# innate2adaptive/decombinator

Hardware: AMD Instinct MI355X
Metric: Mreads/s decombined (150 bp human-beta) (higher is better)
Workload: dtype u8

## Files before the change

decombinator_amd/csrc/dcrx_kernels_v2.hip:

```cpp
#include <hip/hip_runtime.h>
#include <hip/hip_ext.h>

#include <algorithm>
#include <cstddef>
#include <cstdio>
#include <cstdlib>
#include <vector>

#include "../../include/dcrx.h"
#include "dcrx_device.h"
#include "dcrx_launch.h"
#include "dcrx_dcr_device.h"
#include "dcrx_v2_device.h"
#include "dcrx_sink_device.h"

namespace dcrx {

bool first_use_on_device(bool (&seen)[64]);
void attributes_set_on_device(bool (&seen)[64]);

constexpr int DCRX_V2_BLOCK = 1024;
#ifdef DCRX_SCAN_STAMPS
__device__ uint32_t *g_scan_stamps;
#endif
// ... 115 lines not shown
    const uint32_t n_ok = (uint32_t)__popcll(m_ok), n_jn = (uint32_t)__popcll(m_jn), n_jm = (uint32_t)__popcll(m_jm),
                   n_tl = (uint32_t)__popcll(m_tl), n_im = (uint32_t)__popcll(m_im), n_ov = (uint32_t)__popcll(m_ov);
    const uint32_t all = (uint32_t)__popcll(m_all);
    if (m_jw) atomicAdd(&lds_counts[DCRX_C_VJ_ASSIGNMENT_FAILED], (uint32_t)__popcll(m_jw));
    if (all) atomicAdd(&lds_counts[DCRX_C_READ_COUNT], all);
    if (n_ok) { atomicAdd(&lds_counts[DCRX_C_VJ_COUNT], n_ok); if (forward) atomicAdd(&lds_counts[DCRX_C_FRAME_FORWARD], n_ok); }
    if (n_jn) atomicAdd(&lds_counts[DCRX_C_NO_J_ASSIGNED], n_jn);
    if (n_jm) atomicAdd(&lds_counts[DCRX_C_MULTIPLE_J_MATCHES], n_jm);
    if (n_jn + n_jm) atomicAdd(&lds_counts[DCRX_C_VJ_ASSIGNMENT_FAILED], n_jn + n_jm);
    if (n_tl) atomicAdd(&lds_counts[DCRX_C_DCRFILTER_TOOLONG_INTERTAG], n_tl);
    if (n_im) atomicAdd(&lds_counts[DCRX_C_DCRFILTER_IMPOSS_DELETION], n_im);
    if (n_ov) atomicAdd(&lds_counts[DCRX_C_DCRFILTER_TAG_OVERLAP], n_ov);
  }
}

__device__ __forceinline__ void v2_tally_rescue(uint32_t *lds_counts, const int lane, const int status, const uint32_t errs, const bool forward) {
  const bool done = status >= 0;
  const unsigned long long m_all = __ballot(done);
  if (!m_all) return;
  auto cnt = [&](const bool c) { return (uint32_t)__popcll(__ballot(done && c)); };
  const uint32_t n_ok = cnt(status == DCRX_S_OK), n_v1 = cnt(status == DCRX_S_V_HALF1_EXHAUSTED), n_v2 = cnt(status == DCRX_S_V_HALF2_EXHAUSTED),
                 n_vn = cnt(status == DCRX_S_V_NONE), n_jm = cnt(status == DCRX_S_J_MULTI), n_jn = cnt(status == DCRX_S_J_NONE),
                 n_j1 = cnt(status == DCRX_S_J_HALF1_EXHAUSTED), n_j2 = cnt(status == DCRX_S_J_HALF2_EXHAUSTED),
                 n_tl = cnt(status == DCRX_S_F_TOOLONG), n_im = cnt(status == DCRX_S_F_IMPOSS_DEL), n_ov = cnt(status == DCRX_S_F_OVERLAP),
                 n_jw = cnt(status == DCRX_S_J_WALK_FAIL),
                 e_v1 = cnt((errs & 1u) != 0u), e_v2 = cnt((errs & 2u) != 0u), e_j1 = cnt((errs & 4u) != 0u), e_j2 = cnt((errs & 8u) != 0u);
  if (lane == 0) {
    auto add = [&](const int c, const uint32_t k) { if (k) atomicAdd(&lds_counts[c], k); };
    add(DCRX_C_READ_COUNT, (uint32_t)__popcll(m_all));
    add(DCRX_C_VJ_COUNT, n_ok);
    if (forward) add(DCRX_C_FRAME_FORWARD, n_ok);
    add(DCRX_C_FOUNDV1NOTV2, n_v1);
    add(DCRX_C_FOUNDV2NOTV1, n_v2 + n_j2);
    add(DCRX_C_NO_VTAGS_FOUND, n_vn);
    add(DCRX_C_MULTIPLE_J_MATCHES, n_jm);
    add(DCRX_C_NO_J_ASSIGNED, n_jn);
    add(DCRX_C_FOUNDJ1NOTJ2, n_j1);
    add(DCRX_C_VJ_ASSIGNMENT_FAILED, n_jm + n_jn + n_j1 + n_j2 + n_jw);
    add(DCRX_C_DCRFILTER_TOOLONG_INTERTAG, n_tl);
    add(DCRX_C_DCRFILTER_IMPOSS_DELETION, n_im);
    add(DCRX_C_DCRFILTER_TAG_OVERLAP, n_ov);
    add(DCRX_C_VERR1, e_v1); add(DCRX_C_VERR2, e_v2); add(DCRX_C_JERR1, e_j1); add(DCRX_C_JERR2, e_j2);
  }
}

template <int NW, int RPL>
__device__ __forceinline__ void v2_load_item(const BatchDev &B, const uint32_t nw, const uint64_t first, const uint64_t hi, const int lane,
                                             uint32_t (&w)[RPL][NW], unsigned long long (&xm)[RPL]) {
#pragma unroll
  for (int q = 0; q < RPL; q++) {
    const uint64_t r = first + (uint64_t)q * 64 + lane;
    const uint2 *wp2 = reinterpret_cast<const uint2 *>(B.packed + (r < hi ? r : 0) * B.stride);
#pragma unroll
    for (int k = 0; k < NW / 2; k++) {
      uint2 t = make_uint2(0u, 0u);
      if ((uint32_t)(2 * k) < nw && r < hi) t = wp2[k];
      w[q][2 * k] = t.x; w[q][2 * k + 1] = t.y;
    }
    xm[q] = 0ull;
    if (B.n_exc) {
      const uint64_t g = (first + (uint64_t)q * 64) >> 5;
      xm[q] = (unsigned long long)B.exc_flag[g] | ((unsigned long long)B.exc_flag[g + 1] << 32);
    }
  }
}


__device__ __forceinline__ void v2_exc_slice(const BatchDev &B, const uint64_t blk_lo, const uint64_t blk_hi, uint32_t *s, const int tid) {
  if (B.n_exc <= 16u * blockDim.x) {
    if (tid < 4) s[tid] = 0u;
    __syncthreads();
    uint32_t below_lo = 0, below_hi = 0;
    for (uint64_t i = (uint32_t)tid; i < B.n_exc; i += blockDim.x) {
      const uint64_t r = B.exc_read[i];
      below_lo += r < blk_lo ? 1u : 0u;
      below_hi += r < blk_hi ? 1u : 0u;
    }
#pragma unroll
    for (int o = 32; o > 0; o >>= 1) { below_lo += __shfl_xor(below_lo, o); below_hi += __shfl_xor(below_hi, o); }
    if ((tid & 63) == 0) { if (below_lo) atomicAdd(&s[0], below_lo); if (below_hi) atomicAdd(&s[2], below_hi); }
    __syncthreads();
    return;
  }
  const uint32_t half = blockDim.x >> 1;
  const int which = (uint32_t)tid >= half ? 1 : 0;
  const uint32_t j = (uint32_t)tid - (which ? half : 0u);
  const uint64_t key = which ? blk_hi : blk_lo;
  if (tid < 2) { s[2 * tid] = 0u; s[2 * tid + 1] = (uint32_t)B.n_exc; }
  for (;;) {
    __syncthreads();
    const uint32_t lo = s[2 * which], hi = s[2 * which + 1], span = hi - lo;
    const bool done = s[1] == s[0] && s[3] == s[2];
    __syncthreads();
    if (done) break;
    if (tid < 2) s[4 + tid] = 0u;
    __syncthreads();
    const uint32_t step = span ? (span + half - 1) / half : 1u;
    const uint64_t idx = (uint64_t)lo + (uint64_t)j * step;
    const bool below = span && idx < hi && (uint64_t)B.exc_read[idx] < key;
    const unsigned long long m = __ballot(below);
    if ((tid & 63) == 0 && m) atomicAdd(&s[4 + which], (uint32_t)__popcll(m));
    __syncthreads();
    if (j == 0 && span) {
      const uint32_t c = s[4 + which], probes = (span + step - 1) / step;
      s[2 * which] = c ? lo + (c - 1) * step + 1 : lo;
      s[2 * which + 1] = c < probes ? lo + c * step : hi;
    }
  }
}
__device__ __forceinline__ void v2_exc_marks(const BatchDev &B, const uint32_t e_lo, const uint32_t e_hi, const bool set, const int tid) {
  uint32_t *flag = const_cast<uint32_t *>(B.exc_flag);
  for (uint64_t i = (uint64_t)e_lo + (uint32_t)tid; i < e_hi; i += blockDim.x) {
    const uint32_t r = B.exc_read[i];
    if (set) { if (i == e_lo || B.exc_read[i - 1] != r) atomicOr(&flag[r >> 5], 1u << (r & 31)); }
    else flag[r >> 5] = 0u;
  }
}

template <int NW>
__device__ __forceinline__ uint32_t *v2_left_valid(uint4 *left_rows) { return reinterpret_cast<uint32_t *>(left_rows + (size_t)V2_LEFT_CAP * V2Rows<NW>::E); }
template <int NW>
__device__ __forceinline__ bool v2_left_push(uint4 *left_rows, uint32_t *__restrict__ queue_count, const uint32_t x0, const uint32_t (&lg)[NW], const uint32_t (&w)[NW]) {
  const uint32_t at = atomicAdd(queue_count + V2_QC_LEFT, 1u);
  if (at >= V2_LEFT_CAP) return false;
  uint32_t x[1 + 2 * NW];
  x[0] = x0;
#pragma unroll
  for (int k = 0; k < NW; k++) { x[1 + k] = lg[k]; x[1 + NW + k] = w[k]; }
  v2_put_rows<1 + 2 * NW>(left_rows, 0u, at, x);
  __threadfence();
  __hip_atomic_store(v2_left_valid<NW>(left_rows) + at, 1u, __ATOMIC_RELAXED, __HIP_MEMORY_SCOPE_AGENT);
  return true;
}

enum { V2_WK_NEXT = 0, V2_WK_LIST = 1, V2_WK_EXC = 8, V2_WK_HEAD = 16, V2_WK_CLAIM = 17, V2_WK_SCANNED = 18, V2_WK_SINK = 19, V2_WK_HEAD2 = 20, V2_WK_CLAIM2 = 21,
       V2_WK_FILLED = 32, V2_WK_GEN = 48, V2_WK_FILLED2 = 64, V2_WK_GEN2 = 80, V2_WK_WORDS = 96 };
#ifndef DCRX_V2_FUSE_TAILWAVES
#define DCRX_V2_FUSE_TAILWAVES 3
#endif
#ifndef DCRX_V2_PRIO_TAIL
#define DCRX_V2_PRIO_TAIL 1
#endif
constexpr int V2_FUSE_TAILWAVES = DCRX_V2_FUSE_TAILWAVES;
constexpr uint32_t V2_TW6_FRAC256 = 243, V2_TW5_FRAC256 = 205, V2_TW4_FRAC256 = 136, V2_TW3_FRAC256 = 64;
constexpr int V2_RING_STRIDE = 15;
constexpr uint32_t V2_RING_MAXBATCHES = 16;
template <int NW> constexpr int v2_ering_stride() { return (2 * NW + 4) | 1; }
constexpr uint32_t V2_ERING_BATCHES = 8;
#ifndef DCRX_V2_HELP_DRAIN
#define DCRX_V2_HELP_DRAIN 0
#endif
constexpr float V2_FUSE_E_MAX_SHARE = 0.25f;

template <bool UNIFORM_LEN, int NW, int RPL, bool NARROW, bool PREFETCH = true, int FUSE = -1, bool SINK = false, bool FUSE_E = false>
__global__ __launch_bounds__(DCRX_V2_BLOCK) void scan2_kernel(
    DevTables T0, BatchDev B, CfgDev cfg, dcrx_record_t *__restrict__ records, unsigned long long *__restrict__ counters,
    V2Lists Q, uint32_t *__restrict__ queue, uint32_t *__restrict__ gqueue, uint32_t qcap, uint32_t *__restrict__ queue_count,
    uint64_t per_block, uint32_t retry, const DevTables *__restrict__ Tmem, uint32_t ring_batches, V2SinkCall S, uint32_t tail_waves, uint32_t rescue_waves) {
  static_assert(!FUSE_E || (FUSE >= 0 && !SINK), "the event ring rides on the fused form, without a tuple sink");
  extern __shared__ __align__(64) uint32_t smem[];
  if constexpr (FUSE >= 0 && !SINK) S.dev = nullptr;
  const int o = FUSE >= 0 ? FUSE : (cfg.orientation == DCRX_ORIENT_FORWARD ? 0 : 1);
  V2Ori V0 = T0.v2[0];
  if (o) V0 = T0.v2[1];
  uint32_t *lds_trans = smem;
  uint32_t *lds_counts = smem + V0.trans_bytes / 4;
  uint32_t *lds_work = lds_counts + DCRX_N_COUNTERS;
  const int tid = threadIdx.x;
#ifdef DCRX_SCAN_STAMPS
  const unsigned long long stamp_r0 = __builtin_amdgcn_s_memrealtime();
  unsigned long long stamp_setup = 0, stamp_loop_end = 0;
#endif
  if (tid < DCRX_N_COUNTERS) lds_counts[tid] = 0;
  if (tid < V2_WK_WORDS) lds_work[tid] = 0;
  {
    const uint4 *src = reinterpret_cast<const uint4 *>(V0.trans);
    uint4 *dst = reinterpret_cast<uint4 *>(lds_trans);
    for (uint32_t i = tid; i < V0.trans_bytes / 16; i += blockDim.x) dst[i] = src[i];
  }
  const V2Tab tab{};
  uint32_t *lds_side = lds_work + V2_WK_WORDS;
  uint32_t *lds_bk = lds_side + (T0.lds_image_bytes - T0.dfa_bytes) / 4;
  uint32_t *ring = lds_bk + V0.bk_bytes / 4;
  const uint32_t ring_mask = 64u * ring_batches - 1u;
  constexpr uint32_t ES = (uint32_t)v2_ering_stride<NW>(), ering_mask = 64u * V2_ERING_BATCHES - 1u;
  uint32_t *ring2 = ring + (size_t)(ring_mask + 1u) * V2_RING_STRIDE;
  uint32_t *lds_dry = ring2 + (size_t)(ering_mask + 1u) * ES;
  if (FUSE >= 0) {
    {
      const uint4 *s1 = reinterpret_cast<const uint4 *>(T0.image + T0.dfa_bytes), *s2 = reinterpret_cast<const uint4 *>(V0.bk);
      uint4 *d1 = reinterpret_cast<uint4 *>(lds_side), *d2 = reinterpret_cast<uint4 *>(lds_bk);
      for (uint32_t i = tid; i < (T0.lds_image_bytes - T0.dfa_bytes) / 16; i += blockDim.x) d1[i] = s1[i];
      for (uint32_t i = tid; i < V0.bk_bytes / 16; i += blockDim.x) d2[i] = s2[i];
    }
    for (uint32_t i = tid; i <= ring_mask; i += blockDim.x) { ring[i * V2_RING_STRIDE + NW] = 0u; ring[i * V2_RING_STRIDE + NW + 1] = 0u; }
    if (FUSE_E) for (uint32_t i = tid; i <= ering_mask; i += blockDim.x) { ring2[i * ES + NW] = 0u; ring2[i * ES + NW + 1] = 0u; }
  }
  __syncthreads();
  const uint32_t nw = B.stride >> 2;
  const int lane = tid & 63;
  const unsigned long long lt_mask = (1ull << lane) - 1ull;
  const bool tagged = B.n_reads < (1ull << 30);

  const uint64_t blk_lo = (uint64_t)blockIdx.x * per_block;
  const uint64_t blk_hi = blk_lo + per_block < B.n_reads ? blk_lo + per_block : B.n_reads;
  uint32_t e_lo = 0u, e_hi = 0u;
  if (B.n_exc) {
    v2_exc_slice(B, blk_lo < blk_hi ? blk_lo : blk_hi, blk_hi, lds_work + V2_WK_EXC, tid);
    e_lo = lds_work[V2_WK_EXC]; e_hi = lds_work[V2_WK_EXC + 2];
    v2_exc_marks(B, e_lo, e_hi, true, tid);
    asm volatile("s_waitcnt vmcnt(0)" ::: "memory");
    __syncthreads();
  }
  uint32_t tw = tail_waves;
  if (FUSE >= 0 && tw == 0u) {
    const uint32_t h = Q.counts[V2_L_COUNTS * blockIdx.x + V2_L_TWHINT + (o ? 0 : 1)];
    tw = (h >= 2u && h <= 8u) ? h : (uint32_t)V2_FUSE_TAILWAVES;
    if (FUSE_E && tw > 2u) tw -= 1u;
  }
  const uint32_t rw = FUSE_E ? rescue_waves : 0u;
  const uint32_t n_scan_waves = (blockDim.x >> 6) - (FUSE >= 0 ? tw : 0u) - rw;
  const size_t region = blockIdx.x;
#ifdef DCRX_SCAN_STAMPS
  stamp_setup = __builtin_amdgcn_s_memrealtime();
#endif
  const uint32_t wv = (uint32_t)(tid >> 6);
  const bool scans = wv < n_scan_waves;
  if (scans) {
#ifdef DCRX_V2_PRIO_SCAN
  if (FUSE >= 0) __builtin_amdgcn_s_setprio(DCRX_V2_PRIO_SCAN);
#endif
  constexpr uint32_t WT = 64u * RPL;
  const uint32_t n_items = blk_lo < blk_hi ? (uint32_t)((blk_hi - blk_lo + WT - 1) / WT) : 0u;
  uint4 *tq = Q.tail + region * Q.tcap * V2Rows<NW>::T;
  uint4 *eq = Q.ev + region * Q.ecap * V2Rows<NW>::E;
  auto draw = [&]() -> uint32_t {
    uint32_t i = 0;
    if (lane == 0) i = atomicAdd(&lds_work[V2_WK_NEXT], 1u);
    return (uint32_t)__builtin_amdgcn_readfirstlane((int)i);
  };

  const int npairs = UNIFORM_LEN ? (int)((B.read_len + 1u) >> 1) : 8 * (int)(nw < (uint32_t)NW ? nw : (uint32_t)NW);
  uint32_t w[RPL][NW];
  unsigned long long xm[RPL];
  uint32_t item = draw();
  if (PREFETCH && item < n_items) v2_load_item<NW, RPL>(B, nw, blk_lo + (uint64_t)item * WT, blk_hi, lane, w, xm);
  if (PREFETCH) {
#pragma unroll
    for (int q = 0; q < RPL; q++) {
#pragma unroll
      for (int k = 0; k < NW; k++) asm volatile("" : "+v"(w[q][k]));
      asm volatile("" : "+v"(xm[q]));
    }
  }
  while (item < n_items) {
    uint32_t wn[RPL][NW];
    unsigned long long xn[RPL];
    const uint32_t next = draw();
    const bool more = next < n_items;
    if (!PREFETCH) v2_load_item<NW, RPL>(B, nw, blk_lo + (uint64_t)item * WT, blk_hi, lane, w, xm);
    if (PREFETCH) { if (more) v2_load_item<NW, RPL>(B, nw, blk_lo + (uint64_t)next * WT, blk_hi, lane, wn, xn); }
    uint32_t lg[RPL][NW];
#if DCRX_V2_LOOP_PRIO
    __builtin_amdgcn_s_setprio(DCRX_V2_LOOP_PRIO);
#endif
    if (UNIFORM_LEN && NW == 10 && npairs == 75) scan2<NW, RPL, NARROW, (UNIFORM_LEN && NW == 10) ? 75 : 0>(tab, w, lg, npairs);
    else scan2<NW, RPL, NARROW>(tab, w, lg, npairs);
#if DCRX_V2_LOOP_PRIO
    __builtin_amdgcn_s_setprio(0);
#endif
    unsigned long long tmask[RPL];
    uint32_t tdg[RPL];
#pragma unroll
    for (int q = 0; q < RPL; q++) { tmask[q] = 0ull; tdg[q] = 0u; }
#pragma unroll
    for (int q = 0; q < RPL; q++) {
      const uint64_t r = blk_lo + (uint64_t)item * WT + (uint64_t)q * 64 + lane;
      bool live = r < blk_hi;
      if (retry && live) live = records[r].status != DCRX_S_OK;
      const bool exc = live && ((xm[q] >> lane) & 1ull);
      const int n = UNIFORM_LEN ? (int)B.read_len : (live ? (int)B.lens[r] : 0);
      if (!UNIFORM_LEN) mask_log2<NW>(lg[q], n);
      const Digest2 d = digest2_scan<NW>(lg[q]);
      if (cfg.flags & DCRX_F_PROFILE_SCAN_ONLY) {
        if (live) {
          __align__(16) dcrx_record_t rec;
          rec.v = (uint16_t)d.any; rec.j = (uint16_t)d.vf_n; rec.v_start = (uint16_t)d.vf_pair; rec.j_end = (uint16_t)d.jf_n;
          rec.ins_start = (uint16_t)d.jf_pair; rec.ins_len = 0; rec.vdel = rec.jdel = 0; rec.status = 254; rec.frame = 0;
          DCRX_STORE_SCAN(records + r, rec);
        }
        continue;
      }
      const uint32_t bnd = (n & 1) ? log_nibble<NW>(lg[q], n >> 1) : 0u;
      int what = live ? classify2(d, bnd) : -1;
      if (exc && what != V2_VNONE) what = V2_EVENTS;
      const bool vnone = what == V2_VNONE, vmulti = what == V2_VMULTI;
#if DCRX_V2_FULL_LINE_RECORDS
      if (live && !(FUSE >= 0 && what == V2_TAIL)) {
#else
      if (vnone || vmulti) {
#endif
        __align__(16) dcrx_record_t rec;
        rec.v = rec.j = rec.v_start = rec.j_end = rec.ins_start = rec.ins_len = 0;
        rec.vdel = rec.jdel = 0;
        rec.status = (uint8_t)(vnone ? DCRX_S_V_NONE : (vmulti ? DCRX_S_V_MULTI : DCRX_S_DEFER));
        rec.frame = (uint8_t)(o == 0 ? 1 : 0);
        DCRX_STORE_SCAN(records + r, rec);
      }
      const unsigned long long mn = __ballot(vnone), mm = __ballot(vmulti);
      if (lane == 0) {
        if (mn) atomicAdd(&lds_counts[DCRX_C_NO_VTAGS_FOUND], (uint32_t)__popcll(mn));
        if (mm) atomicAdd(&lds_counts[DCRX_C_MULTIPLE_V_MATCHES], (uint32_t)__popcll(mm));
        if (mn | mm) atomicAdd(&lds_counts[DCRX_C_READ_COUNT], (uint32_t)__popcll(mn | mm));
      }
      if (cfg.flags & DCRX_F_PROFILE_NO_FINISH) continue;
      bool to_tail = what == V2_TAIL;
      const unsigned long long mt0 = __ballot(to_tail);
      if (FUSE >= 0) {
        tmask[q] = mt0; tdg[q] = tail2_pack(d);
      } else if (mt0) {
        uint32_t base = 0;
        if (lane == 0) base = atomicAdd(&lds_work[V2_WK_LIST + V2_L_TAIL], (uint32_t)__popcll(mt0));
        base = (uint32_t)__builtin_amdgcn_readfirstlane((int)base);
        const uint32_t at = base + (uint32_t)__popcll(mt0 & lt_mask);
        if (to_tail && at >= Q.tcap) { v2_hand_over(B, queue, gqueue, qcap, queue_count, tagged, (uint32_t)r, false); to_tail = false; }
        if (to_tail) {
          uint32_t x[2 + NW];
          x[0] = (uint32_t)r; x[1] = tail2_pack(d);
#pragma unroll
          for (int k = 0; k < NW; k++) x[2 + k] = w[q][k];
          v2_put_rows<2 + NW>(tq, Q.tcap, at, x);
        }
      }
      int lst = 0;
      if (what == V2_EVENTS) lst = (exc || bnd) ? V2_L_X : (shape2(d.vf_n, d.jf_n, d.any) == V2_SHAPE_BOTH ? V2_L_C : V2_L_E);
      auto put_event = [&](uint4 *rows, const uint32_t at) {
        uint32_t x[2 + 2 * NW];
        x[0] = (uint32_t)r | (exc ? V2_R_EXC : 0u);
#pragma unroll
        for (int k = 0; k < NW; k++) { x[1 + k] = lg[q][k]; x[1 + NW + k] = w[q][k]; }
        x[1 + 2 * NW] = rescue2_digest_pack(d);
        v2_put_rows<2 + 2 * NW>(rows, 0u, at, x);
      };
      bool to_ev = lst == V2_L_E;
      const unsigned long long me0 = __ballot(to_ev);
      if (FUSE_E) {
        if (me0) {
          constexpr uint32_t nb_mask = V2_ERING_BATCHES - 1u, nb_shift = (uint32_t)__builtin_ctz(V2_ERING_BATCHES);
          const uint32_t total = (uint32_t)__popcll(me0);
          const uint32_t genv = __hip_atomic_load(&lds_work[V2_WK_GEN2 + ((uint32_t)lane & nb_mask)], __ATOMIC_RELAXED, __HIP_MEMORY_SCOPE_WORKGROUP);
          uint32_t base = 0;
          if (lane == 0) base = atomicAdd(&lds_work[V2_WK_HEAD2], total);
          base = (uint32_t)__builtin_amdgcn_readfirstlane((int)base);
          const uint32_t gb0 = base >> 6, gbl = (base + total - 1u) >> 6;
          bool room = true;
          for (uint32_t g = gb0; g <= gbl; g++) room = room && (uint32_t)__builtin_amdgcn_readlane((int)genv, (int)(g & nb_mask)) >= (g >> nb_shift);
          if (!room && lane == 0) {
            bool ok = false;
            for (uint32_t spins = 0; spins < (1u << 24) && !ok; spins++) {
              ok = true;
              for (uint32_t g = gb0; g <= gbl; g++)
                ok = ok && __hip_atomic_load(&lds_work[V2_WK_GEN2 + (g & nb_mask)], __ATOMIC_RELAXED, __HIP_MEMORY_SCOPE_WORKGROUP) >= (g >> nb_shift);
              if (!ok) __builtin_amdgcn_s_sleep(2);
            }
            if (!ok) atomicAdd(&counters[DCRX_C_DEVICE_ERRORS], 1ull);
          }
          asm volatile("" ::: "memory");
          if (to_ev) {
            uint32_t *sl = ring2 + ((base + (uint32_t)__popcll(me0 & lt_mask)) & ering_mask) * ES;
#pragma unroll
            for (int k = 0; k < NW; k++) { sl[k] = w[q][k]; sl[NW + 3 + k] = lg[q][k]; }
            sl[NW + 2] = (uint32_t)r; sl[2 * NW + 3] = rescue2_digest_pack(d);
          }
          asm volatile("" ::: "memory");
          if (lane == 0) {
            for (uint32_t g = gb0; g <= gbl; g++) {
              const uint32_t lo = max(base, g << 6), hi = min(base + total, (g + 1u) << 6);
              atomicAdd(&lds_work[V2_WK_FILLED2 + (g & nb_mask)], hi - lo);
            }
          }
        }
      } else if (me0) {
        uint32_t base = 0;
        if (lane == 0) base = atomicAdd(&lds_work[V2_WK_LIST + V2_L_E], (uint32_t)__popcll(me0));
        base = (uint32_t)__builtin_amdgcn_readfirstlane((int)base);
        const uint32_t at = base + (uint32_t)__popcll(me0 & lt_mask);
        if (to_ev && at >= Q.ecap) {
          v2_hand_over(B, queue, gqueue, qcap, queue_count, tagged, (uint32_t)r, exc);
          to_ev = false;
        }
        if (to_ev) put_event(eq, at);
      }
      if (__ballot(lst > V2_L_E)) {
#pragma unroll 1
        for (int which = V2_L_C; which <= V2_L_X; which++) {
          const bool mine = lst == which;
          const unsigned long long mr = __ballot(mine);
          if (!mr) continue;
          uint32_t base = 0;
          if (lane == 0) base = atomicAdd(&lds_work[V2_WK_LIST + which], (uint32_t)__popcll(mr));
          base = (uint32_t)__builtin_amdgcn_readfirstlane((int)base);
          if (mine) {
            const V2ListRef l = v2_list<NW>(Q, which, region);
            const uint32_t at = base + (uint32_t)__popcll(mr & lt_mask);
            if (at >= l.cap) v2_hand_over(B, queue, gqueue, qcap, queue_count, tagged, (uint32_t)r, exc);
            else put_event(l.rows, at);
          }
        }
      }
    }
    if constexpr (FUSE >= 0) {
      uint32_t cnts[RPL], total = 0;
#pragma unroll
      for (int q = 0; q < RPL; q++) { cnts[q] = (uint32_t)__popcll(tmask[q]); total += cnts[q]; }
      if (total) {
        const uint32_t nb_mask = ring_batches - 1u, nb_shift = (uint32_t)__builtin_ctz(ring_batches);
        const uint32_t genv = __hip_atomic_load(&lds_work[V2_WK_GEN + ((uint32_t)lane & nb_mask)], __ATOMIC_RELAXED, __HIP_MEMORY_SCOPE_WORKGROUP);
        uint32_t base = 0;
        if (lane == 0) base = atomicAdd(&lds_work[V2_WK_HEAD], total);
        base = (uint32_t)__builtin_amdgcn_readfirstlane((int)base);
        const uint32_t gb0 = base >> 6, gbl = (base + total - 1u) >> 6;
        bool room = true;
        for (uint32_t g = gb0; g <= gbl; g++) room = room && (uint32_t)__builtin_amdgcn_readlane((int)genv, (int)(g & nb_mask)) >= (g >> nb_shift);
        if (!room && lane == 0) {
          bool ok = false;
          for (uint32_t spins = 0; spins < (1u << 24) && !ok; spins++) {
            ok = true;
            for (uint32_t g = gb0; g <= gbl; g++)
              ok = ok && __hip_atomic_load(&lds_work[V2_WK_GEN + (g & nb_mask)], __ATOMIC_RELAXED, __HIP_MEMORY_SCOPE_WORKGROUP) >= (g >> nb_shift);
            if (!ok) __builtin_amdgcn_s_sleep(2);
          }
          if (!ok) atomicAdd(&counters[DCRX_C_DEVICE_ERRORS], 1ull);
        }
        asm volatile("" ::: "memory");
        uint32_t at0 = base;
#pragma unroll
        for (int q = 0; q < RPL; q++) {
          if ((tmask[q] >> lane) & 1ull) {
            uint32_t *sl = ring + ((at0 + (uint32_t)__popcll(tmask[q] & lt_mask)) & ring_mask) * V2_RING_STRIDE;
#pragma unroll
            for (int k = 0; k < NW; k++) sl[k] = w[q][k];
            sl[NW + 2] = (uint32_t)(blk_lo + (uint64_t)item * WT + (uint64_t)q * 64 + lane); sl[NW + 3] = tdg[q];
          }
          at0 += cnts[q];
        }
        asm volatile("" ::: "memory");
        if (lane == 0) {
          for (uint32_t g = gb0; g <= gbl; g++) {
            const uint32_t lo = max(base, g << 6), hi = min(base + total, (g + 1u) << 6);
            atomicAdd(&lds_work[V2_WK_FILLED + (g & nb_mask)], hi - lo);
          }
        }
      }
    }
    if (PREFETCH && more) {
#pragma unroll
      for (int q = 0; q < RPL; q++) {
#pragma unroll
        for (int k = 0; k < NW; k++) w[q][k] = wn[q][k];
        xm[q] = xn[q];
      }
    }
    item = next;
  }
  if (FUSE >= 0 && lane == 0) {
    asm volatile("s_waitcnt lgkmcnt(0)" ::: "memory");
    atomicAdd(&lds_work[V2_WK_SCANNED], 1u);
  }
  }
  if (FUSE_E && (wv >= n_scan_waves + tw || (DCRX_V2_HELP_DRAIN && scans))) {
   if constexpr (FUSE_E) {
    constexpr bool REV = FUSE == 1;
#if DCRX_V2_PRIO_TAIL
    __builtin_amdgcn_s_setprio(DCRX_V2_PRIO_TAIL);
#endif
    uint32_t kw_base[K_NCLASS];
#pragma unroll
    for (int c = 0; c < K_NCLASS; c++) kw_base[c] = T0.kw_base[c];
    const Rescue2Tabs rt = rescue2_tabs(T0, V0, reinterpret_cast<const uint8_t *>(lds_side), reinterpret_cast<const uint8_t *>(lds_bk), REV, kw_base);
    const Counters C{lds_counts}, Cdry{lds_dry};
    constexpr uint32_t nb_mask = V2_ERING_BATCHES - 1u, nb_shift = (uint32_t)__builtin_ctz(V2_ERING_BATCHES);
    constexpr uint32_t V2_RING_EXIT = 0xFFFFFFFFu;
    for (uint32_t spins = 0;;) {
      uint32_t c = 0, nvalid = 0;
      if (lane == 0) {
        c = __hip_atomic_load(&lds_work[V2_WK_CLAIM2], __ATOMIC_RELAXED, __HIP_MEMORY_SCOPE_WORKGROUP);
        const bool mine = __hip_atomic_load(&lds_work[V2_WK_GEN2 + (c & nb_mask)], __ATOMIC_RELAXED, __HIP_MEMORY_SCOPE_WORKGROUP) == (c >> nb_shift);
        const uint32_t f = __hip_atomic_load(&lds_work[V2_WK_FILLED2 + (c & nb_mask)], __ATOMIC_RELAXED, __HIP_MEMORY_SCOPE_WORKGROUP);
        if (!mine) nvalid = 0;
        else if (f == 64u) nvalid = 64u;
        else if (__hip_atomic_load(&lds_work[V2_WK_SCANNED], __ATOMIC_RELAXED, __HIP_MEMORY_SCOPE_WORKGROUP) == n_scan_waves) {
          const uint32_t h = __hip_atomic_load(&lds_work[V2_WK_HEAD2], __ATOMIC_RELAXED, __HIP_MEMORY_SCOPE_WORKGROUP);
          const uint32_t rem = h - 64u * c;
          nvalid = (int32_t)rem <= 0 ? V2_RING_EXIT : min(rem, 64u);
        }
        if (nvalid && nvalid != V2_RING_EXIT) {
          uint32_t expect = c;
          if (!__hip_atomic_compare_exchange_strong(&lds_work[V2_WK_CLAIM2], &expect, c + 1u, __ATOMIC_RELAXED, __ATOMIC_RELAXED, __HIP_MEMORY_SCOPE_WORKGROUP)) nvalid = 0;
        }
      }
      c = (uint32_t)__builtin_amdgcn_readfirstlane((int)c);
      nvalid = (uint32_t)__builtin_amdgcn_readfirstlane((int)nvalid);
      if (nvalid == V2_RING_EXIT) break;
      if (!nvalid) {
        if (++spins > (1u << 24)) { if (lane == 0) atomicAdd(&counters[DCRX_C_DEVICE_ERRORS], 1ull); break; }
        __builtin_amdgcn_s_sleep(4);
        continue;
      }
      asm volatile("s_waitcnt lgkmcnt(0)" ::: "memory");
      uint32_t *sl = ring2 + ((64u * c + (uint32_t)lane) & ering_mask) * ES;
      int status = -2;
      uint32_t errs = 0, x0 = 0;
      uint32_t lg[NW];
#pragma unroll
      for (int k = 0; k < NW; k++) lg[k] = 0u;
      if ((uint32_t)lane < nvalid) {
        x0 = sl[NW + 2];
#pragma unroll
        for (int k = 0; k < NW; k++) lg[k] = sl[NW + 3 + k];
        const uint32_t dg = sl[2 * NW + 3];
        const uint32_t r = x0 & V2_R_MASK;
        const int n = UNIFORM_LEN ? (int)B.read_len : (int)B.lens[r];
        const LdsWords lw{dcrx_ldsaddr_of(sl)};
        auto on_ok = [&](dcrx_record_t rec, const uint32_t) {
          rec.frame = (uint8_t)(o ? 0 : 1);
          DCRX_STORE_FINISH(records + r, rec);
        };
        status = rescue2_fast_to<REV, NW, V2_SHAPE_ONE>(rt, lw, lg, n, cfg, on_ok, errs, *Tmem, C, Cdry, dg);
        if (status > 0) {
          dcrx_record_t rec;
          rec.v = rec.j = rec.v_start = rec.j_end = rec.ins_start = rec.ins_len = 0; rec.vdel = rec.jdel = 0;
          rec.status = (uint8_t)status; rec.frame = (uint8_t)(o ? 0 : 1);
          DCRX_STORE_FINISH(records + r, rec);
        } else if (status < 0) errs = 0;
      }
      v2_tally_rescue(lds_counts, lane, status, errs, o == 0);
      if (__builtin_expect(status == RESCUE2_SLOW, 0)) {
        uint32_t ww[NW];
#pragma unroll
        for (int k = 0; k < NW; k++) ww[k] = sl[k];
        if (!v2_left_push<NW>(Q.left, queue_count, x0, lg, ww)) v2_hand_over(B, queue, gqueue, qcap, queue_count, tagged, x0 & V2_R_MASK, false);
      }
      asm volatile("s_waitcnt lgkmcnt(0)" ::: "memory");
      if (lane == 0) {
        __hip_atomic_store(&lds_work[V2_WK_FILLED2 + (c & nb_mask)], 0u, __ATOMIC_RELAXED, __HIP_MEMORY_SCOPE_WORKGROUP);
        asm volatile("s_waitcnt lgkmcnt(0)" ::: "memory");
        atomicAdd(&lds_work[V2_WK_GEN2 + (c & nb_mask)], 1u);
      }
      spins = 0;
    }
   }
  }
  if (FUSE >= 0 && (DCRX_V2_HELP_DRAIN || (wv >= n_scan_waves && wv < n_scan_waves + tw))) {
   if constexpr (FUSE >= 0) {
    constexpr bool REV = FUSE == 1;
#if DCRX_V2_PRIO_TAIL
    __builtin_amdgcn_s_setprio(DCRX_V2_PRIO_TAIL);
#endif
    const Tail2Tabs tt = tail2_tabs(T0, V0, reinterpret_cast<const uint8_t *>(lds_side), reinterpret_cast<const uint8_t *>(lds_bk), REV);
    const Counters C{lds_counts};
    const uint32_t nb_mask = ring_batches - 1u, nb_shift = (uint32_t)__builtin_ctz(ring_batches);
    constexpr uint32_t V2_RING_EXIT = 0xFFFFFFFFu;
    for (uint32_t spins = 0;;) {
      uint32_t c = 0, nvalid = 0;
      if (lane == 0) {
        c = __hip_atomic_load(&lds_work[V2_WK_CLAIM], __ATOMIC_RELAXED, __HIP_MEMORY_SCOPE_WORKGROUP);
        const bool mine = __hip_atomic_load(&lds_work[V2_WK_GEN + (c & nb_mask)], __ATOMIC_RELAXED, __HIP_MEMORY_SCOPE_WORKGROUP) == (c >> nb_shift);
        const uint32_t f = __hip_atomic_load(&lds_work[V2_WK_FILLED + (c & nb_mask)], __ATOMIC_RELAXED, __HIP_MEMORY_SCOPE_WORKGROUP);
        if (!mine) nvalid = 0;
        else if (f == 64u) nvalid = 64u;
        else if (__hip_atomic_load(&lds_work[V2_WK_SCANNED], __ATOMIC_RELAXED, __HIP_MEMORY_SCOPE_WORKGROUP) == n_scan_waves) {
          const uint32_t h = __hip_atomic_load(&lds_work[V2_WK_HEAD], __ATOMIC_RELAXED, __HIP_MEMORY_SCOPE_WORKGROUP);
          const uint32_t rem = h - 64u * c;
          nvalid = (int32_t)rem <= 0 ? V2_RING_EXIT : min(rem, 64u);
        }
        if (nvalid && nvalid != V2_RING_EXIT) {
          uint32_t expect = c;
          if (!__hip_atomic_compare_exchange_strong(&lds_work[V2_WK_CLAIM], &expect, c + 1u, __ATOMIC_RELAXED, __ATOMIC_RELAXED, __HIP_MEMORY_SCOPE_WORKGROUP)) nvalid = 0;
        }
      }
      c = (uint32_t)__builtin_amdgcn_readfirstlane((int)c);
      nvalid = (uint32_t)__builtin_amdgcn_readfirstlane((int)nvalid);
      if (nvalid == V2_RING_EXIT) break;
      if (!nvalid) {
        if (++spins > (1u << 24)) {
          if (lane == 0) atomicAdd(&counters[DCRX_C_DEVICE_ERRORS], 1ull);
          break;
        }
        __builtin_amdgcn_s_sleep(4);
        continue;
      }
      asm volatile("s_waitcnt lgkmcnt(0)" ::: "memory");
      uint32_t *sl = ring + ((64u * c + (uint32_t)lane) & ring_mask) * V2_RING_STRIDE;
      int status = -2;
      uint32_t r = 0, dg = 0;
      uint64_t tup = 0;
      if ((uint32_t)lane < nvalid) {
        r = sl[NW + 2]; dg = sl[NW + 3];
        const int n = UNIFORM_LEN ? (int)B.read_len : (int)B.lens[r];
        dcrx_record_t rec;
        rec.v = rec.j = rec.v_start = rec.j_end = rec.ins_start = rec.ins_len = 0; rec.vdel = rec.jdel = 0;
        const LdsWords lw{dcrx_ldsaddr_of(sl)};
        if (cfg.flags & DCRX_F_PROFILE_TAIL_STREAM_ONLY) { status = DCRX_S_J_NONE; rec.v = (uint16_t)(sl[0] ^ sl[NW - 1]); }
        else
        status = tail2_fast<REV>(tt, lw, n, dg, cfg, rec, *Tmem, C);
        rec.frame = (uint8_t)(o ? 0 : 1);
        if (status >= 0) { rec.status = (uint8_t)status; DCRX_STORE_FINISH(records + r, rec); }
        if (S.dev && status == DCRX_S_OK) tup = sink_tuple_lean(rec, S.wpack, false);
      }
      v2_tally(lds_counts, lane, status, o == 0);
      if (S.dev) sink_put(S, (uint32_t)region, 0u, 64u * c + (uint32_t)lane, (uint32_t)lane < nvalid, status == DCRX_S_OK, r, tup, lane, &lds_work[V2_WK_SINK]);
      if (__builtin_expect(status == TAIL2_SLOW, 0)) {
        __align__(16) dcrx_record_t rec;
        rec.v = rec.j = rec.v_start = rec.j_end = rec.ins_start = rec.ins_len = 0; rec.vdel = rec.jdel = 0;
        rec.status = (uint8_t)DCRX_S_DEFER; rec.frame = (uint8_t)(o ? 0 : 1);
        DCRX_STORE_FINISH(records + r, rec);
        const uint32_t vp = dg & 0xFFu, jp = (dg >> 8) & 0xFFu, jc = (dg >> 16) & 3u;
        uint32_t lg[NW], ww[NW];
#pragma unroll
        for (int k = 0; k < NW; k++) {
          uint32_t l = (vp >> 3) == (uint32_t)k ? (V2_F_VF << (4 * (vp & 7u))) : 0u;
          if (jc == 1u && (jp >> 3) == (uint32_t)k) l |= V2_F_JF << (4 * (jp & 7u));
          lg[k] = l; ww[k] = sl[k];
        }
        if (!v2_left_push<NW>(Q.left, queue_count, r | (jc == 2u ? V2_R_JMULTI : 0u), lg, ww)) v2_hand_over(B, queue, gqueue, qcap, queue_count, tagged, r, false);
      }
      asm volatile("s_waitcnt lgkmcnt(0)" ::: "memory");
      if (lane == 0) {
        __hip_atomic_store(&lds_work[V2_WK_FILLED + (c & nb_mask)], 0u, __ATOMIC_RELAXED, __HIP_MEMORY_SCOPE_WORKGROUP);
        asm volatile("s_waitcnt lgkmcnt(0)" ::: "memory");
        atomicAdd(&lds_work[V2_WK_GEN + (c & nb_mask)], 1u);
      }
      spins = 0;
    }
   }
  }
#ifdef DCRX_SCAN_STAMPS
  stamp_loop_end = __builtin_amdgcn_s_memrealtime();
#endif
  __syncthreads();
  if (B.n_exc) v2_exc_marks(B, e_lo, e_hi, false, tid);
#ifdef DCRX_SCAN_STAMPS
  if (lane == 0) {
    uint32_t *c = g_scan_stamps + 4 * ((size_t)blockIdx.x * (DCRX_V2_BLOCK / 64) + (size_t)(tid >> 6));
    c[0] = (uint32_t)stamp_r0; c[1] = (uint32_t)stamp_setup; c[2] = (uint32_t)stamp_loop_end; c[3] = (uint32_t)__builtin_amdgcn_s_memrealtime();
  }
#else
  if (tid < V2_L_COUNTS) {
    uint32_t c = tid <= V2_L_X ? lds_work[V2_WK_LIST + tid] : 0u;
    c = min(c, tid == V2_L_TAIL ? Q.tcap : (tid == V2_L_E ? Q.ecap : Q.scap / 2));
    if (tid == V2_L_RING) c = lds_work[V2_WK_HEAD];
    if ((tid == V2_L_TWHINT || tid == V2_L_TWHINT + 1) && FUSE >= 0) c = Q.counts[V2_L_COUNTS * region + tid];
    if (tid == V2_L_TWHINT + (o ? 0 : 1) && FUSE >= 0 && blk_hi > blk_lo) {
      const uint32_t frac256 = (uint32_t)(((uint64_t)lds_work[V2_WK_HEAD] << 8) / (blk_hi - blk_lo));
      c = frac256 >= V2_TW6_FRAC256 ? 6u : (frac256 >= V2_TW5_FRAC256 ? 5u : (frac256 >= V2_TW4_FRAC256 ? 4u : (frac256 >= V2_TW3_FRAC256 ? 3u : 2u)));
    }
    Q.counts[V2_L_COUNTS * region + tid] = c;
  }
  if (S.dev && tid == 0 && lds_work[V2_WK_SINK]) (void)__hip_atomic_fetch_add(S.hits + region, lds_work[V2_WK_SINK], __ATOMIC_RELAXED, __HIP_MEMORY_SCOPE_AGENT);
#endif
  if (tid < DCRX_N_COUNTERS && lds_counts[tid]) atomicAdd(&counters[tid], (unsigned long long)lds_counts[tid]);
}

static uint32_t v2_finish_lds_bytes(const DevTables &T, int o) {
  return DCRX_N_COUNTERS * 4 + (T.lds_image_bytes - T.dfa_bytes) + T.v2[o].bk_bytes;
}

template <bool UNIFORM_LEN, int NW, int ORI>
__device__ __forceinline__ void v2_general_entry(const DevTables &T, const V2Ori &V, const BatchDev &B, const CfgDev &cfg, const uint32_t x0,
                                                 const uint32_t (&lg)[NW], const uint32_t (&w)[NW], const Counters &C, dcrx_record_t *__restrict__ records,
                                                 uint32_t *__restrict__ queue, uint32_t *__restrict__ gqueue, const uint32_t qcap,
                                                 uint32_t *__restrict__ queue_count, const bool tagged) {
  const uint32_t r = x0 & V2_R_MASK;
  const bool exc = (x0 & V2_R_EXC) != 0u;
  const int n = UNIFORM_LEN ? (int)B.read_len : (int)B.lens[r];
  const Digest2 d = digest2<NW>(lg);
  const uint32_t bnd = (n & 1) ? log_nibble<NW>(lg, n >> 1) : 0u;
  uint32_t ev[3];
  const bool fits = events2<NW>(lg, d, exc ? 0xFu : bnd, ev);
  if (!fits) { v2_hand_over(B, queue, gqueue, qcap, queue_count, tagged, r, exc); return; }
  int x0e = 0, x1e = 0;
  if (exc) {
    uint64_t lo = 0, hi = B.n_exc;
    while (lo < hi) { const uint64_t mid = (lo + hi) >> 1; if (B.exc_read[mid] < r) lo = mid + 1; else hi = mid; }
    x0e = (int)lo;
    while (lo < B.n_exc && B.exc_read[lo] == r) lo++;
    x1e = (int)lo;
    ExcLayout xl;
    if (x1e - x0e > V2_MAX_EXC && !exc_layout(B.exc_pos, B.exc_chr, x0e, x1e, xl)) {
      v2_hand_over(B, queue, gqueue, qcap, queue_count, tagged, r, true); return;
    }
  }
  if (!finish2_words<UNIFORM_LEN, NW, ORI>(T, V, B, cfg, (uint64_t)r, w, ev, (x0 & V2_R_JMULTI) != 0u, x0e, x1e, C, records))
    v2_hand_over(B, queue, gqueue, qcap, queue_count, tagged, r, exc);
}

constexpr int V2_LEFT_SLOTS = 15;
struct V2FinishLds {
  uint32_t *counts, *side, *bk, *strip, *dry, *left;
};
template <int NW, int BLOCK>
__device__ __forceinline__ V2FinishLds v2_finish_layout(const DevTables &T0, const V2Ori &V, uint32_t *smem, const int tid) {
  V2FinishLds L;
  L.counts = smem;
  L.side = smem + DCRX_N_COUNTERS;
  L.bk = L.side + (T0.lds_image_bytes - T0.dfa_bytes) / 4;
  L.strip = L.bk + V.bk_bytes / 4 + (uint32_t)tid * lds_words_stride<NW>();
  L.dry = L.bk + V.bk_bytes / 4 + (uint32_t)BLOCK * lds_words_stride<NW>();
  L.left = L.dry + DCRX_N_COUNTERS + (uint32_t)(tid >> 6) * (1 + V2_LEFT_SLOTS);
  return L;
}
template <int NW, int BLOCK>
__device__ __forceinline__ V2FinishLds v2_finish_stage(const DevTables &T0, const V2Ori &V, uint32_t *smem, const int tid) {
  const V2FinishLds L = v2_finish_layout<NW, BLOCK>(T0, V, smem, tid);
  if (tid < DCRX_N_COUNTERS) L.counts[tid] = 0;
  stage_lds<BLOCK>(T0.image + T0.dfa_bytes, L.side, (T0.lds_image_bytes - T0.dfa_bytes) / 16, 0, 0, tid);
  stage_lds<BLOCK>(V.bk, L.bk, V.bk_bytes / 16, 0, 0, tid);
  L.strip[NW] = 0u; L.strip[NW + 1] = 0u;
  if ((tid & 63) == 0) L.left[0] = 0u;
  return L;
}
template <int NW>
static uint32_t v2_finish_block_lds(const DevTables &T, int o, int block) {
  return DCRX_N_COUNTERS * 4 + (T.lds_image_bytes - T.dfa_bytes) + T.v2[o].bk_bytes + (uint32_t)block * lds_words_stride<NW>() * 4 + DCRX_N_COUNTERS * 4 +
         (uint32_t)(block / 64) * (1 + V2_LEFT_SLOTS) * 4;
}

__device__ __forceinline__ void v2_note_left(uint32_t *left, const uint32_t slot, const BatchDev &B, uint32_t *__restrict__ queue, uint32_t *__restrict__ gqueue,
                                             const uint32_t qcap, uint32_t *__restrict__ queue_count, const uint32_t r, const bool exc) {
  const uint32_t at = atomicAdd(&left[0], 1u);
  if (at < (uint32_t)V2_LEFT_SLOTS) left[1 + at] = slot;
  else v2_hand_over(B, queue, gqueue, qcap, queue_count, B.n_reads < (1ull << 30), r, exc);
}
template <int NW>
struct V2EntryWords { uint32_t lg[NW], w[NW]; };
template <bool UNIFORM_LEN, int NW, int ORI>
__device__ __forceinline__ void v2_tail_jobs(const Tail2Tabs &tt, const V2FinishLds &L, const BatchDev &B, const CfgDev &cfg, dcrx_record_t *__restrict__ records,
                                             const V2Lists &Q, const uint32_t n_regions, const uint32_t split, uint32_t *__restrict__ queue,
                                             uint32_t *__restrict__ gqueue, const uint32_t qcap, uint32_t *__restrict__ queue_count,
                                             const DevTables *__restrict__ Tmem, const uint32_t gwave, const uint32_t n_gwaves, const int tid, const V2SinkCall &S) {
  constexpr int o = ORI;
  const Counters C{L.counts};
  const LdsWords lw{dcrx_ldsaddr_of(L.strip)};
  uint32_t *strip = L.strip, *lds_counts = L.counts;
  uint32_t *s_left = L.left;
  const int lane = tid & 63;
  for (uint32_t job = gwave; job < n_regions * split; job += n_gwaves) {
    const uint32_t region = job / split, part = job % split;
    const uint32_t tn = Q.counts[V2_L_COUNTS * region + V2_L_TAIL];
    const uint4 *tq = Q.tail + (size_t)region * Q.tcap * V2Rows<NW>::T;
    const uint32_t STEP = 64 * split;
    constexpr bool AHEAD = NW <= DCRX_NWMAX;
    uint32_t x1[2 + NW];
    if constexpr (AHEAD) v2_get_rows<2 + NW>(tq, Q.tcap, 64 * part + lane, 64 * part + lane < tn, x1);
    for (uint32_t first = 64 * part; first < tn && !(cfg.flags & DCRX_F_PROFILE_NO_TAIL); first += STEP) {
      uint32_t x[2 + NW];
      if constexpr (AHEAD) {
#pragma unroll
        for (int k = 0; k < 2 + NW; k++) x[k] = x1[k];
        const uint32_t nf = v2_landed(x, first + STEP);
        v2_get_rows<2 + NW>(tq, Q.tcap, nf + lane, nf + lane < tn, x1);
      } else {
        v2_get_rows<2 + NW>(tq, Q.tcap, first + lane, first + lane < tn, x);
      }
      uint32_t w[NW];
#pragma unroll
      for (int k = 0; k < NW; k++) w[k] = x[2 + k];
      int status = -2;
      uint64_t tup = 0;
      const uint32_t r = x[0], dg = x[1];
      if (first + lane < tn) {
        const int n = UNIFORM_LEN ? (int)B.read_len : (int)B.lens[r];
        dcrx_record_t rec;
        rec.v = rec.j = rec.v_start = rec.j_end = rec.ins_start = rec.ins_len = 0; rec.vdel = rec.jdel = 0;
#if DCRX_LEAN_LDS_WORDS
#pragma unroll
        for (int k = 0; k < NW; k++) strip[k] = w[k];
        if (cfg.flags & DCRX_F_PROFILE_TAIL_STREAM_ONLY) { status = DCRX_S_J_NONE; rec.v = (uint16_t)(w[0] ^ w[NW - 1]); }
        else
        status = tail2_fast<ORI == 1>(tt, lw, n, dg, cfg, rec, *Tmem, C);
#else
        const RegWords<NW> rw{w};
        status = tail2_fast<ORI == 1>(tt, rw, n, dg, cfg, rec, *Tmem, C);
#endif
        if (status >= 0) { rec.status = (uint8_t)status; rec.frame = (uint8_t)(o ? 0 : 1); DCRX_STORE_FINISH(records + r, rec); }
        if (S.dev && status == DCRX_S_OK) tup = sink_tuple_lean(rec, S.wpack, false);
      }
      v2_tally(lds_counts, lane, status, o == 0);
      if (S.dev) sink_put(S, region, 0u, first + (uint32_t)lane, first + lane < tn, status == DCRX_S_OK, r, tup, lane, nullptr);
      if (__builtin_expect(status == TAIL2_SLOW, 0)) v2_note_left(s_left, first + (uint32_t)lane, B, queue, gqueue, qcap, queue_count, r, false);
    }
    const uint32_t n_left = min(s_left[0], (uint32_t)V2_LEFT_SLOTS);
    if (__builtin_expect(n_left != 0u, 0)) {
      const bool live = (uint32_t)lane < n_left;
      const uint32_t slot = live ? s_left[1 + lane] : 0u;
      uint32_t x[2 + NW];
      v2_get_rows<2 + NW>(tq, Q.tcap, slot, live, x);
      if (live) {
        const uint32_t dg = x[1], vp = dg & 0xFFu, jp = (dg >> 8) & 0xFFu, jc = (dg >> 16) & 3u;
        V2EntryWords<NW> e;
#pragma unroll
        for (int k = 0; k < NW; k++) {
          uint32_t l = (vp >> 3) == (uint32_t)k ? (V2_F_VF << (4 * (vp & 7u))) : 0u;
          if (jc == 1u && (jp >> 3) == (uint32_t)k) l |= V2_F_JF << (4 * (jp & 7u));
          e.lg[k] = l; e.w[k] = x[2 + k];
        }
        if (!v2_left_push<NW>(Q.left, queue_count, x[0] | (jc == 2u ? V2_R_JMULTI : 0u), e.lg, e.w)) v2_hand_over(B, queue, gqueue, qcap, queue_count, B.n_reads < (1ull << 30), x[0], false);
      }
      if (lane == 0) s_left[0] = 0u;
    }
  }
}

template <bool UNIFORM_LEN, int NW, int ORI>
__device__ __forceinline__ void v2_rescue_jobs(const Rescue2Tabs &rt, const V2FinishLds &L, const BatchDev &B, const CfgDev &cfg, dcrx_record_t *__restrict__ records,
                                               const V2Lists &Q, const uint32_t n_regions, const uint32_t split_ec, uint32_t *__restrict__ queue,
                                               uint32_t *__restrict__ gqueue, const uint32_t qcap, uint32_t *__restrict__ queue_count,
                                               const DevTables *__restrict__ Tmem, const uint32_t gwave, const uint32_t n_gwaves, const int tid, const V2SinkCall &S,
                                               uint32_t *__restrict__ tickets) {
  constexpr int o = ORI;
  const Counters C{L.counts}, Cdry{L.dry};
  const LdsWords lw{dcrx_ldsaddr_of(L.strip)};
  uint32_t *strip = L.strip, *lds_counts = L.counts;
  uint32_t *s_left = L.left;
  const int lane = tid & 63;
  const uint32_t split_e = split_ec & 255u, split_c = (split_ec >> 8) ? (split_ec >> 8) : split_e;
  for (uint32_t job = gwave; job < n_regions * (split_e + split_c) && !(cfg.flags & DCRX_F_PROFILE_NO_EVENTS); job += n_gwaves) {
    const int which = job < n_regions * split_e ? V2_L_E : V2_L_C;
    const uint32_t split = which == V2_L_E ? split_e : split_c, jrel = which == V2_L_E ? job : job - n_regions * split_e;
    const uint32_t region = jrel / split, part = jrel % split;
    const V2ListRef l = v2_list<NW>(Q, which, region);
    const uint32_t en = min(Q.counts[V2_L_COUNTS * region + which], l.cap);
    auto draw = [&]() -> uint32_t {
      uint32_t t = 0;
      if (lane == 0) t = __hip_atomic_fetch_add(tickets + V2_L_COUNTS * region + V2_L_TICKETS, which == V2_L_E ? 1u : 0x10000u, __ATOMIC_RELAXED, __HIP_MEMORY_SCOPE_AGENT);
      t = (uint32_t)__builtin_amdgcn_readfirstlane((int)t);
      return split + (which == V2_L_E ? (t & 0xFFFFu) : (t >> 16));
    };
    constexpr bool AHEAD = NW <= 10;
    uint32_t x1[2 + 2 * NW];
    uint32_t first = 64 * part, next_first = 64 * part + 64 * en + 64;
    if (first < en) next_first = 64 * draw();
    if constexpr (AHEAD) v2_get_rows<2 + 2 * NW>(l.rows, l.cap, first + lane, first + lane < en, x1);
    for (; first < en; ) {
      uint32_t x[2 + 2 * NW];
      const bool more = next_first < en;
      uint32_t after_raw = 0;
      uint32_t nf = next_first;
      if constexpr (AHEAD) {
#pragma unroll
        for (int k = 0; k < 2 + 2 * NW; k++) x[k] = x1[k];
        nf = v2_landed(x, next_first);
      }
      if (more && lane == 0) after_raw = __hip_atomic_fetch_add(tickets + V2_L_COUNTS * region + V2_L_TICKETS, which == V2_L_E ? 1u : 0x10000u, __ATOMIC_RELAXED, __HIP_MEMORY_SCOPE_AGENT);
      if constexpr (AHEAD) {
        v2_get_rows<2 + 2 * NW>(l.rows, l.cap, nf + lane, nf + lane < en, x1);
      } else {
        v2_get_rows<2 + 2 * NW>(l.rows, l.cap, first + lane, first + lane < en, x);
      }
      uint32_t lg[NW], w[NW];
#pragma unroll
      for (int k = 0; k < NW; k++) { lg[k] = x[1 + k]; w[k] = x[1 + NW + k]; }
      int status = -2;
      uint32_t errs = 0;
      uint64_t tup = 0;
      const uint32_t r = x[0] & V2_R_MASK;
      if (first + lane < en) {
        status = RESCUE2_SLOW;
        if (!(x[0] & V2_R_EXC)) {
          const int n = UNIFORM_LEN ? (int)B.read_len : (int)B.lens[r];
#pragma unroll
          for (int k = 0; k < NW; k++) strip[k] = w[k];
          auto on_ok = [&](dcrx_record_t rec, const uint32_t e) {
            rec.frame = (uint8_t)(o ? 0 : 1);
            DCRX_STORE_FINISH(records + r, rec);
            if (S.dev) tup = sink_tuple_lean(rec, S.wpack, (e & 8u) != 0u && 2 * rt.split[1] != (int)rt.t.L[1]);
          };
          if (which == V2_L_E) status = rescue2_fast_to<ORI == 1, NW, V2_SHAPE_ONE>(rt, lw, lg, n, cfg, on_ok, errs, *Tmem, C, Cdry, x[1 + 2 * NW]);
          else status = rescue2_fast_to<ORI == 1, NW, V2_SHAPE_BOTH>(rt, lw, lg, n, cfg, on_ok, errs, *Tmem, C, Cdry, x[1 + 2 * NW]);
          if (status > 0) {
            dcrx_record_t rec;
            rec.v = rec.j = rec.v_start = rec.j_end = rec.ins_start = rec.ins_len = 0; rec.vdel = rec.jdel = 0;
            rec.status = (uint8_t)status; rec.frame = (uint8_t)(o ? 0 : 1);
            DCRX_STORE_FINISH(records + r, rec);
          } else if (status < 0) errs = 0;
        }
      }
      v2_tally_rescue(lds_counts, lane, status, errs, o == 0);
      if (S.dev) sink_put(S, region, which == V2_L_E ? S.e_off : S.c_off, first + (uint32_t)lane, first + lane < en, status == DCRX_S_OK, r, tup, lane, nullptr);
      if (__builtin_expect(status == RESCUE2_SLOW, 0)) v2_note_left(s_left, first + (uint32_t)lane, B, queue, gqueue, qcap, queue_count, r, (x[0] & V2_R_EXC) != 0u);
      first = next_first;
      if (more) {
        const uint32_t t = (uint32_t)__builtin_amdgcn_readfirstlane((int)after_raw);
        next_first = 64u * (split + (which == V2_L_E ? (t & 0xFFFFu) : (t >> 16)));
      }
    }
    const uint32_t n_left = min(s_left[0], (uint32_t)V2_LEFT_SLOTS);
    if (__builtin_expect(n_left != 0u, 0)) {
      const bool live = (uint32_t)lane < n_left;
      const uint32_t slot = live ? s_left[1 + lane] : 0u;
      uint32_t x[1 + 2 * NW];
      v2_get_rows<1 + 2 * NW>(l.rows, l.cap, slot, live, x);
      if (live) {
        V2EntryWords<NW> e;
#pragma unroll
        for (int k = 0; k < NW; k++) { e.lg[k] = x[1 + k]; e.w[k] = x[1 + NW + k]; }
        if (!v2_left_push<NW>(Q.left, queue_count, x[0], e.lg, e.w)) v2_hand_over(B, queue, gqueue, qcap, queue_count, B.n_reads < (1ull << 30), x[0] & V2_R_MASK, (x[0] & V2_R_EXC) != 0u);
      }
      if (lane == 0) s_left[0] = 0u;
    }
  }
}

template <bool UNIFORM_LEN, int NW, int ORI, bool SINK>
DCRX_V2_ROLE void v2_general_role(const uint32_t mode_, const uint32_t vblock_, const uint32_t ka_lo, const uint32_t ka_hi);

struct V2Roles { uint32_t xgrid, rgrid, tgrid, rsplit, tsplit, bsplit, width; };
struct V2FinishArgs {
  DevTables T0; BatchDev B; CfgDev cfg; dcrx_record_t *records; unsigned long long *counters; V2Lists Q; uint32_t n_regions; V2Roles R;
  uint32_t *queue, *gqueue; uint32_t qcap; uint32_t *queue_count; const DevTables *Tmem; V2SinkCall S;
};
typedef const __attribute__((address_space(4))) uint32_t *dcrx_kwords;
template <class T>
__device__ __forceinline__ T v2_karg(const dcrx_kwords base, const size_t offset) {
  static_assert(sizeof(T) % 4 == 0, "whole dwords");
  T out;
  uint32_t *d = reinterpret_cast<uint32_t *>(&out);
#pragma unroll
  for (size_t i = 0; i < sizeof(T) / 4; i++) d[i] = base[offset / 4 + i];
  return out;
}
template <class T>
__device__ __forceinline__ T *v2_global(T *p) {
  return (T *)(__attribute__((address_space(1))) T *)(uintptr_t)p;
}
template <class T>
__device__ __forceinline__ T *v2_constant(T *p) { return (T *)(__attribute__((address_space(4))) T *)(uintptr_t)p; }
struct V2FinishLocals {
  DevTables T0; BatchDev B; CfgDev cfg; dcrx_record_t *records; V2Lists Q; uint32_t n_regions; V2Roles R;
  uint32_t *queue, *gqueue; uint32_t qcap; uint32_t *queue_count; const DevTables *Tmem; V2SinkCall S;
  uint32_t *tickets;
};
__device__ __forceinline__ V2FinishLocals v2_finish_args(const uint32_t lo, const uint32_t hi) {
  uint32_t slo = (uint32_t)__builtin_amdgcn_readfirstlane((int)lo), shi = (uint32_t)__builtin_amdgcn_readfirstlane((int)hi);
  asm volatile("" : "+s"(slo), "+s"(shi));
  const uint64_t p = (uint64_t)slo | ((uint64_t)shi << 32);
  const dcrx_kwords k = reinterpret_cast<dcrx_kwords>(p);
  V2FinishLocals A;
#define DCRX_KARG(F) A.F = v2_karg<decltype(A.F)>(k, offsetof(V2FinishArgs, F))
  DCRX_KARG(T0); DCRX_KARG(B); DCRX_KARG(cfg); DCRX_KARG(records); DCRX_KARG(Q); DCRX_KARG(R);
  DCRX_KARG(queue); DCRX_KARG(gqueue); DCRX_KARG(queue_count); DCRX_KARG(Tmem); DCRX_KARG(S);
#undef DCRX_KARG
  A.n_regions = k[offsetof(V2FinishArgs, n_regions) / 4];
  A.qcap = k[offsetof(V2FinishArgs, qcap) / 4];
#define DCRX_GLOBAL(P) P = v2_global(P)
  DCRX_GLOBAL(A.records); DCRX_GLOBAL(A.Q.tail); DCRX_GLOBAL(A.Q.ev); DCRX_GLOBAL(A.Q.sx); DCRX_GLOBAL(A.queue);
  DCRX_GLOBAL(A.gqueue); DCRX_GLOBAL(A.queue_count); DCRX_GLOBAL(A.B.packed); DCRX_GLOBAL(A.B.lens); DCRX_GLOBAL(A.B.exc_read);
  DCRX_GLOBAL(A.B.exc_pos); DCRX_GLOBAL(A.B.exc_chr); DCRX_GLOBAL(A.B.exc_flag); DCRX_GLOBAL(A.T0.image);
#undef DCRX_GLOBAL
  A.tickets = v2_global(A.Q.counts);
  A.Tmem = v2_constant(A.Tmem); A.Q.counts = v2_constant(A.Q.counts); A.T0.kw_base = v2_constant(A.T0.kw_base);
  A.S.dev = v2_constant(A.S.dev);
  A.S.items = v2_global(A.S.items); A.S.hits = v2_global(A.S.hits);
  return A;
}
template <bool UNIFORM_LEN, int NW, int ORI, bool SINK>
DCRX_V2_ROLE void v2_rescue_role(const uint32_t vblock_, const uint32_t ka_lo, const uint32_t ka_hi) {
  extern __shared__ __align__(64) uint32_t smem[];
  V2FinishLocals A = v2_finish_args(ka_lo, ka_hi);
  if constexpr (!SINK) A.S.dev = nullptr;
  const uint32_t vblock = (uint32_t)__builtin_amdgcn_readfirstlane((int)vblock_);
  const int tid = threadIdx.x;
  const V2Ori V = A.T0.v2[ORI];
  const V2FinishLds L = v2_finish_layout<NW, DCRX_V2_FBLOCK>(A.T0, V, smem, tid);
  uint32_t kw_base[K_NCLASS];
#pragma unroll
  for (int c = 0; c < K_NCLASS; c++) kw_base[c] = A.T0.kw_base[c];
  const Rescue2Tabs rt = rescue2_tabs(A.T0, V, reinterpret_cast<const uint8_t *>(L.side), reinterpret_cast<const uint8_t *>(L.bk), ORI == 1, kw_base);
  constexpr uint32_t WPB = DCRX_V2_FBLOCK / 64;
  v2_rescue_jobs<UNIFORM_LEN, NW, ORI>(rt, L, A.B, A.cfg, A.records, A.Q, A.n_regions, A.R.rsplit, A.queue, A.gqueue, A.qcap, A.queue_count, A.Tmem,
                                       vblock * WPB + (uint32_t)(tid >> 6), A.R.rgrid * WPB, tid, A.S, A.tickets);
}
template <bool UNIFORM_LEN, int NW, int ORI, bool SINK>
DCRX_V2_ROLE void v2_tail_role(const uint32_t vblock_, const uint32_t ka_lo, const uint32_t ka_hi) {
  extern __shared__ __align__(64) uint32_t smem[];
  V2FinishLocals A = v2_finish_args(ka_lo, ka_hi);
  if constexpr (!SINK) A.S.dev = nullptr;
  const uint32_t vblock = (uint32_t)__builtin_amdgcn_readfirstlane((int)vblock_);
  const int tid = threadIdx.x;
  const V2Ori V = A.T0.v2[ORI];
  const V2FinishLds L = v2_finish_layout<NW, DCRX_V2_FBLOCK>(A.T0, V, smem, tid);
  const Tail2Tabs tt = tail2_tabs(A.T0, V, reinterpret_cast<const uint8_t *>(L.side), reinterpret_cast<const uint8_t *>(L.bk), ORI == 1);
  constexpr uint32_t WPB = DCRX_V2_FBLOCK / 64;
  v2_tail_jobs<UNIFORM_LEN, NW, ORI>(tt, L, A.B, A.cfg, A.records, A.Q, A.n_regions, A.R.tsplit, A.queue, A.gqueue, A.qcap, A.queue_count, A.Tmem,
                                     vblock * WPB + (uint32_t)(tid >> 6), A.R.tgrid * WPB, tid, A.S);
}
template <bool UNIFORM_LEN, int NW, int ORI, bool SINK>
DCRX_V2_ROLE void v2_general_role(const uint32_t mode_, const uint32_t vblock_, const uint32_t ka_lo, const uint32_t ka_hi) {
  extern __shared__ __align__(64) uint32_t smem[];
  V2FinishLocals A = v2_finish_args(ka_lo, ka_hi);
  if constexpr (!SINK) A.S.dev = nullptr;
  const uint32_t vblock = (uint32_t)__builtin_amdgcn_readfirstlane((int)vblock_), mode = (uint32_t)__builtin_amdgcn_readfirstlane((int)mode_);
  const int tid = threadIdx.x, lane = tid & 63;
  V2Ori V = A.T0.v2[ORI];
  const V2FinishLds L = v2_finish_layout<NW, DCRX_V2_FBLOCK>(A.T0, V, smem, tid);
  const DevTables T = tables_in_lds(A.T0, reinterpret_cast<const uint8_t *>(L.side), A.T0.dfa_bytes, false);
  V.bk = reinterpret_cast<const uint8_t *>(L.bk);
  const Counters C{L.counts};
  const bool tagged = A.B.n_reads < (1ull << 30);
  uint32_t width = A.R.width;
  const uint32_t region = vblock / A.R.bsplit, bpart = vblock % A.R.bsplit;
  const bool do_x = (mode & 1u) && region < A.n_regions && !(A.cfg.flags & DCRX_F_PROFILE_NO_EVENTS);
  const V2ListRef lx = v2_list<NW>(A.Q, V2_L_X, do_x ? region : 0u);
  const uint32_t x_total = do_x ? min(A.Q.counts[V2_L_COUNTS * region + V2_L_X], lx.cap) : 0u;
  if (x_total > 64u * A.R.bsplit * (DCRX_V2_FBLOCK / 64)) width = 64u;
  else if (x_total > 16u * A.R.bsplit * (DCRX_V2_FBLOCK / 64)) width = 16u;
  uint32_t first = width * ((uint32_t)(tid >> 6) + (DCRX_V2_FBLOCK / 64) * bpart);
  const uint32_t step = width * (DCRX_V2_FBLOCK / 64) * A.R.bsplit;
  uint4 *lrows = A.Q.left;
  uint32_t *valid = v2_left_valid<NW>(lrows);
  const uint32_t others = A.R.xgrid + A.R.rgrid + A.R.tgrid - 1u;
  bool polling = false;
  uint32_t consumed = 0, spins = 0;
  for (;;) {
    const uint4 *rows;
    uint32_t i;
    bool live;
    if (!polling) {
      if (first >= x_total) {
        if (!(mode & 2u) || tid >= 64) break;
        polling = true;
        continue;
      }
      rows = lx.rows; i = first + (uint32_t)lane; live = (uint32_t)lane < width && i < x_total;
      first += step;
    } else {
      const uint32_t done = __hip_atomic_load(A.queue_count + V2_QC_DONE, __ATOMIC_RELAXED, __HIP_MEMORY_SCOPE_AGENT);
      const uint32_t n = min(__hip_atomic_load(A.queue_count + V2_QC_LEFT, __ATOMIC_RELAXED, __HIP_MEMORY_SCOPE_AGENT), V2_LEFT_CAP);
      i = consumed + (uint32_t)lane;
      const bool ok = i < n && __hip_atomic_load(valid + (i < V2_LEFT_CAP ? i : 0u), __ATOMIC_RELAXED, __HIP_MEMORY_SCOPE_AGENT) != 0u;
      const unsigned long long m = __ballot(ok);
      const uint32_t run = ~m ? (uint32_t)__builtin_ctzll(~m) : 64u;
      if (!run) {
        if (done >= others && consumed >= n) break;
        if (++spins > (1u << 22)) break;
        __builtin_amdgcn_s_sleep(16);
        continue;
      }
      __builtin_amdgcn_fence(__ATOMIC_ACQUIRE, "agent");
      rows = lrows; live = (uint32_t)lane < run;
      consumed += run;
    }
    uint32_t x[1 + 2 * NW];
    v2_get_rows<1 + 2 * NW>(rows, 0u, i, live, x);
    uint32_t lg[NW], w[NW];
#pragma unroll
    for (int k = 0; k < NW; k++) { lg[k] = x[1 + k]; w[k] = x[1 + NW + k]; }
    if (live) {
      v2_general_entry<UNIFORM_LEN, NW, ORI>(T, V, A.B, A.cfg, x[0], lg, w, C, A.records, A.queue, A.gqueue, A.qcap, A.queue_count, tagged);
      if (A.S.dev) sink_late(A.S, A.records, x[0] & V2_R_MASK);
      if (polling) valid[i] = 0u;
    }
  }
  if (polling && lane == 0) { A.queue_count[V2_QC_LEFT] = 0u; A.queue_count[V2_QC_DONE] = 0u; }
}

template <bool UNIFORM_LEN, int NW, int ORI, bool TAIL_ROLE = true, bool SINK = false>
__global__ __launch_bounds__(DCRX_V2_FBLOCK, DCRX_V2_RWAVES) void finish2_kernel(const V2FinishArgs A) {
  extern __shared__ __align__(64) uint32_t smem[];
  const int tid = threadIdx.x;
  const V2Roles R = A.R;
  const uint64_t ka = (uint64_t)__builtin_amdgcn_kernarg_segment_ptr();
  uint32_t b = blockIdx.x;
  int role;
  bool work = true;
  if (b < R.xgrid) {
    role = 0;
    const uint32_t g = b / R.bsplit;
    work = g < A.n_regions && R.width * (DCRX_V2_FBLOCK / 64) * (b % R.bsplit) < A.Q.counts[V2_L_COUNTS * g + V2_L_X];
  } else {
    b -= R.xgrid;
    const uint32_t paired = 2u * min(R.rgrid, R.tgrid);
    if (b < paired) { role = (b & 1u) ? 2 : 1; b >>= 1; }
    else { b -= paired; role = R.rgrid > R.tgrid ? 1 : 2; b += min(R.rgrid, R.tgrid); }
  }
  const V2Ori V = A.T0.v2[ORI];
  V2FinishLds L = v2_finish_layout<NW, DCRX_V2_FBLOCK>(A.T0, V, smem, tid);
  const bool staged = work || blockIdx.x == 0;
  if (staged) {
    L = v2_finish_stage<NW, DCRX_V2_FBLOCK>(A.T0, V, smem, tid);
    __syncthreads();
    if (role == 1) v2_rescue_role<UNIFORM_LEN, NW, ORI, SINK>(b, (uint32_t)ka, (uint32_t)(ka >> 32));
    else if (TAIL_ROLE && role == 2) v2_tail_role<UNIFORM_LEN, NW, ORI, SINK>(b, (uint32_t)ka, (uint32_t)(ka >> 32));
    else v2_general_role<UNIFORM_LEN, NW, ORI, SINK>(blockIdx.x == 0 ? 3u : 1u, b, (uint32_t)ka, (uint32_t)(ka >> 32));
  }
  __syncthreads();
  if (blockIdx.x != 0 && tid == 0) atomicAdd(A.queue_count + V2_QC_DONE, 1u);
  __syncthreads();
  if (staged && tid < DCRX_N_COUNTERS && L.counts[tid]) atomicAdd(&A.counters[tid], (unsigned long long)L.counts[tid]);
}

template <bool UNIFORM_LEN, int NW, int ORI>
__global__ __launch_bounds__(DCRX_V2_FBLOCK, DCRX_V2_RWAVES) void left2_kernel(const V2FinishArgs A) {
  extern __shared__ __align__(64) uint32_t smem[];
  const int tid = threadIdx.x;
  if (A.queue_count[V2_QC_LEFT] == 0u) return;
  if (tid == 0) A.queue_count[V2_QC_DONE] = A.R.xgrid + A.R.rgrid + A.R.tgrid;
  __syncthreads();
  const uint64_t ka = (uint64_t)__builtin_amdgcn_kernarg_segment_ptr();
  const V2Ori V = A.T0.v2[ORI];
  const V2FinishLds L = v2_finish_stage<NW, DCRX_V2_FBLOCK>(A.T0, V, smem, tid);
  __syncthreads();
  v2_general_role<UNIFORM_LEN, NW, ORI, false>(2u, 0u, (uint32_t)ka, (uint32_t)(ka >> 32));
  __syncthreads();
  if (tid < DCRX_N_COUNTERS && L.counts[tid]) atomicAdd(&A.counters[tid], (unsigned long long)L.counts[tid]);
}

template <bool UNIFORM_LEN, int NW, int ORI>
__global__ __launch_bounds__(DCRX_V2_TBLOCK, DCRX_V2_TWAVES) void tail2_kernel(
    DevTables T0, BatchDev B, CfgDev cfg, dcrx_record_t *__restrict__ records, unsigned long long *__restrict__ counters,
    V2Lists Q, uint32_t n_regions, uint32_t split, uint32_t *__restrict__ queue, uint32_t *__restrict__ gqueue, uint32_t qcap,
    uint32_t *__restrict__ queue_count, const DevTables *__restrict__ Tmem) {
  extern __shared__ __align__(64) uint32_t smem[];
  const int tid = threadIdx.x;
  const V2Ori V = T0.v2[ORI];
  const V2FinishLds L = v2_finish_stage<NW, DCRX_V2_TBLOCK>(T0, V, smem, tid);
  const Tail2Tabs tt = tail2_tabs(T0, V, reinterpret_cast<const uint8_t *>(L.side), reinterpret_cast<const uint8_t *>(L.bk), ORI == 1);
  __syncthreads();
  v2_tail_jobs<UNIFORM_LEN, NW, ORI>(tt, L, B, cfg, records, Q, n_regions, split, queue, gqueue, qcap, queue_count, Tmem,
                                     blockIdx.x * (DCRX_V2_TBLOCK / 64) + (uint32_t)(tid >> 6), gridDim.x * (DCRX_V2_TBLOCK / 64), tid, V2SinkCall{});
  __syncthreads();
  if (tid < DCRX_N_COUNTERS && L.counts[tid]) atomicAdd(&counters[tid], (unsigned long long)L.counts[tid]);
}

template <bool UNIFORM_LEN, int NW, int ORI>
__global__ __launch_bounds__(DCRX_V2_FBLOCK, DCRX_V2_RWAVES) void rescue2_kernel(
    DevTables T0, BatchDev B, CfgDev cfg, dcrx_record_t *__restrict__ records, unsigned long long *__restrict__ counters,
    V2Lists Q, uint32_t n_regions, uint32_t split, uint32_t *__restrict__ queue, uint32_t *__restrict__ gqueue, uint32_t qcap,
    uint32_t *__restrict__ queue_count, const DevTables *__restrict__ Tmem) {
  extern __shared__ __align__(64) uint32_t smem[];
  const int tid = threadIdx.x;
  const V2Ori V = T0.v2[ORI];
  const V2FinishLds L = v2_finish_stage<NW, DCRX_V2_FBLOCK>(T0, V, smem, tid);
  uint32_t kw_base[K_NCLASS];
#pragma unroll
  for (int c = 0; c < K_NCLASS; c++) kw_base[c] = T0.kw_base[c];
  const Rescue2Tabs rt = rescue2_tabs(T0, V, reinterpret_cast<const uint8_t *>(L.side), reinterpret_cast<const uint8_t *>(L.bk), ORI == 1, kw_base);
  __syncthreads();
  v2_rescue_jobs<UNIFORM_LEN, NW, ORI>(rt, L, B, cfg, records, Q, n_regions, split, queue, gqueue, qcap, queue_count, Tmem,
                                       blockIdx.x * (DCRX_V2_FBLOCK / 64) + (uint32_t)(tid >> 6), gridDim.x * (DCRX_V2_FBLOCK / 64), tid, V2SinkCall{}, Q.counts);
  __syncthreads();
  if (tid < DCRX_N_COUNTERS && L.counts[tid]) atomicAdd(&counters[tid], (unsigned long long)L.counts[tid]);
}

template <bool UNIFORM_LEN, int NW, int ORI>
__global__ __launch_bounds__(DCRX_V2_FBLOCK, 4) void events2_kernel(
    DevTables T0, BatchDev B, CfgDev cfg, dcrx_record_t *__restrict__ records, unsigned long long *__restrict__ counters,
    V2Lists Q, int which, uint32_t group, uint32_t width, uint32_t bsplit, uint32_t ext, uint32_t n_regions, uint32_t *__restrict__ queue, uint32_t *__restrict__ gqueue, uint32_t qcap,
    uint32_t *__restrict__ queue_count) {
  extern __shared__ __align__(64) uint32_t smem[];
  V2Ori V = T0.v2[ORI];
  const uint32_t lcap = v2_list<NW>(Q, which, 0).cap;
  const uint32_t side_bytes = (ext ? T0.lds_image2_bytes : T0.lds_image_bytes) - T0.dfa_bytes;
  uint32_t *lds_counts = smem;
  uint32_t *lds_side = smem + DCRX_N_COUNTERS;
  uint32_t *lds_bk = lds_side + side_bytes / 4;
  const int tid = threadIdx.x;
  if (group == 1u && gridDim.x / bsplit >= n_regions) {
    const uint32_t g = blockIdx.x / bsplit;
    if (g >= n_regions || width * (DCRX_V2_FBLOCK / 64) * (blockIdx.x % bsplit) >= min(Q.counts[V2_L_COUNTS * g + which], lcap)) return;
  }
  if (tid < DCRX_N_COUNTERS) lds_counts[tid] = 0;
  stage_lds<DCRX_V2_FBLOCK>(T0.image + T0.dfa_bytes, lds_side, side_bytes / 16, 0, 0, tid);
  stage_lds<DCRX_V2_FBLOCK>(V.bk, lds_bk, V.bk_bytes / 16, 0, 0, tid);
  const DevTables T = tables_in_lds(T0, reinterpret_cast<const uint8_t *>(lds_side), T0.dfa_bytes, ext != 0u);
  V.bk = reinterpret_cast<const uint8_t *>(lds_bk);
  __syncthreads();
  const Counters C{lds_counts};
  const int lane = tid & 63;
  const bool tagged = B.n_reads < (1ull << 30);
  __shared__ uint32_t pref[DCRX_V2_GROUP_MAX + 1];
  const uint32_t bpart = blockIdx.x % bsplit, bsteps = width * (DCRX_V2_FBLOCK / 64) * bsplit;
  for (uint32_t g0 = (blockIdx.x / bsplit) * group; g0 < n_regions; g0 += (gridDim.x / bsplit) * group) {
    __syncthreads();
    if (tid == 0) {
      uint32_t acc = 0;
      for (uint32_t k = 0; k < group; k++) {
        pref[k] = acc;
        if (g0 + k < n_regions) acc += min(Q.counts[V2_L_COUNTS * (g0 + k) + which], lcap);
      }
      pref[group] = acc;
    }
    __syncthreads();
    const uint32_t total = pref[group];
    for (uint32_t first = width * ((uint32_t)(tid >> 6) + (DCRX_V2_FBLOCK / 64) * bpart); first < total && !(cfg.flags & DCRX_F_PROFILE_NO_EVENTS); first += bsteps) {
      const uint32_t i = first + lane;
      const bool live = (uint32_t)lane < width && i < total;
      uint32_t g = 0;
      for (uint32_t k = 1; k < group; k++) g += i >= pref[k] ? 1u : 0u;
      const uint32_t slot = i - pref[g];
      const V2ListRef l = v2_list<NW>(Q, which, (size_t)(g0 + g));
      uint32_t x[1 + 2 * NW];
      v2_get_rows<1 + 2 * NW>(l.rows, l.cap, slot, live, x);
      uint32_t lg[NW], w[NW];
#pragma unroll
      for (int k = 0; k < NW; k++) { lg[k] = x[1 + k]; w[k] = x[1 + NW + k]; }
      if (live) v2_general_entry<UNIFORM_LEN, NW, ORI>(T, V, B, cfg, x[0], lg, w, C, records, queue, gqueue, qcap, queue_count, tagged);
    }
  }
  __syncthreads();
  if (tid < DCRX_N_COUNTERS && lds_counts[tid]) atomicAdd(&counters[tid], (unsigned long long)lds_counts[tid]);
}

constexpr int V2_PLACE_BLOCK = 1024;
constexpr int V2_PLACE_KEEP = 24;
__device__ __forceinline__ uint32_t v2_wave_sum(uint32_t x) {
#pragma unroll
  for (int d = 32; d > 0; d >>= 1) x += (uint32_t)__shfl_xor((int)x, d);
  return x;
}
__device__ __forceinline__ uint32_t v2_block_sum(uint32_t x, uint32_t *s16, const int tid) {
  x = v2_wave_sum(x);
  __syncthreads();
  if ((tid & 63) == 0) s16[tid >> 6] = x;
  __syncthreads();
  uint32_t t = 0;
#pragma unroll
  for (int w = 0; w < V2_PLACE_BLOCK / 64; w++) t += s16[w];
  return t;
}
__device__ __forceinline__ uint32_t v2_block_exclusive(const uint32_t x, uint32_t *s16, const int tid) {
  uint32_t inc = x;
#pragma unroll
  for (int d = 1; d < 64; d <<= 1) { const uint32_t v = (uint32_t)__shfl_up((int)inc, d); if ((tid & 63) >= d) inc += v; }
  __syncthreads();
  if ((tid & 63) == 63) s16[tid >> 6] = inc;
  __syncthreads();
  uint32_t off = 0;
#pragma unroll
  for (int w = 0; w < V2_PLACE_BLOCK / 64; w++) off += w < (tid >> 6) ? s16[w] : 0u;
  return off + inc - x;
}
__global__ __launch_bounds__(V2_PLACE_BLOCK) void v2_place_kernel(const V2SinkCall S, const uint32_t *__restrict__ counts, const uint32_t n_regions,
                                                                  const uint32_t tcap, const uint32_t ecap, const uint32_t ccap, const uint32_t fused,
                                                                  const uint64_t n_reads, const uint64_t n_slots, uint8_t *__restrict__ msg,
                                                                  const uint32_t hi_bytes, uint64_t *__restrict__ d_total, const uint32_t hcap) {
  extern __shared__ __align__(16) uint32_t smem[];
  __shared__ uint32_t s16[V2_PLACE_BLOCK / 64];
  __shared__ uint32_t s_last, s_mine;
  const V2SinkDev D = *S.dev;
  const int tid = threadIdx.x;
  const uint32_t region = blockIdx.x;
  const uint32_t wpr = S.per_block >> 5;
  uint32_t *bm = smem, *pre = smem + wpr;
  uint32_t *stage_a = smem + 2 * wpr;
  uint8_t *stage_b = reinterpret_cast<uint8_t *>(stage_a + hcap);
  const uint32_t n_late = D.late[region];
  const uint32_t n_tail = fused ? counts[V2_L_COUNTS * region + V2_L_RING] : min(counts[V2_L_COUNTS * region + V2_L_TAIL], tcap);
  const uint32_t n_e = min(counts[V2_L_COUNTS * region + V2_L_E], ecap), n_c = min(counts[V2_L_COUNTS * region + V2_L_C], ccap);
  const uint32_t c0 = n_tail, c1 = c0 + n_e, c2 = c1 + n_c, n_items = c2 + min(n_late, S.late_cap);
  const uint64_t blk_lo = (uint64_t)region * S.per_block;
  const uint2 *items = S.items + (size_t)region * S.stride;
  auto addr = [&](const uint32_t f) -> uint32_t {
    return f < c0 ? f : (f < c1 ? S.e_off + (f - c0) : (f < c2 ? S.c_off + (f - c1) : S.late_off + (f - c2)));
  };
  constexpr int KEEP = V2_PLACE_KEEP;
  uint2 it[KEEP];
#pragma unroll
  for (int k = 0; k < KEEP; k++) {
    const uint32_t f = (uint32_t)tid + (uint32_t)k * V2_PLACE_BLOCK;
    it[k] = make_uint2(0u, V2_SINK_EMPTY);
    if (f < n_items) it[k] = items[addr(f)];
  }
  uint32_t before = 0, all = 0;
  for (uint32_t q = (uint32_t)tid; q < n_regions; q += V2_PLACE_BLOCK) { const uint32_t h = S.hits[q]; all += h; if (q < region) before += h; if (q == region) s_mine = h; }
  for (uint32_t i = (uint32_t)tid; i < wpr; i += V2_PLACE_BLOCK) bm[i] = 0u;
  const uint64_t base = v2_block_sum(before, s16, tid);
  const uint64_t total = v2_block_sum(all, s16, tid);
  if (tid == 0) s_last = atomicAdd(D.ticket, 1u) == n_regions - 1u ? 1u : 0u;
  auto mark = [&](const uint32_t y) { if (y != V2_SINK_EMPTY) { const uint32_t k = y & 0xFFFFFFu; atomicOr(&bm[k >> 5], 1u << (k & 31u)); } };
#pragma unroll
  for (int k = 0; k < KEEP; k++) mark(it[k].y);
  for (uint32_t f = (uint32_t)tid + (uint32_t)KEEP * V2_PLACE_BLOCK; f < n_items; f += V2_PLACE_BLOCK) mark(items[addr(f)].y);
  __syncthreads();
  const uint32_t per = (wpr + V2_PLACE_BLOCK - 1) / V2_PLACE_BLOCK;
  uint32_t run = 0;
  for (uint32_t i = (uint32_t)tid * per; i < min(((uint32_t)tid + 1u) * per, wpr); i++) run += (uint32_t)__popc(bm[i]);
  uint32_t acc = v2_block_exclusive(run, s16, tid);
  for (uint32_t i = (uint32_t)tid * per; i < min(((uint32_t)tid + 1u) * per, wpr); i++) { pre[i] = acc; acc += (uint32_t)__popc(bm[i]); }
  __syncthreads();
  const uint64_t bm_bytes = ((n_slots + 63) / 64) * 8;
  uint32_t *plane_a = reinterpret_cast<uint32_t *>(msg + bm_bytes);
  uint8_t *plane_b = msg + bm_bytes + total * 4;
  const uint32_t mine = s_mine;
  const bool staged = mine <= hcap;
  auto place = [&](const uint2 v) {
    if (v.y == V2_SINK_EMPTY) return;
    const uint32_t k = v.y & 0xFFFFFFu;
    const uint32_t rank = pre[k >> 5] + (uint32_t)__popc(bm[k >> 5] & ((1u << (k & 31u)) - 1u));
    if (staged) {
      if (rank < hcap) { stage_a[rank] = v.x; stage_b[rank] = (uint8_t)(v.y >> 24); }
    } else {
      plane_a[base + rank] = v.x;
      if (hi_bytes) plane_b[base + rank] = (uint8_t)(v.y >> 24);
    }
  };
#pragma unroll
  for (int k = 0; k < KEEP; k++) place(it[k]);
  for (uint32_t f = (uint32_t)tid + (uint32_t)KEEP * V2_PLACE_BLOCK; f < n_items; f += V2_PLACE_BLOCK) place(items[addr(f)]);
  if (staged) {
    __syncthreads();
    for (uint32_t i = (uint32_t)tid; i < mine; i += V2_PLACE_BLOCK) plane_a[base + i] = stage_a[i];
    if (hi_bytes)
      for (uint32_t i = (uint32_t)tid; i < mine; i += V2_PLACE_BLOCK) plane_b[base + i] = stage_b[i];
  }
  uint64_t *out_bm = reinterpret_cast<uint64_t *>(msg);
  const uint64_t w_lo = blk_lo >> 6, w_all = bm_bytes / 8;
  for (uint32_t i = (uint32_t)tid; i < (wpr >> 1); i += V2_PLACE_BLOCK)
    if (w_lo + i < w_all) out_bm[w_lo + i] = (uint64_t)bm[2 * i] | ((uint64_t)bm[2 * i + 1] << 32);
  if (region == n_regions - 1u)
    for (uint64_t w = w_lo + (wpr >> 1) + (uint32_t)tid; w < w_all; w += V2_PLACE_BLOCK) out_bm[w] = 0ull;
  if (region == 0 && tid == 0) *d_total = total;
  if (tid == 0) D.late[region] = 0u;
  if (s_last) {
    for (uint32_t q = (uint32_t)tid; q < n_regions; q += V2_PLACE_BLOCK) S.hits[q] = 0u;
    if (tid == 0) *D.ticket = 0u;
  }
}

static uint32_t v2_scan_lds_bytes(const DevTables &T, int o) { return T.v2[o].trans_bytes + DCRX_N_COUNTERS * 4 + V2_WK_WORDS * 4; }

bool v2_applies(const LaunchPlan &P, const DevTables &T, const CfgDev &cfg, const uint32_t stride) {
  if (!T.v2_ok || !P.v2_events || !P.v2_slow || !P.v2_acc || !P.v2_left) return false;
  if (cfg.flags & (DCRX_F_V1_KERNELS | DCRX_F_FORCE_SLOW_READER | DCRX_F_ONE_BASE_SCAN | DCRX_F_LIST_RESCUE | DCRX_F_PROFILE_LIST_SCAN_ONLY)) return false;
  auto fits = [&](int o) {
    const uint32_t fin = stride <= 40 ? v2_finish_block_lds<10>(T, o, DCRX_V2_FBLOCK)
                                      : (stride <= 4 * DCRX_NWMAX ? v2_finish_block_lds<DCRX_NWMAX>(T, o, DCRX_V2_FBLOCK) : v2_finish_block_lds<DCRX_V2_NWLONG>(T, o, DCRX_V2_FBLOCK));
    return v2_scan_lds_bytes(T, o) <= 160u * 1024u && fin <= 64u * 1024u;
  };
  if (cfg.orientation == DCRX_ORIENT_BOTH) return fits(0) && fits(1) && !(cfg.flags & DCRX_F_PROFILE_MASK);
  return fits(cfg.orientation == DCRX_ORIENT_FORWARD ? 0 : 1);
}

template <bool UNIFORM, int NW, int RPL, bool NARROW, bool PREFETCH = true>
static hipError_t launch_v2(const LaunchPlan &P, const DevTables &T, const BatchDev &B, const CfgDev &cfg, dcrx_record_t *rec,
                            uint32_t *queue, uint32_t *gqueue, uint32_t qcap, uint32_t *queue_count,
                            unsigned long long *d_counters, hipStream_t s, hipEvent_t ev_start, hipEvent_t ev_stop, uint32_t retry, V2SinkLaunch *sink) {
  const int o = cfg.orientation == DCRX_ORIENT_FORWARD ? 0 : 1;
  constexpr bool CAN_FUSE = NW == 10 && ((RPL == 2 && PREFETCH) || (RPL == 3 && !PREFETCH));
  uint32_t ring_batches = 0;
  static const uint32_t fuse_limit = [] { const char *e = dcrx_debug_env("DCRX_DEBUG_FUSE_LIMIT_KB"); const int v = e ? atoi(e) : 0; return v > 0 ? (uint32_t)v * 1024u : 64u * 1024u; }();
  if (CAN_FUSE && T.v2[o].trans_bytes <= fuse_limit && !(cfg.flags & (DCRX_F_V2_NO_FUSE | DCRX_F_V2_SIDE_STREAMS | DCRX_F_V2_LEAN_SERIAL | DCRX_F_V2_NO_LEAN_RESCUE | (DCRX_F_PROFILE_MASK & ~DCRX_F_PROFILE_TAIL_STREAM_ONLY)))) {
    const uint32_t fixed = v2_scan_lds_bytes(T, o) + (T.lds_image_bytes - T.dfa_bytes) + T.v2[o].bk_bytes;
    static const uint32_t nb_max = [] {
      const char *e = dcrx_debug_env("DCRX_DEBUG_RING_BATCHES");
      const uint32_t v = e ? (uint32_t)atoi(e) : V2_RING_MAXBATCHES;
      return (v == 4u || v == 8u || v == 16u) ? v : V2_RING_MAXBATCHES;
    }();
    const uint32_t nb_min = dcrx_debug_env("DCRX_DEBUG_RING_BATCHES") ? 4u : 8u;
    for (uint32_t nb = nb_max; nb >= nb_min; nb >>= 1)
      if (fixed + nb * 64u * V2_RING_STRIDE * 4u <= 160u * 1024u) { ring_batches = nb; break; }
  }
  auto ks = scan2_kernel<UNIFORM, NW, RPL, NARROW, PREFETCH>;
  if constexpr (CAN_FUSE) {
    if (ring_batches) ks = o ? scan2_kernel<UNIFORM, NW, RPL, NARROW, PREFETCH, 1> : scan2_kernel<UNIFORM, NW, RPL, NARROW, PREFETCH, 0>;
  }
  constexpr bool CAN_FUSE_E = CAN_FUSE && UNIFORM && RPL == 2;
  auto ks_e = ks;
  bool fuse_e = false;
  uint32_t ring_batches_e = 0, scan_lds_e = 0;
  static const int fuse_e_env = [] { const char *e = dcrx_debug_env("DCRX_DEBUG_FUSE_E"); return e ? atoi(e) : -1; }();
  static const uint32_t rescue_waves_fused = [] { const char *e = dcrx_debug_env("DCRX_DEBUG_FUSE_E_WAVES"); const int v = e ? atoi(e) : 0; return (v >= 1 && v <= 8) ? (uint32_t)v : 3u; }();
  V2TuneSlot *eslot = nullptr;
  hipEvent_t e_ev_start = nullptr, e_ev_stop = nullptr;
  if constexpr (CAN_FUSE_E) {
    const int ec = V2Tune::size_class(B.n_reads);
    if (P.tune && ec >= 0 && !retry && !cfg.flags && ring_batches) eslot = &P.tune[o].slot[ec];
    if (eslot && eslot->fuse_e == -1 && eslot->e_sampling && hipEventQuery(eslot->ev_counts) == hipSuccess) {
      uint64_t e_entries = 0;
      for (uint32_t r = 0; r < eslot->e_regions; r++) e_entries += eslot->h_counts[(size_t)V2_L_COUNTS * r + V2_L_E];
      eslot->e_share = eslot->e_reads ? (float)((double)e_entries / (double)eslot->e_reads) : 0.f;
      eslot->fuse_e = eslot->e_share <= V2_FUSE_E_MAX_SHARE ? -2 : 0;
      eslot->e_sampling = false;
      static const bool say = dcrx_debug_env("DCRX_DEBUG_TUNE") != nullptr;
      if (say) fprintf(stderr, "dcrx tune: list E holds %.1f %% of %llu reads, frame %d: %s\n", 100.0 * eslot->e_share, (unsigned long long)eslot->e_reads, o,
                       eslot->fuse_e ? "both forms will be timed" : "stays a role of the finishing launch");
    }
    (void)hipGetLastError();
    bool want = fuse_e_env >= 0 ? fuse_e_env != 0 : (eslot && eslot->fuse_e == 1);
    if (fuse_e_env < 0 && eslot && eslot->fuse_e == -2 && eslot->choice != 0u && !ev_start && !ev_stop && !P.ev_step_start && !P.ev_step_stop && !(sink && P.sink.dev)) {
      bool ok = true;
      constexpr int NP = V2TuneSlot::E_PAIRS, FIRST = V2TuneSlot::E_FIRST;
      if (!eslot->ev_e[0][0])
        for (int a = 0; a < 2 * NP && ok; a++) for (int b = 0; b < 2 && ok; b++) ok = hipEventCreate(&eslot->ev_e[a][b]) == hipSuccess;
      const int k = eslot->e_phase - FIRST;
      if (!ok) { (void)hipGetLastError(); eslot->fuse_e = 0; }
      else if (k < 0) eslot->e_phase++;
      else if (k < NP) { e_ev_start = eslot->ev_e[k][0]; e_ev_stop = eslot->ev_e[k][1]; want = false; eslot->e_phase++; }
      else if (k == NP) { want = true; eslot->e_phase++; }
      else if (k <= 2 * NP) { e_ev_start = eslot->ev_e[k - 1][0]; e_ev_stop = eslot->ev_e[k - 1][1]; want = true; eslot->e_phase++; }
      else {
        bool ready = true;
        for (int a = 0; a < 2 * NP && ready; a++) ready = hipEventQuery(eslot->ev_e[a][1]) == hipSuccess;
        want = true;
        if (ready) {
          float ms[2] = {0.f, 0.f};
          for (int a = 0; a < 2 * NP && ok; a++) { float t = 0.f; ok = hipEventElapsedTime(&t, eslot->ev_e[a][0], eslot->ev_e[a][1]) == hipSuccess; ms[a < NP ? 0 : 1] += t; }
          eslot->us_e[0] = 1e3f * ms[0] / NP; eslot->us_e[1] = 1e3f * ms[1] / NP;
          eslot->fuse_e = (ok && ms[1] > 0.f && ms[1] < 0.985f * ms[0]) ? 1 : 0;
          want = eslot->fuse_e == 1;
          static const bool say = dcrx_debug_env("DCRX_DEBUG_TUNE") != nullptr;
          if (say) fprintf(stderr, "dcrx tune: scan + finishing launch of %llu reads, frame %d: %.1f us with list E a role, %.1f inside the scan -> %s\n",
                           (unsigned long long)B.n_reads, o, eslot->us_e[0], eslot->us_e[1], eslot->fuse_e ? "inside the scan" : "a role");
        }
      }
      (void)hipGetLastError();
    }
    if (ring_batches && want && !retry && !(cfg.flags & ~(DCRX_F_V2_SHAPE(3)))) {
      const uint32_t fixed = v2_scan_lds_bytes(T, o) + (T.lds_image_bytes - T.dfa_bytes) + T.v2[o].bk_bytes + 64u * V2_ERING_BATCHES * (uint32_t)v2_ering_stride<NW>() * 4u +
                             DCRX_N_COUNTERS * 4u;
      for (uint32_t nb = ring_batches; nb >= 8u; nb >>= 1)
        if (fixed + nb * 64u * V2_RING_STRIDE * 4u <= 160u * 1024u) { ring_batches_e = nb; scan_lds_e = fixed + nb * 64u * V2_RING_STRIDE * 4u; break; }
      if (!ring_batches_e && eslot && fuse_e_env < 0) eslot->fuse_e = 0;
      if (ring_batches_e) {
        fuse_e = true;
        ks_e = o ? scan2_kernel<UNIFORM, NW, RPL, NARROW, PREFETCH, 1, false, true> : scan2_kernel<UNIFORM, NW, RPL, NARROW, PREFETCH, 0, false, true>;
      }
    }
  }
  if (P.tune && ring_batches) P.tune[o].last_form = 3u;
  const uint32_t scan_lds = v2_scan_lds_bytes(T, o) + (ring_batches ? (T.lds_image_bytes - T.dfa_bytes) + T.v2[o].bk_bytes + ring_batches * 64u * V2_RING_STRIDE * 4u : 0u);
  auto ke = o ? events2_kernel<UNIFORM, NW, 1> : events2_kernel<UNIFORM, NW, 0>;
  auto kt = o ? tail2_kernel<UNIFORM, NW, 1> : tail2_kernel<UNIFORM, NW, 0>;
  auto kr = o ? rescue2_kernel<UNIFORM, NW, 1> : rescue2_kernel<UNIFORM, NW, 0>;
  auto kf = o ? finish2_kernel<UNIFORM, NW, 1> : finish2_kernel<UNIFORM, NW, 0>;
  auto kf0 = o ? finish2_kernel<UNIFORM, NW, 1, false> : finish2_kernel<UNIFORM, NW, 0, false>;
  constexpr bool CAN_SINK = NW == 10;
  auto ks_sink = ks;
  auto kf_sink = kf, kf0_sink = kf0;
  if constexpr (CAN_SINK) {
    kf_sink = o ? finish2_kernel<UNIFORM, NW, 1, true, true> : finish2_kernel<UNIFORM, NW, 0, true, true>;
    kf0_sink = o ? finish2_kernel<UNIFORM, NW, 1, false, true> : finish2_kernel<UNIFORM, NW, 0, false, true>;
    if constexpr (CAN_FUSE) {
      if (ring_batches) ks_sink = o ? scan2_kernel<UNIFORM, NW, RPL, NARROW, PREFETCH, 1, true> : scan2_kernel<UNIFORM, NW, RPL, NARROW, PREFETCH, 0, true>;
    }
  }
  auto kl = o ? left2_kernel<UNIFORM, NW, 1> : left2_kernel<UNIFORM, NW, 0>;
  static bool seen[64];
  hipError_t e;
  if (first_use_on_device(seen)) {
    {
      const void *scans[] = {reinterpret_cast<const void *>(ks), reinterpret_cast<const void *>(ks_sink)};
      for (const void *k : scans) {
        hipFuncAttributes fa;
        e = hipFuncGetAttributes(&fa, k);
        if (e != hipSuccess) return e;
        if (fa.sharedSizeBytes != 0) return hipErrorNotSupported;
      }
    }
    e = hipFuncSetAttribute(reinterpret_cast<const void *>(scan2_kernel<UNIFORM, NW, RPL, NARROW, PREFETCH>), hipFuncAttributeMaxDynamicSharedMemorySize, 160 * 1024);
    if (e != hipSuccess) return e;
    if constexpr (CAN_FUSE_E) {
      const void *ke2[] = {reinterpret_cast<const void *>(scan2_kernel<UNIFORM, NW, RPL, NARROW, PREFETCH, 0, false, true>),
                           reinterpret_cast<const void *>(scan2_kernel<UNIFORM, NW, RPL, NARROW, PREFETCH, 1, false, true>)};
      for (const void *k : ke2) {
        hipFuncAttributes fa;
        e = hipFuncGetAttributes(&fa, k);
        if (e != hipSuccess) return e;
        if (fa.sharedSizeBytes != 0) return hipErrorNotSupported;
        e = hipFuncSetAttribute(k, hipFuncAttributeMaxDynamicSharedMemorySize, 160 * 1024);
        if (e != hipSuccess) return e;
      }
    }
    if constexpr (CAN_FUSE) {
      e = hipFuncSetAttribute(reinterpret_cast<const void *>(scan2_kernel<UNIFORM, NW, RPL, NARROW, PREFETCH, 0>), hipFuncAttributeMaxDynamicSharedMemorySize, 160 * 1024);
      if (e != hipSuccess) return e;
      e = hipFuncSetAttribute(reinterpret_cast<const void *>(scan2_kernel<UNIFORM, NW, RPL, NARROW, PREFETCH, 1>), hipFuncAttributeMaxDynamicSharedMemorySize, 160 * 1024);
      if (e != hipSuccess) return e;
    }
    e = hipFuncSetAttribute(reinterpret_cast<const void *>(kt), hipFuncAttributeMaxDynamicSharedMemorySize, 128 * 1024);
    if (e != hipSuccess) return e;
    e = hipFuncSetAttribute(reinterpret_cast<const void *>(ke), hipFuncAttributeMaxDynamicSharedMemorySize, 64 * 1024);
    if (e != hipSuccess) return e;
    e = hipFuncSetAttribute(reinterpret_cast<const void *>(kr), hipFuncAttributeMaxDynamicSharedMemorySize, 64 * 1024);
    if (e != hipSuccess) return e;
    e = hipFuncSetAttribute(reinterpret_cast<const void *>(kf), hipFuncAttributeMaxDynamicSharedMemorySize, 64 * 1024);
    if (e != hipSuccess) return e;
    e = hipFuncSetAttribute(reinterpret_cast<const void *>(kf0), hipFuncAttributeMaxDynamicSharedMemorySize, 64 * 1024);
    if (e != hipSuccess) return e;
    e = hipFuncSetAttribute(reinterpret_cast<const void *>(kl), hipFuncAttributeMaxDynamicSharedMemorySize, 64 * 1024);
    if (e != hipSuccess) return e;
    if constexpr (CAN_SINK) {
      e = hipFuncSetAttribute(reinterpret_cast<const void *>(kf_sink), hipFuncAttributeMaxDynamicSharedMemorySize, 64 * 1024);
      if (e != hipSuccess) return e;
      e = hipFuncSetAttribute(reinterpret_cast<const void *>(kf0_sink), hipFuncAttributeMaxDynamicSharedMemorySize, 64 * 1024);
      if (e != hipSuccess) return e;
      if constexpr (CAN_FUSE) {
        e = hipFuncSetAttribute(reinterpret_cast<const void *>(scan2_kernel<UNIFORM, NW, RPL, NARROW, PREFETCH, 0, true>), hipFuncAttributeMaxDynamicSharedMemorySize, 160 * 1024);
        if (e != hipSuccess) return e;
        e = hipFuncSetAttribute(reinterpret_cast<const void *>(scan2_kernel<UNIFORM, NW, RPL, NARROW, PREFETCH, 1, true>), hipFuncAttributeMaxDynamicSharedMemorySize, 160 * 1024);
        if (e != hipSuccess) return e;
      }
    }
    attributes_set_on_device(seen);
  }
#ifdef DCRX_SCAN_STAMPS
  {
    static uint32_t *stamps = nullptr;
    if (!stamps) { (void)hipMalloc(&stamps, (size_t)4096 * 16 * 16); (void)hipMemcpyToSymbol(HIP_SYMBOL(g_scan_stamps), &stamps, sizeof(stamps)); }
  }
#endif
  if (B.n_reads == 0) return hipSuccess;
  const uint32_t cus = P.n_cu > P.reserved_cus ? P.n_cu - P.reserved_cus : 1u;
  const uint64_t wt = 64ull * RPL;
  const uint64_t n_items = (B.n_reads + wt - 1) / wt;
  const uint32_t grid = (uint32_t)std::max<uint64_t>(1, std::min<uint64_t>(cus, (n_items + 15) / 16));
  const uint64_t per_block = (((B.n_reads + grid - 1) / grid + 511) / 512) * 512;
  V2Lists Q;
  Q.tail = P.v2_tail; Q.ev = P.v2_events; Q.sx = P.v2_slow; Q.left = P.v2_left; Q.counts = P.v2_counts;
  const uint32_t n_regions = grid;
  const uint64_t pb128 = (per_block + 255) & ~127ull;
  Q.tcap = (uint32_t)std::min<uint64_t>(pb128, P.v2_tail_rows / V2Rows<NW>::T / n_regions) & ~63u;
  Q.ecap = (uint32_t)std::min<uint64_t>(pb128, P.v2_event_rows / V2Rows<NW>::E / n_regions) & ~127u;
  Q.scap = (uint32_t)std::min<uint64_t>(Q.ecap, P.v2_slow_rows / V2Rows<NW>::E / n_regions) & ~127u;
  if (!ring_batches && (!P.v2_tail || Q.tcap < 64)) return B.n_reads ? hipErrorNotReady : hipSuccess;
  if (ring_batches) Q.tcap = (uint32_t)pb128 & ~63u;
  if (Q.ecap < 128 || Q.scap < 128) return hipErrorInvalidValue;
  const bool finish = !(cfg.flags & (DCRX_F_PROFILE_SCAN_ONLY | DCRX_F_PROFILE_NO_FINISH));
  const bool separate = (cfg.flags & (DCRX_F_V2_SIDE_STREAMS | DCRX_F_V2_LEAN_SERIAL | DCRX_F_V2_NO_LEAN_RESCUE)) != 0u;
  const bool side = finish && (cfg.flags & DCRX_F_V2_SIDE_STREAMS) && !(cfg.flags & DCRX_F_V2_LEAN_SERIAL) && P.v2_side && P.v2_side2 && P.v2_ev_fork &&
                    P.v2_ev_join && P.v2_ev_join2;
  const hipEvent_t fork_ev = ev_stop ? ev_stop : P.v2_ev_fork;
  static const uint32_t tail_waves_forced = [] { const char *e = dcrx_debug_env("DCRX_DEBUG_TAIL_WAVES"); const int v = e ? atoi(e) : 0; return (v >= 2 && v <= 8) ? (uint32_t)v : 0u; }();
  V2SinkCall S{};
  if (CAN_SINK && sink && P.sink.dev && finish && !separate && !retry && !(cfg.flags & DCRX_F_PROFILE_MASK)) {
    const uint64_t stride = (uint64_t)Q.tcap + Q.ecap + Q.scap / 2 + pb128;
    if (n_regions <= P.sink.regions_cap && stride * n_regions <= P.sink.items_cap && stride < (1ull << 32) && per_block / 32 * 8 <= 144u * 1024u &&
        per_block < 0xFFFFFFull) {
      S.dev = P.sink.dev; S.items = P.sink.items; S.hits = P.sink.hits; S.stride = (uint32_t)stride; S.e_off = Q.tcap; S.c_off = Q.tcap + Q.ecap; S.late_off = Q.tcap + Q.ecap + Q.scap / 2;
      S.late_cap = (uint32_t)pb128; S.per_block = (uint32_t)per_block; S.wpack = P.sink.wpack;
      sink->S = S; sink->n_regions = n_regions; sink->tcap = Q.tcap; sink->ecap = Q.ecap; sink->ccap = Q.scap / 2; sink->fused = ring_batches ? 1u : 0u;
      sink->counts = Q.counts;
    }
  }
  if (S.dev) fuse_e = false;
  if (P.tune && fuse_e) P.tune[o].last_form = 4u;
  static const uint32_t scan_threads = [] { const char *e = dcrx_debug_env("DCRX_DEBUG_SCAN_THREADS"); const int v = e ? atoi(e) : 0; return (v >= 512 && v <= DCRX_V2_BLOCK && v % 64 == 0) ? (uint32_t)v : (uint32_t)DCRX_V2_BLOCK; }();
  hipExtLaunchKernelGGL(S.dev ? ks_sink : (fuse_e ? ks_e : ks), dim3(grid), dim3(scan_threads), fuse_e ? scan_lds_e : scan_lds, s, ev_start ? ev_start : e_ev_start, side ? fork_ev : ev_stop, 0, T, B, cfg, rec,
                        d_counters, Q, queue, gqueue, qcap, queue_count, per_block, retry, P.dev_tables, fuse_e ? ring_batches_e : ring_batches, S, tail_waves_forced,
                        fuse_e ? rescue_waves_fused : 0u);
  e = hipGetLastError();
  if (e != hipSuccess) return e;
  if constexpr (CAN_FUSE_E) {
    if (eslot && eslot->fuse_e == -1 && !eslot->e_sampling && !fuse_e && fuse_e_env < 0 && !S.dev && finish) {
      bool ok = eslot->h_counts || hipHostMalloc(reinterpret_cast<void **>(&eslot->h_counts), (size_t)4096 * V2_L_COUNTS * 4, hipHostMallocDefault) == hipSuccess;
      ok = ok && (eslot->ev_counts || hipEventCreateWithFlags(&eslot->ev_counts, hipEventDisableTiming) == hipSuccess);
      ok = ok && grid <= 4096u && hipMemcpyAsync(eslot->h_counts, Q.counts, (size_t)grid * V2_L_COUNTS * 4, hipMemcpyDeviceToHost, s) == hipSuccess &&
           hipEventRecord(eslot->ev_counts, s) == hipSuccess;
      if (ok) { eslot->e_sampling = true; eslot->e_regions = grid; eslot->e_reads = B.n_reads; }
      else { (void)hipGetLastError(); eslot->fuse_e = 0; }
    }
  }
  if (finish) {
    static const uint32_t rescue_waves_env = [] { const char *e = dcrx_debug_env("DCRX_DEBUG_RESCUE_WAVES"); const int v = e ? atoi(e) : 0; return v >= 256 ? (uint32_t)v : 0u; }();
    const bool big = B.n_reads >= V2Tune::BIG_BATCH;
    const uint32_t waves_first = (ring_batches && !separate && big) ? 8192u : 4096u, waves_second = (ring_batches && !separate && big) ? 4096u : 3072u;
    uint32_t rescue_waves = rescue_waves_env ? rescue_waves_env : ((ring_batches || separate) ? waves_first : (big ? 4096u : 3072u));
    hipEvent_t tune_start = nullptr, tune_stop = nullptr;
    static const bool tune_off = dcrx_debug_env("DCRX_DEBUG_NO_TUNE") != nullptr;
    const int tune_class = V2Tune::size_class(B.n_reads);
    if (ring_batches && !separate && !rescue_waves_env && !tune_off && P.tune && !retry && !cfg.flags && tune_class >= 0) {
      V2TuneSlot &U = P.tune[o].slot[tune_class];
      if (U.choice) rescue_waves = U.choice;
      else {
        const int k = U.launches - 1;
        if (k >= 0 && k < V2Tune::SAMPLES) {
          if (!U.created) {
            bool ok = true;
            for (int i = 0; i < V2Tune::SAMPLES && ok; i++)
              ok = hipEventCreate(&U.ev[i][0]) == hipSuccess && hipEventCreate(&U.ev[i][1]) == hipSuccess;
            U.created = ok;
            if (!ok) { (void)hipGetLastError(); U.choice = waves_first; }
          }
          if (U.created) { rescue_waves = (k & 1) ? waves_second : waves_first; tune_start = U.ev[k][0]; tune_stop = U.ev[k][1]; }
        } else if (k >= V2Tune::SAMPLES && U.created) {
          if (big && k == V2Tune::SAMPLES && P.tune[o].may_wait) (void)hipEventSynchronize(U.ev[V2Tune::SAMPLES - 1][1]);
          bool ready = true;
          for (int i = 0; i < V2Tune::SAMPLES && ready; i++) ready = hipEventQuery(U.ev[i][1]) == hipSuccess;
          (void)hipGetLastError();
          if (ready) {
            float ms[2] = {0.f, 0.f};
            bool ok = true;
            for (int i = 0; i < V2Tune::SAMPLES && ok; i++) {
              float t = 0.f;
              ok = hipEventElapsedTime(&t, U.ev[i][0], U.ev[i][1]) == hipSuccess;
              ms[i & 1] += t;
            }
            (void)hipGetLastError();
            U.choice = (ok && ms[1] < 0.985f * ms[0]) ? waves_second : waves_first;
            if (ok) { U.us[0] = 1e3f * ms[0] / (V2Tune::SAMPLES / 2); U.us[1] = 1e3f * ms[1] / (V2Tune::SAMPLES / 2); }
            rescue_waves = U.choice;
            static const bool say = dcrx_debug_env("DCRX_DEBUG_TUNE") != nullptr;
            if (say) fprintf(stderr, "dcrx tune: finishing launches of %llu reads, frame %d: %.1f us on %u rescue waves, %.1f on %u -> %u (launch %d)\n",
                             (unsigned long long)B.n_reads, o, 1e3f * ms[0] / (V2Tune::SAMPLES / 2), waves_first, 1e3f * ms[1] / (V2Tune::SAMPLES / 2), waves_second, U.choice, U.launches);
          }
        }
        U.launches++;
      }
    }
    static const uint32_t tail_role_waves_env = [] { const char *e = dcrx_debug_env("DCRX_DEBUG_TAIL_ROLE_WAVES"); const int v = e ? atoi(e) : 0; return v >= 256 ? (uint32_t)v : 0u; }();
    const uint32_t tail_role_waves = tail_role_waves_env ? tail_role_waves_env : (separate ? 8192u : 4096u);
    const uint32_t tsplit = std::max<uint32_t>(1u, std::min<uint32_t>(64u, tail_role_waves / n_regions));
    const uint32_t rsplit_full = std::max<uint32_t>(1u, std::min<uint32_t>(64u, rescue_waves / n_regions));
    const uint32_t rsplit = fuse_e ? 1u : rsplit_full;
    static const uint32_t rescue_waves_c = [] { const char *e = dcrx_debug_env("DCRX_DEBUG_RESCUE_WAVES_C"); const int v = e ? atoi(e) : 0; return v >= 256 ? (uint32_t)v : 0u; }();
    const uint32_t csplit = rescue_waves_c ? std::max<uint32_t>(1u, std::min<uint32_t>(64u, rescue_waves_c / n_regions)) : rsplit_full;
    const uint32_t fgrid = (n_regions * (rsplit + csplit) + DCRX_V2_FBLOCK / 64 - 1) / (DCRX_V2_FBLOCK / 64);
    const uint32_t egrid = (n_regions + DCRX_V2_FBLOCK / 64 - 1) / (DCRX_V2_FBLOCK / 64);
    static const uint32_t bsplit_env = [] { const char *e = dcrx_debug_env("DCRX_DEBUG_X_BSPLIT"); const int v = e ? atoi(e) : 0; return (v >= 1 && v <= 16) ? (uint32_t)v : 0u; }();
    const uint32_t bsplit = bsplit_env ? bsplit_env : (separate ? std::max<uint32_t>(1u, std::min<uint32_t>(16u, 1024u / n_regions)) : (fuse_e ? 2u : 1u));
    const uint32_t sgrid = n_regions * bsplit;
    const uint32_t flds = v2_finish_lds_bytes(T, o);
    const uint32_t llds = v2_finish_block_lds<NW>(T, o, DCRX_V2_FBLOCK);
    const uint32_t tlds = v2_finish_block_lds<NW>(T, o, DCRX_V2_TBLOCK);
    const uint32_t elds_ext = flds + (T.lds_image2_bytes - T.lds_image_bytes);
    const uint32_t ext = elds_ext <= 64u * 1024u ? 1u : 0u;
    const uint32_t elds = ext ? elds_ext : flds;
    const uint32_t slow_width = 4u;
    const uint32_t tgrid = (n_regions * tsplit + DCRX_V2_TBLOCK / 64 - 1) / (DCRX_V2_TBLOCK / 64);
    V2Roles R;
    R.xgrid = sgrid; R.rgrid = fgrid; R.tgrid = ring_batches ? 0u : (n_regions * tsplit + DCRX_V2_FBLOCK / 64 - 1) / (DCRX_V2_FBLOCK / 64);
    R.rsplit = rsplit | (csplit << 8); R.tsplit = tsplit; R.bsplit = bsplit; R.width = slow_width;
    V2FinishArgs A;
    A.T0 = T; A.B = B; A.cfg = cfg; A.records = rec; A.counters = d_counters; A.Q = Q; A.n_regions = n_regions; A.R = R;
    A.queue = queue; A.gqueue = gqueue; A.qcap = qcap; A.queue_count = queue_count; A.Tmem = P.dev_tables; A.S = S;
    if (!separate) {
      hipExtLaunchKernelGGL(S.dev ? (ring_batches ? kf0_sink : kf_sink) : (ring_batches ? kf0 : kf), dim3(R.xgrid + R.rgrid + R.tgrid), dim3(DCRX_V2_FBLOCK), llds, s, tune_start,
                            tune_stop ? tune_stop : e_ev_stop, 0, A);
      e = hipGetLastError();
      if (e != hipSuccess) return e;
    } else {
      auto general = [&](hipStream_t st, const int which, const bool whole_list, hipEvent_t stop) -> hipError_t {
        if (whole_list)
          hipExtLaunchKernelGGL(ke, dim3(egrid), dim3(DCRX_V2_FBLOCK), elds, st, nullptr, stop, 0, T, B, cfg, rec, d_counters, Q, which, (uint32_t)(DCRX_V2_FBLOCK / 64), 64u, 1u, ext,
                                n_regions, queue, gqueue, qcap, queue_count);
        else
          hipExtLaunchKernelGGL(ke, dim3(sgrid), dim3(DCRX_V2_FBLOCK), elds, st, nullptr, stop, 0, T, B, cfg, rec, d_counters, Q, which, 1u, slow_width, bsplit, ext, n_regions, queue,
                                gqueue, qcap, queue_count);
        return hipGetLastError();
      };
      if (side) {
        e = hipStreamWaitEvent(P.v2_side, fork_ev, 0); if (e != hipSuccess) return e;
        hipExtLaunchKernelGGL(kt, dim3(tgrid), dim3(DCRX_V2_TBLOCK), tlds, P.v2_side, nullptr, P.v2_ev_join, 0, T, B, cfg, rec, d_counters, Q, n_regions, tsplit, queue,
                              gqueue, qcap, queue_count, P.dev_tables);
        e = hipGetLastError(); if (e != hipSuccess) return e;
        e = hipStreamWaitEvent(P.v2_side2, fork_ev, 0); if (e != hipSuccess) return e;
        e = general(P.v2_side2, V2_L_X, false, P.v2_ev_join2); if (e != hipSuccess) return e;
      }
      if (cfg.flags & DCRX_F_V2_NO_LEAN_RESCUE) {
        for (int which = V2_L_E; which <= V2_L_C; which++) { e = general(s, which, true, nullptr); if (e != hipSuccess) return e; }
      } else {
        hipLaunchKernelGGL(kr, dim3(fgrid), dim3(DCRX_V2_FBLOCK), llds, s, T, B, cfg, rec, d_counters, Q, n_regions, rsplit | (csplit << 8), queue, gqueue, qcap,
                           queue_count, P.dev_tables);
        e = hipGetLastError();
        if (e != hipSuccess) return e;
      }
      if (side) {
        e = hipStreamWaitEvent(s, P.v2_ev_join, 0); if (e != hipSuccess) return e;
        e = hipStreamWaitEvent(s, P.v2_ev_join2, 0); if (e != hipSuccess) return e;
      } else {
        hipLaunchKernelGGL(kt, dim3(tgrid), dim3(DCRX_V2_TBLOCK), tlds, s, T, B, cfg, rec, d_counters, Q, n_regions, tsplit, queue, gqueue, qcap, queue_count, P.dev_tables);
        e = hipGetLastError();
        if (e != hipSuccess) return e;
        e = general(s, V2_L_X, false, nullptr); if (e != hipSuccess) return e;
      }
      hipLaunchKernelGGL(kl, dim3(1), dim3(DCRX_V2_FBLOCK), llds, s, A);
      e = hipGetLastError(); if (e != hipSuccess) return e;
    }
    static const bool dbg = dcrx_debug_env("DCRX_DEBUG_V2_COUNTS") != nullptr;
    if (dbg && e == hipSuccess) {
      std::vector<uint32_t> h((size_t)V2_L_COUNTS * n_regions);
      (void)hipStreamSynchronize(s);
      (void)hipMemcpy(h.data(), Q.counts, h.size() * 4, hipMemcpyDeviceToHost);
      unsigned long long t[V2_L_COUNTS] = {0};
      for (uint32_t r = 0; r < n_regions; r++) for (int k = 0; k < V2_L_COUNTS; k++) t[k] += h[(size_t)V2_L_COUNTS * r + k];
      fprintf(stderr, "dcrx v2 lists: regions %u tail %llu E %llu C %llu X %llu; LDS of a finishing block %u bytes (side tables %u, buckets %u), of a scan block %u\n", n_regions,
              t[V2_L_TAIL], t[V2_L_E], t[V2_L_C], t[V2_L_X], llds, T.lds_image_bytes - T.dfa_bytes, T.v2[o].bk_bytes, scan_lds);
    }
  }
#ifdef DCRX_SCAN_STAMPS
  {
    static int launches = 0;
    static const int want = [] { const char *e = dcrx_debug_env("DCRX_STAMPS_LAUNCH"); return e ? atoi(e) : 30; }();
    if (launches++ == want && e == hipSuccess) {
      const size_t nw = (size_t)n_regions * (DCRX_V2_BLOCK / 64);
      std::vector<uint32_t> h(4 * nw);
      (void)hipStreamSynchronize(s);
      uint32_t *dptr = nullptr;
      (void)hipMemcpyFromSymbol(&dptr, HIP_SYMBOL(g_scan_stamps), sizeof(dptr));
      (void)hipMemcpy(h.data(), dptr, h.size() * 4, hipMemcpyDeviceToHost);
      if (const char *dump = dcrx_debug_env("DCRX_STAMPS_DUMP")) { FILE *f = fopen(dump, "wb"); if (f) { fwrite(h.data(), 4, h.size(), f); fclose(f); } }
      uint32_t t0 = 0xFFFFFFFFu;
      for (size_t i = 0; i < nw; i++) t0 = std::min(t0, h[4 * i]);
      auto pcs = [&](const char *what, std::vector<double> v) {
        std::sort(v.begin(), v.end());
        auto pc = [&](double q) { return v[(size_t)(q * (v.size() - 1))]; };
        fprintf(stderr, "dcrx scan stamps: %-44s min %6.1f p10 %6.1f p50 %6.1f p90 %6.1f p99 %6.1f max %6.1f us\n", what, pc(0), pc(0.1), pc(0.5), pc(0.9), pc(0.99), pc(1.0));
      };
      std::vector<double> st, su, le_scan, le_tail, en, blk_scan_end, blk_end;
      for (uint32_t r = 0; r < n_regions; r++) {
        double last_scan = 0, last = 0;
        for (int wv = 0; wv < DCRX_V2_BLOCK / 64; wv++) {
          const uint32_t *c = &h[4 * ((size_t)r * (DCRX_V2_BLOCK / 64) + wv)];
          st.push_back((c[0] - t0) / 100.0); su.push_back((c[1] - t0) / 100.0); en.push_back((c[3] - t0) / 100.0);
          const bool tailw = ring_batches && wv >= (DCRX_V2_BLOCK / 64) - 3;
          (tailw ? le_tail : le_scan).push_back((c[2] - t0) / 100.0);
          if (!tailw) last_scan = std::max(last_scan, (c[2] - t0) / 100.0);
          last = std::max(last, (c[3] - t0) / 100.0);
        }
        blk_scan_end.push_back(last_scan); blk_end.push_back(last);
      }
      pcs("wave start", st); pcs("wave set-up done (tables staged)", su); pcs("scanning wave leaves its loop", le_scan);
      if (!le_tail.empty()) pcs("tail wave leaves its loop (last three waves)", le_tail);
      pcs("wave end", en); pcs("per block: last scanning wave leaves", blk_scan_end); pcs("per block: end", blk_end);
    }
  }
#endif
  return e;
}

hipError_t launch_v2_place(const LaunchPlan &P, const V2SinkLaunch &K, uint64_t n_reads, hipStream_t s, hipEvent_t ev_stop) {
  static bool seen[64];
  if (first_use_on_device(seen)) {
    hipError_t e = hipFuncSetAttribute(reinterpret_cast<const void *>(v2_place_kernel), hipFuncAttributeMaxDynamicSharedMemorySize, 150 * 1024);
    if (e != hipSuccess) return e;
    attributes_set_on_device(seen);
  }
  const uint32_t words = (K.S.per_block / 32u) * 2u;
  static const int hcap_forced = [] { const char *e = dcrx_debug_env("DCRX_DEBUG_PLACE_HCAP"); return e ? atoi(e) : -1; }();
  const uint32_t hcap = hcap_forced >= 0 ? ((uint32_t)hcap_forced & ~3u) : (std::min<uint32_t>(K.S.per_block, (150u * 1024u - words * 4u) / 5u) & ~3u);
  const uint32_t lds = words * 4u + hcap * 5u;
  hipExtLaunchKernelGGL(v2_place_kernel, dim3(K.n_regions), dim3(V2_PLACE_BLOCK), lds, s, nullptr, ev_stop, 0, K.S, K.counts, K.n_regions, K.tcap, K.ecap,
                        K.ccap, K.fused, (uint64_t)n_reads, P.sink.n_slots, P.sink.msg, P.sink.bytes - 4u, P.sink.d_total, hcap);
  return hipGetLastError();
}
uint64_t v2_sink_items(uint64_t max_reads, uint32_t n_cu) { return 4 * (max_reads + (uint64_t)n_cu * 1024) + 4096; }

hipError_t launch_v2_any(const LaunchPlan &P, const DevTables &T, const BatchDev &B, const CfgDev &cfg, dcrx_record_t *rec,
                         uint32_t *queue, uint32_t *gqueue, uint32_t qcap, uint32_t *queue_count, unsigned long long *d_counters,
                         hipStream_t s, hipEvent_t ev_start, hipEvent_t ev_stop, uint32_t retry, V2SinkLaunch *sink) {
  const int o = cfg.orientation == DCRX_ORIENT_FORWARD ? 0 : 1;
  const bool uniform = B.lens == nullptr, nw10 = B.stride <= 40, narrow = T.v2[o].narrow != 0;
  int shape = (int)((cfg.flags >> 8) & 3u);
  if (shape == 0) shape = nw10 ? 2 : 3;
#define DCRX_V2A(UN, NW_, RP, NA) launch_v2<UN, NW_, RP, NA>(P, T, B, cfg, rec, queue, gqueue, qcap, queue_count, d_counters, s, ev_start, ev_stop, retry, sink)
#define DCRX_V2X(UN, NW_, RP, NA, PF) launch_v2<UN, NW_, RP, NA, PF>(P, T, B, cfg, rec, queue, gqueue, qcap, queue_count, d_counters, s, ev_start, ev_stop, retry, sink)
#define DCRX_V2(UN, NW_, NA) (shape == 3 ? DCRX_V2A(UN, NW_, 1, NA) : (shape == 1 && UN && NW_ == 10 && NA) ? DCRX_V2X(true, 10, 4, true, false) : DCRX_V2A(UN, NW_, 2, NA))
#ifdef DCRX_FAST_BUILD
  if (nw10 && uniform && shape == 2) return narrow ? DCRX_V2A(true, 10, 2, true) : DCRX_V2A(true, 10, 2, false);
  return hipErrorNotSupported;
#else
  if (nw10) {
    if (uniform) return narrow ? DCRX_V2(true, 10, true) : DCRX_V2(true, 10, false);
    return narrow ? DCRX_V2(false, 10, true) : DCRX_V2(false, 10, false);
  }
  if (B.stride <= 4 * DCRX_NWMAX) {
    if (uniform) return narrow ? DCRX_V2(true, DCRX_NWMAX, true) : DCRX_V2(true, DCRX_NWMAX, false);
    return narrow ? DCRX_V2(false, DCRX_NWMAX, true) : DCRX_V2(false, DCRX_NWMAX, false);
  }
  if (uniform) return narrow ? DCRX_V2X(true, DCRX_V2_NWLONG, 1, true, false) : DCRX_V2X(true, DCRX_V2_NWLONG, 1, false, false);
  return narrow ? DCRX_V2X(false, DCRX_V2_NWLONG, 1, true, false) : DCRX_V2X(false, DCRX_V2_NWLONG, 1, false, false);
#endif
#undef DCRX_V2
#undef DCRX_V2A
#undef DCRX_V2X
}

void v2_list_rows(uint64_t max_reads, uint32_t stride, uint32_t n_cu, uint64_t *tail_rows, uint64_t *event_rows) {
  const uint64_t rt = stride <= 40 ? V2Rows<10>::T : stride <= 4 * DCRX_NWMAX ? V2Rows<DCRX_NWMAX>::T : V2Rows<DCRX_V2_NWLONG>::T;
  const uint64_t re = stride <= 40 ? V2Rows<10>::E : stride <= 4 * DCRX_NWMAX ? V2Rows<DCRX_NWMAX>::E : V2Rows<DCRX_V2_NWLONG>::E;
  const uint64_t entries = max_reads + max_reads / 8 + (uint64_t)n_cu * 16 * 256;
  *tail_rows = entries * rt;
  *event_rows = (entries / 2) * re;
}
uint64_t v2_slow_rows(uint64_t max_reads, uint32_t stride, uint32_t n_cu) {
  uint64_t tr, er;
  v2_list_rows(max_reads, stride, n_cu, &tr, &er);
  return er;
}

}
```

decombinator_amd/csrc/dcrx_v2_device.h:

```cpp
#pragma once

#include "dcrx_dcr_device.h"

namespace dcrx {

#ifndef DCRX_HOST_EMUL
DCRX_DEV uint32_t dcrx_alignbit(uint32_t hi, uint32_t lo, uint32_t sh) { return __builtin_amdgcn_alignbit(hi, lo, sh); }
typedef __attribute__((address_space(3))) uint16_t dcrx_lds_u16;
struct V2Tab {};
DCRX_DEV uint32_t v2_entry(const V2Tab &, uint32_t byte_off) {
  return *reinterpret_cast<const dcrx_lds_u16 *>(static_cast<uintptr_t>(byte_off));
}
#else
inline uint32_t dcrx_alignbit(uint32_t hi, uint32_t lo, uint32_t sh) { return (uint32_t)((((uint64_t)hi << 32) | lo) >> (sh & 31)); }
struct V2Tab { const uint16_t *base; };
inline uint32_t v2_entry(const V2Tab &tab, uint32_t byte_off) { return tab.base[byte_off >> 1]; }
#endif

#ifndef DCRX_HOST_EMUL
typedef uint32_t dcrx_ldsaddr;
template <typename T>
DCRX_DEV T dcrx_lds_at(dcrx_ldsaddr a, uint32_t i) {
  return reinterpret_cast<const __attribute__((address_space(3))) T *>(static_cast<uintptr_t>(a))[i];
}
// ... 680 lines not shown
}

template <int NW>
DCRX_DEV uint64_t reg_stored64(const uint32_t (&w)[NW], const int s) {
  const int i = s >> 4, sh = (s & 15) * 2;
  uint32_t w0 = 0, w1 = 0, w2 = 0;
#pragma unroll
  for (int k = 0; k < NW; k++) {
    const bool at = i == k;
    w0 = at ? w[k] : w0;
    if (k + 1 < NW) w1 = at ? w[k + 1] : w1;
    if (k + 2 < NW) w2 = at ? w[k + 2] : w2;
  }
  return (uint64_t)dcrx_funnel_r(w0, w1, sh) | ((uint64_t)dcrx_funnel_r(w1, w2, sh) << 32);
}

template <int NW>
struct RegWords {
  const uint32_t (&w)[NW];
  DCRX_DEV uint64_t stored64(const int s) const { return reg_stored64<NW>(w, s); }
};
struct LdsWords {
  dcrx_ldsaddr strip;
  DCRX_DEV uint64_t stored64(const int s) const {
    const uint32_t i = (uint32_t)s >> 4;
    const int sh = (s & 15) * 2;
    const uint32_t w0 = dcrx_lds_at<uint32_t>(strip, i), w1 = dcrx_lds_at<uint32_t>(strip, i + 1), w2 = dcrx_lds_at<uint32_t>(strip, i + 2);
    return (uint64_t)dcrx_funnel_r(w0, w1, sh) | ((uint64_t)dcrx_funnel_r(w1, w2, sh) << 32);
  }
};
template <int NW>
constexpr int lds_words_stride() { return ((NW + 2) | 1); }

template <bool REV_, class WS>
struct FrameWS {
  static constexpr bool kRev = REV_;
  static constexpr bool kWindowedWalks = true;
  const WS &w;
  int len;
  DCRX_DEV int n() const { return len; }
  DCRX_DEV bool has_exc() const { return false; }
  DCRX_DEV bool clean(int, int) const { return true; }
  DCRX_DEV uint64_t exc_slots(int) const { return 0ull; }
  DCRX_DEV bool has_N(int, int) const { return false; }
  DCRX_DEV uint64_t load64(int b) const { return w.stored64(b); }
  DCRX_DEV uint32_t window(int a, int l) const {
    const int lo = REV_ ? len - a - l : a;
    const uint32_t v = (uint32_t)w.stored64(lo);
    return v & ((l >= 16) ? 0xFFFFFFFFu : ((1u << (2 * l)) - 1u));
  }
  DCRX_DEV int code(int i) const {
    const int m = REV_ ? len - 1 - i : i;
    const int c = (int)(w.stored64(m) & 3ull);
    return REV_ ? (c ^ 3) : c;
  }
  DCRX_DEV uint8_t chr(int i) const { return (uint8_t)("ACGT"[code(i)]); }
};

template <bool REV, class WS>
DCRX_DEV int tail2_fast(const Tail2Tabs &tt, const WS &w, const int n, const uint32_t digest, const CfgDev &cfg,
                        dcrx_record_t &rec, const DevTables &T, const Counters &C) {
  const int vpair = (int)(digest & 0xFFu), jpair = (int)((digest >> 8) & 0xFFu), jc = (int)((digest >> 16) & 3u);
  const int Lv = (int)tt.L[0], Lj = (int)tt.L[1];
  bool slow = n < 32 || Lv > 31 || Lj > 31;
  const int top = max(n, 32) - 32;
  const int sva = 2 * vpair - Lv + 1;
  const int wsv = min(max(sva, 0), top);
  const uint64_t Wv = w.stored64(wsv);
  const int sja = 2 * jpair - Lj + 1;
  const int wsj = min(max(sja, 0), top);
  const uint64_t Wj = w.stored64(wsj);
  const uint64_t mv = (1ull << (2 * (Lv & 31))) - 1ull, mj = (1ull << (2 * (Lj & 31))) - 1ull;
  int v, sv, j = 0, sj = 0;
  {
    const LookupQ q[4] = {
        {tt.bk_mask[0], tt.bk_tag[0], tt.bk_pk[0], (Wv >> v2_sh(sva - wsv)) & mv, sva >= 0},
        {tt.bk_mask[0], tt.bk_tag[0], tt.bk_pk[0], (Wv >> v2_sh(sva + 1 - wsv)) & mv, sva + 1 + Lv <= n},
        {tt.bk_mask[1], tt.bk_tag[1], tt.bk_pk[1], (Wj >> v2_sh(sja - wsj)) & mj, jc == 1 && sja >= 0},
        {tt.bk_mask[1], tt.bk_tag[1], tt.bk_pk[1], (Wj >> v2_sh(sja + 1 - wsj)) & mj, jc == 1 && sja + 1 + Lj <= n}};
    int t[4];
    lookup_lockstep<4>(q, t);
    slow |= (t[0] >= 0) == (t[1] >= 0);
    v = max(t[0] >= 0 ? t[0] : t[1], 0); sv = t[0] >= 0 ? sva : sva + 1;
    slow |= jc == 1 && (t[2] >= 0) == (t[3] >= 0);
    j = max(t[2] >= 0 ? t[2] : t[3], 0); sj = t[2] >= 0 ? sja : sja + 1;
  }
  const int jumpv = dcrx_lds_at<int32_t>(tt.jump[0], (uint32_t)v);
  const int vp = REV ? n - sv - Lv : sv;
  const int te = vp + jumpv - 1;
  const int fv = te + 1;
  const bool vedge = !(fv >= 32 && fv < n) || !dcrx_lds_at<uint8_t>(tt.w64_ok[0], (uint32_t)v);
  const uint64_t rwv = w.stored64(min(max(REV ? n - fv : fv - 32, 0), top));
  const int jumpj = dcrx_lds_at<int32_t>(tt.jump[1], (uint32_t)j);
  const int jp = REV ? n - sj - Lj : sj;
  const int ts = jp - jumpj;
  const bool jedge = !(ts >= 0 && ts + 32 <= n) || !dcrx_lds_at<uint8_t>(tt.w64_ok[1], (uint32_t)j);
  const uint64_t rwj = w.stored64(min(max(REV ? n - ts - 32 : ts, 0), top));
  if (slow) return TAIL2_SLOW;
  const uint64_t yv = mismatch_slots(rwv, dcrx_lds_at<uint64_t>(tt.w64[0], (uint32_t)v));
  int kv = REV ? first_clean_up(or10_up(yv), 0) : first_clean_down(or10_down(yv), 0);
  if (vedge) kv = -1;
  int end_v = te - kv;
  if (kv < 0) {
    const FrameWS<REV, WS> F{w, n};
    if (!get_v_deletions(T.g[0], F, v, te, end_v, kv, C)) return te >= n ? DCRX_S_V_WALK_FAIL_AT_END : DCRX_S_V_WALK_FAIL;
  }
  const int end_of_v = end_v + 1;
  const int k0 = end_of_v > ts ? end_of_v - ts : 0;
  const uint64_t yj = mismatch_slots(rwj, dcrx_lds_at<uint64_t>(tt.w64[1], (uint32_t)j));
  int kj = REV ? first_clean_down(or10_down(yj), k0) : first_clean_up(or10_up(yj), k0);
  if (jedge) kj = -1;
  int start_j = ts + kj;
  if (jc == 1 && kj < 0) {
    const FrameWS<REV, WS> F{w, n};
    if (!get_j_deletions(T.g[1], F, j, ts, end_of_v, start_j, kj, C)) return DCRX_S_J_WALK_FAIL;
  }
  const int jend = jp + Lj;
  int status = DCRX_S_OK;
  if (vp + Lv > jend + Lj) status = DCRX_S_F_OVERLAP;
  if (kv > jumpv - Lv || kj > jumpj) status = DCRX_S_F_IMPOSS_DEL;
  if ((vp - jend) >= cfg.lenthreshold) status = DCRX_S_F_TOOLONG;
  if (jc == 2) status = DCRX_S_J_MULTI;
  if (jc == 0) status = DCRX_S_J_NONE;
  int lo, hi;
  pyslice(n, end_v + 1, start_j, lo, hi);
  const bool ok = status == DCRX_S_OK;
  rec.v = (uint16_t)(ok ? v : 0); rec.j = (uint16_t)(ok ? j : 0);
  rec.v_start = (uint16_t)(ok ? vp : 0); rec.j_end = (uint16_t)(ok ? jend : 0);
  rec.ins_start = (uint16_t)(ok ? lo : 0); rec.ins_len = (uint16_t)(ok ? hi - lo : 0);
  rec.vdel = (uint8_t)(ok ? kv : 0); rec.jdel = (uint8_t)(ok ? kj : 0);
  return status;
}

DCRX_DEV void tail2_count(const Counters &C, const int status, const bool forward) {
  C.add(DCRX_C_READ_COUNT);
  if (status == DCRX_S_OK) { C.add(DCRX_C_VJ_COUNT); if (forward) C.add(DCRX_C_FRAME_FORWARD); return; }
  if (status == DCRX_S_J_NONE) { C.add(DCRX_C_NO_J_ASSIGNED); C.add(DCRX_C_VJ_ASSIGNMENT_FAILED); }
  else if (status == DCRX_S_J_MULTI) { C.add(DCRX_C_MULTIPLE_J_MATCHES); C.add(DCRX_C_VJ_ASSIGNMENT_FAILED); }
  else if (status == DCRX_S_J_WALK_FAIL) C.add(DCRX_C_VJ_ASSIGNMENT_FAILED);
  else if (status == DCRX_S_F_TOOLONG) C.add(DCRX_C_DCRFILTER_TOOLONG_INTERTAG);
  else if (status == DCRX_S_F_IMPOSS_DEL) C.add(DCRX_C_DCRFILTER_IMPOSS_DELETION);
  else if (status == DCRX_S_F_OVERLAP) C.add(DCRX_C_DCRFILTER_TAG_OVERLAP);
}

struct Rescue2Tabs {
  Tail2Tabs t;
  uint32_t h_mask[2][2];
  dcrx_ldsaddr h_kw[2][2], h_pk[2][2];
  dcrx_ldsaddr kw_begin, kw_tags;
  dcrx_ldsaddr tag_pk[2];
  uint32_t kw_base[2][2];
  uint32_t Lh[2][2];
  int32_t split[2];
};

DCRX_DEV Rescue2Tabs rescue2_tabs(const DevTables &T0, const V2Ori &V0, const uint8_t *side, const uint8_t *bk, const bool rev,
                                  const uint32_t (&kw_base)[K_NCLASS]) {
  Rescue2Tabs r;
  r.t = tail2_tabs(T0, V0, side, bk, rev);
  auto at_side = [&](const void *p) { return dcrx_ldsaddr_of(side + ((reinterpret_cast<const uint8_t *>(p) - T0.image) - T0.dfa_bytes)); };
  for (int g = 0; g < 2; g++) {
    for (int h = 0; h < 2; h++) {
      const int cls = g == 0 ? (h == 0 ? K_VH1 : K_VH2) : (h == 0 ? K_JH1 : K_JH2);
      r.h_mask[g][h] = V0.bk_mask[cls];
      r.h_kw[g][h] = dcrx_ldsaddr_of(bk + V0.bk_kw_off[cls]);
      r.h_pk[g][h] = dcrx_ldsaddr_of(bk + V0.bk_pk_off[cls]);
      r.kw_base[g][h] = kw_base[cls];
      r.Lh[g][h] = T0.kw_len[cls];
    }
    r.tag_pk[g] = at_side(rev ? T0.g[g].tag_pk_rc : T0.g[g].tag_pk_fwd);
    r.split[g] = T0.g[g].split;
  }
  r.kw_begin = at_side(T0.kw_begin);
  r.kw_tags = at_side(T0.kw_tags);
  return r;
}

constexpr int RESCUE2_SLOW = -1;
#if defined(DCRX_HOST_EMUL) && defined(DCRX_R2_PROFILE)
void r2_prof(int what, int a);
#define R2P(what, a) r2_prof(what, a)
#else
#define R2P(what, a) ((void)0)
#endif
#ifdef DCRX_R2_REASONS
extern unsigned long long g_r2_reasons[32];
#define R2S(k) (g_r2_reasons[k]++, RESCUE2_SLOW)
#else
#define R2S(k) RESCUE2_SLOW
#endif

template <int G>
struct GeneOf {
  const Rescue2Tabs &rt;
  bool j;
  DCRX_DEV uint32_t h_mask(int h) const { return G >= 0 ? rt.h_mask[G < 0 ? 0 : G][h] : (j ? rt.h_mask[1][h] : rt.h_mask[0][h]); }
  DCRX_DEV dcrx_ldsaddr h_kw(int h) const { return G >= 0 ? rt.h_kw[G < 0 ? 0 : G][h] : (j ? rt.h_kw[1][h] : rt.h_kw[0][h]); }
  DCRX_DEV dcrx_ldsaddr h_pk(int h) const { return G >= 0 ? rt.h_pk[G < 0 ? 0 : G][h] : (j ? rt.h_pk[1][h] : rt.h_pk[0][h]); }
  DCRX_DEV uint32_t kw_base(int h) const { return G >= 0 ? rt.kw_base[G < 0 ? 0 : G][h] : (j ? rt.kw_base[1][h] : rt.kw_base[0][h]); }
  DCRX_DEV int Lh(int h) const { return (int)(G >= 0 ? rt.Lh[G < 0 ? 0 : G][h] : (j ? rt.Lh[1][h] : rt.Lh[0][h])); }
  DCRX_DEV dcrx_ldsaddr tag_pk() const { return G >= 0 ? rt.tag_pk[G < 0 ? 0 : G] : (j ? rt.tag_pk[1] : rt.tag_pk[0]); }
  DCRX_DEV int Lt() const { return (int)(G >= 0 ? rt.t.L[G < 0 ? 0 : G] : (j ? rt.t.L[1] : rt.t.L[0])); }
  DCRX_DEV int split() const { return G >= 0 ? rt.split[G < 0 ? 0 : G] : (j ? rt.split[1] : rt.split[0]); }
  DCRX_DEV uint32_t fbit() const { return G >= 0 ? (G == 0 ? V2_F_VH : V2_F_JH) : (j ? V2_F_JH : V2_F_VH); }
};

template <bool REV, class WS, int G>
DCRX_DEV int rescue2_candidates(const GeneOf<G> &g, const WS &w, const int n, const int half, const uint32_t gk,
                                const int p, int &k_out, int &q_out) {
  const Rescue2Tabs &rt = g.rt;
  const int L = g.Lt();
  const int q = half == 1 ? p : p - g.split();
  if (q + L < 0) return R2S(1);
  if (q < 0 || q + L > n) return 0;
  const int b = REV ? n - q - L : q;
  const int ws = min(b, n - 32);
  const uint64_t mask = (1ull << (2 * L)) - 1ull;
  const uint64_t val = (w.stored64(ws) >> (2 * (b - ws))) & mask;
  const uint32_t x0 = dcrx_lds_at<uint32_t>(rt.kw_begin, gk), x1 = dcrx_lds_at<uint32_t>(rt.kw_begin, gk + 1);
  const dcrx_ldsaddr tpk = g.tag_pk();
  int found = 0;
  for (uint32_t x = x0; x < x1 && !found; x++) {
    R2P(5, half);
    const int k = (int)dcrx_lds_at<uint32_t>(rt.kw_tags, x);
    const uint64_t y = mismatch_slots(val, dcrx_lds_at<uint64_t>(tpk, (uint32_t)k)) & mask;
    if (dcrx_popc64(y) <= 1) { found = 1; k_out = k; q_out = q; }
  }
  return found;
}

template <int NW>
DCRX_DEV uint32_t log_word(const uint32_t (&lg)[NW], const int kk) {
  uint32_t l = 0;
#pragma unroll
  for (int k = 0; k < NW; k++) l = (kk == k) ? lg[k] : l;
  return l;
}

template <bool REV, int NW, class WS, int G>
DCRX_DEV int rescue2_half(const GeneOf<G> &g, const WS &w, const uint32_t (&lg)[NW], const int n,
                          int &k_out, int &q_out, int &p_out, int &half_out) {
  const int L1 = g.Lh(0), L2 = g.Lh(1);
  const uint64_t m1 = (1ull << (2 * L1)) - 1ull, m2 = (1ull << (2 * L2)) - 1ull;
  const uint32_t mask8 = g.fbit() * 0x11111111u;
  uint32_t nz = 0;
#pragma unroll
  for (int kk = 0; kk < NW; kk++) nz |= (lg[kk] & mask8) ? (1u << kk) : 0u;
  uint64_t h2lo = 0, h2hi = 0;
  int h2n = 0;
  bool any1 = false;
  int res = 0;
  R2P(1, G);
  while (nz && res == 0) {
    R2P(2, 0);
    const int kk = REV ? 31 - dcrx_clz32(nz) : dcrx_ctz32(nz);
    nz &= ~(1u << kk);
    uint32_t m = log_word<NW>(lg, kk) & mask8;
    while (m && res == 0) {
      R2P(3, 0);
      const int bit = REV ? 31 - dcrx_clz32(m) : dcrx_ctz32(m);
      m &= ~(1u << bit);
      const int pair = 8 * kk + (bit >> 2);
      const int f1 = 2 * pair + 1;
      const int xs = f1 >= 31 ? f1 - 31 : 0;
      const uint64_t X = w.stored64(xs);
      for (int y = 0; y < 2 && res == 0; y++) {
        const int f = REV ? f1 - y : f1 - 1 + y;
        if (f >= n) continue;
        R2P(4, y);
        const int s1 = f - L1 + 1, s2 = f - L2 + 1;
        const LookupQ q[2] = {{g.h_mask(0), g.h_kw(0), g.h_pk(0), (X >> v2_sh(s1 - xs)) & m1, s1 >= 0},
                              {g.h_mask(1), g.h_kw(1), g.h_pk(1), (X >> v2_sh(s2 - xs)) & m2, s2 >= 0}};
        int kw[2];
        lookup_lockstep<2>(q, kw);
        const int kw1 = kw[0], kw2 = kw[1];
        if (kw2 >= 0) {
          const uint64_t e = ((uint64_t)(uint32_t)(kw2 + 1) << 16) | (uint64_t)(uint32_t)f;
          if (h2n < 2) h2lo |= e << (32 * h2n); else if (h2n < 4) h2hi |= e << (32 * (h2n - 2));
          h2n++;
        }
        if (kw1 >= 0) {
          R2P(8, 0);
          any1 = true;
          const int p = REV ? n - s1 - L1 : s1;
          res = rescue2_candidates<REV, WS, G>(g, w, n, 1, g.kw_base(0) + (uint32_t)kw1, p, k_out, q_out);
          p_out = p;
        }
      }
    }
  }
  half_out = 1;
  if (res != 0 || any1) return res;
  if (h2n > 4) return R2S(13);
  half_out = h2n ? 2 : 0;
  for (int i = 0; i < h2n && res == 0; i++) {
    R2P(6, 0);
    const uint32_t e = (uint32_t)((i < 2 ? h2lo : h2hi) >> (32 * (i & 1)));
    const int f = (int)(e & 0xFFFFu), kw2 = (int)(e >> 16) - 1;
    const int s2 = f - L2 + 1;
    const int p = REV ? n - s2 - L2 : s2;
    res = rescue2_candidates<REV, WS, G>(g, w, n, 2, g.kw_base(1) + (uint32_t)kw2, p, k_out, q_out);
    p_out = p;
  }
  return res;
}

enum { V2_SHAPE_ANY = -1, V2_SHAPE_ONE = 0, V2_SHAPE_BOTH = 1 };
DCRX_DEV int shape2(const uint32_t vf_n, const uint32_t jf_n, const uint32_t any) {
  return (vf_n == 0u && jf_n == 0u && (any & V2_F_JH)) ? V2_SHAPE_BOTH : V2_SHAPE_ONE;
}

constexpr uint32_t RESCUE2_NO_DIGEST = 0xFFFFFFFFu;
DCRX_DEV uint32_t rescue2_digest_pack(const Digest2 &d) {
  return min(d.vf_n, 3u) | (min(d.jf_n, 3u) << 2) | ((d.any & 0xFu) << 4) | ((d.vf_pair & 0xFFu) << 8) | ((d.jf_pair & 0xFFu) << 16);
}
template <bool REV, int NW, int SHAPE, class WS, class OnOk>
DCRX_DEV int rescue2_fast_to(const Rescue2Tabs &rt, const WS &w, const uint32_t (&lg)[NW], const int n, const CfgDev &cfg,
                             OnOk &&on_ok, uint32_t &errs, const DevTables &T, const Counters &C, const Counters &Cdry,
                             const uint32_t dg = RESCUE2_NO_DIGEST) {
  const Tail2Tabs &tt = rt.t;
  const int Lv = (int)tt.L[0], Lj = (int)tt.L[1];
  errs = 0;
  if (n < 32 || Lv > 31 || Lj > 31) return R2S(2);
  uint32_t vfn = 0, jfn = 0, any = 0, vf1 = 0xFFFFFFFFu, jf1 = 0xFFFFFFFFu;
  if (dg != RESCUE2_NO_DIGEST) {
    vfn = dg & 3u; jfn = (dg >> 2) & 3u; any = (dg >> 4) & 0xFu;
    vf1 = ((dg >> 8) & 0xFFu) << 2; jf1 = ((dg >> 16) & 0xFFu) << 2;
  } else {
#pragma unroll
    for (int kk = 0; kk < NW; kk++) {
      const uint32_t l = lg[kk];
      any |= l;
      if (SHAPE != V2_SHAPE_BOTH) {
        const uint32_t tv = l & 0x11111111u, tj = l & 0x22222222u;
        const uint32_t kb = (uint32_t)kk << 5;
        vfn += (uint32_t)dcrx_popc64(tv);
        vf1 = min(vf1, (tv ? (uint32_t)dcrx_ctz32(tv) : 0xFFFFFFFFu) | kb);
        jfn += (uint32_t)dcrx_popc64(tj);
        jf1 = min(jf1, (tj ? (uint32_t)dcrx_ctz32(tj) : 0xFFFFFFFFu) | kb);
      }
    }
    any |= any >> 16; any |= any >> 8; any |= any >> 4; any &= 0xFu;
  }
  if ((n & 1) && log_nibble<NW>(lg, n >> 1)) return R2S(3);
  if (vfn > 1 || (vfn == 0 && !(any & V2_F_VH))) return R2S(4);
  const bool vfull = vfn == 1;
  const bool jsweep = jfn == 0 && (any & V2_F_JH) != 0u;
  if (SHAPE == V2_SHAPE_ONE && vfull != jsweep) return R2S(4);
  if (SHAPE == V2_SHAPE_BOTH && (vfull || !jsweep)) return R2S(4);
  const uint64_t mv = (1ull << (2 * Lv)) - 1ull, mj = (1ull << (2 * Lj)) - 1ull;

  int ftag = -1, fs = 0;
  const bool jfull = !vfull && jfn == 1;
  if (SHAPE != V2_SHAPE_BOTH && (vfull || jfull)) {
    const int Lf = vfull ? Lv : Lj;
    const uint64_t mf = vfull ? mv : mj;
// ... 135 lines not shown
```

Before: 33180.

## Move per-gene rescue table parameters into LDS rows and split rescue kernel by list role

Per-gene rescue parameters (hash masks, keyword/pack addresses, bases, lengths, split), previously selected from registers with a runtime j-select, are now written once into a small LDS table. They are read back by row index when the gene is not known at compile time. This is meant to cut register pressure and select instructions in the rescue paths. The rescue kernel also now takes a single kernarg struct and dispatches blocks to separate E-list and C-list role functions. The cost is extra LDS reads on the hot path, more LDS per block, and a larger code reorganisation.

```diff
diff --git a/decombinator_amd/csrc/dcrx_kernels_v2.hip b/decombinator_amd/csrc/dcrx_kernels_v2.hip
--- a/decombinator_amd/csrc/dcrx_kernels_v2.hip
+++ b/decombinator_amd/csrc/dcrx_kernels_v2.hip
@@ -291,6 +291,26 @@
 #endif
 constexpr float V2_FUSE_E_MAX_SHARE = 0.25f;
 
+template <class T>
+__device__ __forceinline__ T *v2_global(T *p) {
+  return (T *)(__attribute__((address_space(1))) T *)(uintptr_t)p;
+}
+template <class T>
+__device__ __forceinline__ T *v2_constant(T *p) { return (T *)(__attribute__((address_space(4))) T *)(uintptr_t)p; }
+
+__device__ __forceinline__ void v2_gene_rows(Rescue2Tabs &rt, const DevTables *__restrict__ Tmem, const uint32_t *side, const uint32_t *bk, const bool rev, uint32_t *rows,
+                                             const int lane) {
+  if (lane == 0) {
+    const DevTables &T = *Tmem;
+    uint32_t kw_base[K_NCLASS];
+#pragma unroll
+    for (int c = 0; c < K_NCLASS; c++) kw_base[c] = v2_constant(T.kw_base)[c];
+    const Rescue2Tabs r = rescue2_tabs(T, T.v2[rev ? 1 : 0], reinterpret_cast<const uint8_t *>(side), reinterpret_cast<const uint8_t *>(bk), rev, kw_base);
+    rescue2_gene_rows(r, rows);
+  }
+  rt.gene_rows = dcrx_ldsaddr_of(rows);
+}
+
 template <bool UNIFORM_LEN, int NW, int RPL, bool NARROW, bool PREFETCH = true, int FUSE = -1, bool SINK = false, bool FUSE_E = false>
 __global__ __launch_bounds__(DCRX_V2_BLOCK) void scan2_kernel(
     DevTables T0, BatchDev B, CfgDev cfg, dcrx_record_t *__restrict__ records, unsigned long long *__restrict__ counters,
@@ -325,6 +345,7 @@
   constexpr uint32_t ES = (uint32_t)v2_ering_stride<NW>(), ering_mask = 64u * V2_ERING_BATCHES - 1u;
   uint32_t *ring2 = ring + (size_t)(ring_mask + 1u) * V2_RING_STRIDE;
   uint32_t *lds_dry = ring2 + (size_t)(ering_mask + 1u) * ES;
+  uint32_t *lds_genes = lds_dry + DCRX_N_COUNTERS;
   if (FUSE >= 0) {
     {
       const uint4 *s1 = reinterpret_cast<const uint4 *>(T0.image + T0.dfa_bytes), *s2 = reinterpret_cast<const uint4 *>(V0.bk);
@@ -616,7 +637,8 @@
     uint32_t kw_base[K_NCLASS];
 #pragma unroll
     for (int c = 0; c < K_NCLASS; c++) kw_base[c] = T0.kw_base[c];
-    const Rescue2Tabs rt = rescue2_tabs(T0, V0, reinterpret_cast<const uint8_t *>(lds_side), reinterpret_cast<const uint8_t *>(lds_bk), REV, kw_base);
+    Rescue2Tabs rt = rescue2_tabs(T0, V0, reinterpret_cast<const uint8_t *>(lds_side), reinterpret_cast<const uint8_t *>(lds_bk), REV, kw_base);
+    v2_gene_rows(rt, Tmem, lds_side, lds_bk, REV, lds_genes, lane);
     const Counters C{lds_counts}, Cdry{lds_dry};
     constexpr uint32_t nb_mask = V2_ERING_BATCHES - 1u, nb_shift = (uint32_t)__builtin_ctz(V2_ERING_BATCHES);
     constexpr uint32_t V2_RING_EXIT = 0xFFFFFFFFu;
@@ -837,6 +859,7 @@
 constexpr int V2_LEFT_SLOTS = 15;
 struct V2FinishLds {
   uint32_t *counts, *side, *bk, *strip, *dry, *left;
+  uint32_t *genes;
 };
 template <int NW, int BLOCK>
 __device__ __forceinline__ V2FinishLds v2_finish_layout(const DevTables &T0, const V2Ori &V, uint32_t *smem, const int tid) {
@@ -847,6 +870,7 @@
   L.strip = L.bk + V.bk_bytes / 4 + (uint32_t)tid * lds_words_stride<NW>();
   L.dry = L.bk + V.bk_bytes / 4 + (uint32_t)BLOCK * lds_words_stride<NW>();
   L.left = L.dry + DCRX_N_COUNTERS + (uint32_t)(tid >> 6) * (1 + V2_LEFT_SLOTS);
+  L.genes = L.dry + DCRX_N_COUNTERS + (uint32_t)(BLOCK / 64) * (1 + V2_LEFT_SLOTS);
   return L;
 }
 template <int NW, int BLOCK>
@@ -862,199 +886,18 @@
 template <int NW>
 static uint32_t v2_finish_block_lds(const DevTables &T, int o, int block) {
   return DCRX_N_COUNTERS * 4 + (T.lds_image_bytes - T.dfa_bytes) + T.v2[o].bk_bytes + (uint32_t)block * lds_words_stride<NW>() * 4 + DCRX_N_COUNTERS * 4 +
-         (uint32_t)(block / 64) * (1 + V2_LEFT_SLOTS) * 4;
-}
-
-__device__ __forceinline__ void v2_note_left(uint32_t *left, const uint32_t slot, const BatchDev &B, uint32_t *__restrict__ queue, uint32_t *__restrict__ gqueue,
-                                             const uint32_t qcap, uint32_t *__restrict__ queue_count, const uint32_t r, const bool exc) {
-  const uint32_t at = atomicAdd(&left[0], 1u);
-  if (at < (uint32_t)V2_LEFT_SLOTS) left[1 + at] = slot;
-  else v2_hand_over(B, queue, gqueue, qcap, queue_count, B.n_reads < (1ull << 30), r, exc);
-}
-template <int NW>
-struct V2EntryWords { uint32_t lg[NW], w[NW]; };
-template <bool UNIFORM_LEN, int NW, int ORI>
-__device__ __forceinline__ void v2_tail_jobs(const Tail2Tabs &tt, const V2FinishLds &L, const BatchDev &B, const CfgDev &cfg, dcrx_record_t *__restrict__ records,
-                                             const V2Lists &Q, const uint32_t n_regions, const uint32_t split, uint32_t *__restrict__ queue,
-                                             uint32_t *__restrict__ gqueue, const uint32_t qcap, uint32_t *__restrict__ queue_count,
-                                             const DevTables *__restrict__ Tmem, const uint32_t gwave, const uint32_t n_gwaves, const int tid, const V2SinkCall &S) {
-  constexpr int o = ORI;
-  const Counters C{L.counts};
-  const LdsWords lw{dcrx_ldsaddr_of(L.strip)};
-  uint32_t *strip = L.strip, *lds_counts = L.counts;
-  uint32_t *s_left = L.left;
-  const int lane = tid & 63;
-  for (uint32_t job = gwave; job < n_regions * split; job += n_gwaves) {
-    const uint32_t region = job / split, part = job % split;
-    const uint32_t tn = Q.counts[V2_L_COUNTS * region + V2_L_TAIL];
-    const uint4 *tq = Q.tail + (size_t)region * Q.tcap * V2Rows<NW>::T;
-    const uint32_t STEP = 64 * split;
-    constexpr bool AHEAD = NW <= DCRX_NWMAX;
-    uint32_t x1[2 + NW];
-    if constexpr (AHEAD) v2_get_rows<2 + NW>(tq, Q.tcap, 64 * part + lane, 64 * part + lane < tn, x1);
-    for (uint32_t first = 64 * part; first < tn && !(cfg.flags & DCRX_F_PROFILE_NO_TAIL); first += STEP) {
-      uint32_t x[2 + NW];
-      if constexpr (AHEAD) {
-#pragma unroll
-        for (int k = 0; k < 2 + NW; k++) x[k] = x1[k];
-        const uint32_t nf = v2_landed(x, first + STEP);
-        v2_get_rows<2 + NW>(tq, Q.tcap, nf + lane, nf + lane < tn, x1);
-      } else {
-        v2_get_rows<2 + NW>(tq, Q.tcap, first + lane, first + lane < tn, x);
-      }
-      uint32_t w[NW];
-#pragma unroll
-      for (int k = 0; k < NW; k++) w[k] = x[2 + k];
-      int status = -2;
-      uint64_t tup = 0;
-      const uint32_t r = x[0], dg = x[1];
-      if (first + lane < tn) {
-        const int n = UNIFORM_LEN ? (int)B.read_len : (int)B.lens[r];
-        dcrx_record_t rec;
-        rec.v = rec.j = rec.v_start = rec.j_end = rec.ins_start = rec.ins_len = 0; rec.vdel = rec.jdel = 0;
-#if DCRX_LEAN_LDS_WORDS
-#pragma unroll
-        for (int k = 0; k < NW; k++) strip[k] = w[k];
-        if (cfg.flags & DCRX_F_PROFILE_TAIL_STREAM_ONLY) { status = DCRX_S_J_NONE; rec.v = (uint16_t)(w[0] ^ w[NW - 1]); }
-        else
-        status = tail2_fast<ORI == 1>(tt, lw, n, dg, cfg, rec, *Tmem, C);
-#else
-        const RegWords<NW> rw{w};
-        status = tail2_fast<ORI == 1>(tt, rw, n, dg, cfg, rec, *Tmem, C);
-#endif
-        if (status >= 0) { rec.status = (uint8_t)status; rec.frame = (uint8_t)(o ? 0 : 1); DCRX_STORE_FINISH(records + r, rec); }
-        if (S.dev && status == DCRX_S_OK) tup = sink_tuple_lean(rec, S.wpack, false);
-      }
-      v2_tally(lds_counts, lane, status, o == 0);
-      if (S.dev) sink_put(S, region, 0u, first + (uint32_t)lane, first + lane < tn, status == DCRX_S_OK, r, tup, lane, nullptr);
-      if (__builtin_expect(status == TAIL2_SLOW, 0)) v2_note_left(s_left, first + (uint32_t)lane, B, queue, gqueue, qcap, queue_count, r, false);
-    }
-    const uint32_t n_left = min(s_left[0], (uint32_t)V2_LEFT_SLOTS);
-    if (__builtin_expect(n_left != 0u, 0)) {
-      const bool live = (uint32_t)lane < n_left;
-      const uint32_t slot = live ? s_left[1 + lane] : 0u;
-      uint32_t x[2 + NW];
-      v2_get_rows<2 + NW>(tq, Q.tcap, slot, live, x);
-      if (live) {
-        const uint32_t dg = x[1], vp = dg & 0xFFu, jp = (dg >> 8) & 0xFFu, jc = (dg >> 16) & 3u;
-        V2EntryWords<NW> e;
-#pragma unroll
-        for (int k = 0; k < NW; k++) {
-          uint32_t l = (vp >> 3) == (uint32_t)k ? (V2_F_VF << (4 * (vp & 7u))) : 0u;
-          if (jc == 1u && (jp >> 3) == (uint32_t)k) l |= V2_F_JF << (4 * (jp & 7u));
-          e.lg[k] = l; e.w[k] = x[2 + k];
-        }
-        if (!v2_left_push<NW>(Q.left, queue_count, x[0] | (jc == 2u ? V2_R_JMULTI : 0u), e.lg, e.w)) v2_hand_over(B, queue, gqueue, qcap, queue_count, B.n_reads < (1ull << 30), x[0], false);
-      }
-      if (lane == 0) s_left[0] = 0u;
-    }
-  }
-}
-
-template <bool UNIFORM_LEN, int NW, int ORI>
-__device__ __forceinline__ void v2_rescue_jobs(const Rescue2Tabs &rt, const V2FinishLds &L, const BatchDev &B, const CfgDev &cfg, dcrx_record_t *__restrict__ records,
-                                               const V2Lists &Q, const uint32_t n_regions, const uint32_t split_ec, uint32_t *__restrict__ queue,
-                                               uint32_t *__restrict__ gqueue, const uint32_t qcap, uint32_t *__restrict__ queue_count,
-                                               const DevTables *__restrict__ Tmem, const uint32_t gwave, const uint32_t n_gwaves, const int tid, const V2SinkCall &S,
-                                               uint32_t *__restrict__ tickets) {
-  constexpr int o = ORI;
-  const Counters C{L.counts}, Cdry{L.dry};
-  const LdsWords lw{dcrx_ldsaddr_of(L.strip)};
-  uint32_t *strip = L.strip, *lds_counts = L.counts;
-  uint32_t *s_left = L.left;
-  const int lane = tid & 63;
-  const uint32_t split_e = split_ec & 255u, split_c = (split_ec >> 8) ? (split_ec >> 8) : split_e;
-  for (uint32_t job = gwave; job < n_regions * (split_e + split_c) && !(cfg.flags & DCRX_F_PROFILE_NO_EVENTS); job += n_gwaves) {
-    const int which = job < n_regions * split_e ? V2_L_E : V2_L_C;
-    const uint32_t split = which == V2_L_E ? split_e : split_c, jrel = which == V2_L_E ? job : job - n_regions * split_e;
-    const uint32_t region = jrel / split, part = jrel % split;
-    const V2ListRef l = v2_list<NW>(Q, which, region);
-    const uint32_t en = min(Q.counts[V2_L_COUNTS * region + which], l.cap);
-    auto draw = [&]() -> uint32_t {
-      uint32_t t = 0;
-      if (lane == 0) t = __hip_atomic_fetch_add(tickets + V2_L_COUNTS * region + V2_L_TICKETS, which == V2_L_E ? 1u : 0x10000u, __ATOMIC_RELAXED, __HIP_MEMORY_SCOPE_AGENT);
-      t = (uint32_t)__builtin_amdgcn_readfirstlane((int)t);
-      return split + (which == V2_L_E ? (t & 0xFFFFu) : (t >> 16));
-    };
-    constexpr bool AHEAD = NW <= 10;
-    uint32_t x1[2 + 2 * NW];
-    uint32_t first = 64 * part, next_first = 64 * part + 64 * en + 64;
-    if (first < en) next_first = 64 * draw();
-    if constexpr (AHEAD) v2_get_rows<2 + 2 * NW>(l.rows, l.cap, first + lane, first + lane < en, x1);
-    for (; first < en; ) {
-      uint32_t x[2 + 2 * NW];
-      const bool more = next_first < en;
-      uint32_t after_raw = 0;
-      uint32_t nf = next_first;
-      if constexpr (AHEAD) {
-#pragma unroll
-        for (int k = 0; k < 2 + 2 * NW; k++) x[k] = x1[k];
-        nf = v2_landed(x, next_first);
-      }
-      if (more && lane == 0) after_raw = __hip_atomic_fetch_add(tickets + V2_L_COUNTS * region + V2_L_TICKETS, which == V2_L_E ? 1u : 0x10000u, __ATOMIC_RELAXED, __HIP_MEMORY_SCOPE_AGENT);
-      if constexpr (AHEAD) {
-        v2_get_rows<2 + 2 * NW>(l.rows, l.cap, nf + lane, nf + lane < en, x1);
-      } else {
-        v2_get_rows<2 + 2 * NW>(l.rows, l.cap, first + lane, first + lane < en, x);
-      }
-      uint32_t lg[NW], w[NW];
-#pragma unroll
-      for (int k = 0; k < NW; k++) { lg[k] = x[1 + k]; w[k] = x[1 + NW + k]; }
-      int status = -2;
-      uint32_t errs = 0;
-      uint64_t tup = 0;
-      const uint32_t r = x[0] & V2_R_MASK;
-      if (first + lane < en) {
-        status = RESCUE2_SLOW;
-        if (!(x[0] & V2_R_EXC)) {
-          const int n = UNIFORM_LEN ? (int)B.read_len : (int)B.lens[r];
-#pragma unroll
-          for (int k = 0; k < NW; k++) strip[k] = w[k];
-          auto on_ok = [&](dcrx_record_t rec, const uint32_t e) {
-            rec.frame = (uint8_t)(o ? 0 : 1);
-            DCRX_STORE_FINISH(records + r, rec);
-            if (S.dev) tup = sink_tuple_lean(rec, S.wpack, (e & 8u) != 0u && 2 * rt.split[1] != (int)rt.t.L[1]);
-          };
-          if (which == V2_L_E) status = rescue2_fast_to<ORI == 1, NW, V2_SHAPE_ONE>(rt, lw, lg, n, cfg, on_ok, errs, *Tmem, C, Cdry, x[1 + 2 * NW]);
-          else status = rescue2_fast_to<ORI == 1, NW, V2_SHAPE_BOTH>(rt, lw, lg, n, cfg, on_ok, errs, *Tmem, C, Cdry, x[1 + 2 * NW]);
-          if (status > 0) {
-            dcrx_record_t rec;
-            rec.v = rec.j = rec.v_start = rec.j_end = rec.ins_start = rec.ins_len = 0; rec.vdel = rec.jdel = 0;
-            rec.status = (uint8_t)status; rec.frame = (uint8_t)(o ? 0 : 1);
-            DCRX_STORE_FINISH(records + r, rec);
-          } else if (status < 0) errs = 0;
-        }
-      }
-      v2_tally_rescue(lds_counts, lane, status, errs, o == 0);
-      if (S.dev) sink_put(S, region, which == V2_L_E ? S.e_off : S.c_off, first + (uint32_t)lane, first + lane < en, status == DCRX_S_OK, r, tup, lane, nullptr);
-      if (__builtin_expect(status == RESCUE2_SLOW, 0)) v2_note_left(s_left, first + (uint32_t)lane, B, queue, gqueue, qcap, queue_count, r, (x[0] & V2_R_EXC) != 0u);
-      first = next_first;
-      if (more) {
-        const uint32_t t = (uint32_t)__builtin_amdgcn_readfirstlane((int)after_raw);
-        next_first = 64u * (split + (which == V2_L_E ? (t & 0xFFFFu) : (t >> 16)));
-      }
-    }
-    const uint32_t n_left = min(s_left[0], (uint32_t)V2_LEFT_SLOTS);
-    if (__builtin_expect(n_left != 0u, 0)) {
-      const bool live = (uint32_t)lane < n_left;
-      const uint32_t slot = live ? s_left[1 + lane] : 0u;
-      uint32_t x[1 + 2 * NW];
-      v2_get_rows<1 + 2 * NW>(l.rows, l.cap, slot, live, x);
-      if (live) {
-        V2EntryWords<NW> e;
-#pragma unroll
-        for (int k = 0; k < NW; k++) { e.lg[k] = x[1 + k]; e.w[k] = x[1 + NW + k]; }
-        if (!v2_left_push<NW>(Q.left, queue_count, x[0], e.lg, e.w)) v2_hand_over(B, queue, gqueue, qcap, queue_count, B.n_reads < (1ull << 30), x[0] & V2_R_MASK, (x[0] & V2_R_EXC) != 0u);
-      }
-      if (lane == 0) s_left[0] = 0u;
-    }
-  }
-}
-
-template <bool UNIFORM_LEN, int NW, int ORI, bool SINK>
-DCRX_V2_ROLE void v2_general_role(const uint32_t mode_, const uint32_t vblock_, const uint32_t ka_lo, const uint32_t ka_hi);
+         (uint32_t)(block / 64) * (1 + V2_LEFT_SLOTS) * 4 + 2 * R2G_ROW * 4;
+}
 
 struct V2Roles { uint32_t xgrid, rgrid, tgrid, rsplit, tsplit, bsplit, width; };
+struct V2RescueSplit { uint32_t split_e, split_c, e_blocks, c_blocks; };
+__host__ __device__ __forceinline__ V2RescueSplit v2_rescue_split(const uint32_t n_regions, const uint32_t split_ec) {
+  constexpr uint32_t WPB = DCRX_V2_FBLOCK / 64;
+  V2RescueSplit s;
+  s.split_e = split_ec & 255u; s.split_c = (split_ec >> 8) ? (split_ec >> 8) : s.split_e;
+  s.e_blocks = (n_regions * s.split_e + WPB - 1) / WPB; s.c_blocks = (n_regions * s.split_c + WPB - 1) / WPB;
+  return s;
+}
 struct V2FinishArgs {
   DevTables T0; BatchDev B; CfgDev cfg; dcrx_record_t *records; unsigned long long *counters; V2Lists Q; uint32_t n_regions; V2Roles R;
   uint32_t *queue, *gqueue; uint32_t qcap; uint32_t *queue_count; const DevTables *Tmem; V2SinkCall S;
@@ -1069,12 +912,6 @@
   for (size_t i = 0; i < sizeof(T) / 4; i++) d[i] = base[offset / 4 + i];
   return out;
 }
-template <class T>
-__device__ __forceinline__ T *v2_global(T *p) {
-  return (T *)(__attribute__((address_space(1))) T *)(uintptr_t)p;
-}
-template <class T>
-__device__ __forceinline__ T *v2_constant(T *p) { return (T *)(__attribute__((address_space(4))) T *)(uintptr_t)p; }
 struct V2FinishLocals {
   DevTables T0; BatchDev B; CfgDev cfg; dcrx_record_t *records; V2Lists Q; uint32_t n_regions; V2Roles R;
   uint32_t *queue, *gqueue; uint32_t qcap; uint32_t *queue_count; const DevTables *Tmem; V2SinkCall S;
@@ -1103,7 +940,198 @@
   A.S.items = v2_global(A.S.items); A.S.hits = v2_global(A.S.hits);
   return A;
 }
+__device__ __forceinline__ void v2_note_left(uint32_t *left, const uint32_t slot, const BatchDev &B, uint32_t *__restrict__ queue, uint32_t *__restrict__ gqueue,
+                                             const uint32_t qcap, uint32_t *__restrict__ queue_count, const uint32_t r, const bool exc) {
+  const uint32_t at = atomicAdd(&left[0], 1u);
+  if (at < (uint32_t)V2_LEFT_SLOTS) left[1 + at] = slot;
+  else v2_hand_over(B, queue, gqueue, qcap, queue_count, B.n_reads < (1ull << 30), r, exc);
+}
+template <int NW>
+struct V2EntryWords { uint32_t lg[NW], w[NW]; };
+template <bool UNIFORM_LEN, int NW, int ORI>
+__device__ __forceinline__ void v2_tail_jobs(const Tail2Tabs &tt, const V2FinishLds &L, const BatchDev &B, const CfgDev &cfg, dcrx_record_t *__restrict__ records,
+                                             const V2Lists &Q, const uint32_t n_regions, const uint32_t split, uint32_t *__restrict__ queue,
+                                             uint32_t *__restrict__ gqueue, const uint32_t qcap, uint32_t *__restrict__ queue_count,
+                                             const DevTables *__restrict__ Tmem, const uint32_t gwave, const uint32_t n_gwaves, const int tid, const V2SinkCall &S) {
+  constexpr int o = ORI;
+  const Counters C{L.counts};
+  const LdsWords lw{dcrx_ldsaddr_of(L.strip)};
+  uint32_t *strip = L.strip, *lds_counts = L.counts;
+  uint32_t *s_left = L.left;
+  const int lane = tid & 63;
+  for (uint32_t job = gwave; job < n_regions * split; job += n_gwaves) {
+    const uint32_t region = job / split, part = job % split;
+    const uint32_t tn = Q.counts[V2_L_COUNTS * region + V2_L_TAIL];
+    const uint4 *tq = Q.tail + (size_t)region * Q.tcap * V2Rows<NW>::T;
+    const uint32_t STEP = 64 * split;
+    constexpr bool AHEAD = NW <= DCRX_NWMAX;
+    uint32_t x1[2 + NW];
+    if constexpr (AHEAD) v2_get_rows<2 + NW>(tq, Q.tcap, 64 * part + lane, 64 * part + lane < tn, x1);
+    for (uint32_t first = 64 * part; first < tn && !(cfg.flags & DCRX_F_PROFILE_NO_TAIL); first += STEP) {
+      uint32_t x[2 + NW];
+      if constexpr (AHEAD) {
+#pragma unroll
+        for (int k = 0; k < 2 + NW; k++) x[k] = x1[k];
+        const uint32_t nf = v2_landed(x, first + STEP);
+        v2_get_rows<2 + NW>(tq, Q.tcap, nf + lane, nf + lane < tn, x1);
+      } else {
+        v2_get_rows<2 + NW>(tq, Q.tcap, first + lane, first + lane < tn, x);
+      }
+      uint32_t w[NW];
+#pragma unroll
+      for (int k = 0; k < NW; k++) w[k] = x[2 + k];
+      int status = -2;
+      uint64_t tup = 0;
+      const uint32_t r = x[0], dg = x[1];
+      if (first + lane < tn) {
+        const int n = UNIFORM_LEN ? (int)B.read_len : (int)B.lens[r];
+        dcrx_record_t rec;
+        rec.v = rec.j = rec.v_start = rec.j_end = rec.ins_start = rec.ins_len = 0; rec.vdel = rec.jdel = 0;
+#if DCRX_LEAN_LDS_WORDS
+#pragma unroll
+        for (int k = 0; k < NW; k++) strip[k] = w[k];
+        if (cfg.flags & DCRX_F_PROFILE_TAIL_STREAM_ONLY) { status = DCRX_S_J_NONE; rec.v = (uint16_t)(w[0] ^ w[NW - 1]); }
+        else
+        status = tail2_fast<ORI == 1>(tt, lw, n, dg, cfg, rec, *Tmem, C);
+#else
+        const RegWords<NW> rw{w};
+        status = tail2_fast<ORI == 1>(tt, rw, n, dg, cfg, rec, *Tmem, C);
+#endif
+        if (status >= 0) { rec.status = (uint8_t)status; rec.frame = (uint8_t)(o ? 0 : 1); DCRX_STORE_FINISH(records + r, rec); }
+        if (S.dev && status == DCRX_S_OK) tup = sink_tuple_lean(rec, S.wpack, false);
+      }
+      v2_tally(lds_counts, lane, status, o == 0);
+      if (S.dev) sink_put(S, region, 0u, first + (uint32_t)lane, first + lane < tn, status == DCRX_S_OK, r, tup, lane, nullptr);
+      if (__builtin_expect(status == TAIL2_SLOW, 0)) v2_note_left(s_left, first + (uint32_t)lane, B, queue, gqueue, qcap, queue_count, r, false);
+    }
+    const uint32_t n_left = min(s_left[0], (uint32_t)V2_LEFT_SLOTS);
+    if (__builtin_expect(n_left != 0u, 0)) {
+      const bool live = (uint32_t)lane < n_left;
+      const uint32_t slot = live ? s_left[1 + lane] : 0u;
+      uint32_t x[2 + NW];
+      v2_get_rows<2 + NW>(tq, Q.tcap, slot, live, x);
+      if (live) {
+        const uint32_t dg = x[1], vp = dg & 0xFFu, jp = (dg >> 8) & 0xFFu, jc = (dg >> 16) & 3u;
+        V2EntryWords<NW> e;
+#pragma unroll
+        for (int k = 0; k < NW; k++) {
+          uint32_t l = (vp >> 3) == (uint32_t)k ? (V2_F_VF << (4 * (vp & 7u))) : 0u;
+          if (jc == 1u && (jp >> 3) == (uint32_t)k) l |= V2_F_JF << (4 * (jp & 7u));
+          e.lg[k] = l; e.w[k] = x[2 + k];
+        }
+        if (!v2_left_push<NW>(Q.left, queue_count, x[0] | (jc == 2u ? V2_R_JMULTI : 0u), e.lg, e.w)) v2_hand_over(B, queue, gqueue, qcap, queue_count, B.n_reads < (1ull << 30), x[0], false);
+      }
+      if (lane == 0) s_left[0] = 0u;
+    }
+  }
+}
+
+template <bool UNIFORM_LEN, int NW, int ORI, int WHICH>
+__device__ __forceinline__ void v2_rescue_jobs(const Rescue2Tabs &rt, const V2FinishLds &L, const BatchDev &B, const CfgDev &cfg, dcrx_record_t *__restrict__ records,
+                                               const V2Lists &Q, const uint32_t n_regions, const uint32_t split, const uint32_t ka_lo, const uint32_t ka_hi,
+                                               const DevTables *__restrict__ Tmem, const uint32_t gwave, const uint32_t n_gwaves, const int tid, const V2SinkCall &S,
+                                               uint32_t *__restrict__ tickets) {
+  static_assert(WHICH == V2_L_E || WHICH == V2_L_C, "the lean rescue takes list E or list C");
+  constexpr int o = ORI, which = WHICH;
+  constexpr int SHAPE = WHICH == V2_L_E ? V2_SHAPE_ONE : V2_SHAPE_BOTH;
+  const Counters C{L.counts}, Cdry{L.dry};
+  const LdsWords lw{dcrx_ldsaddr_of(L.strip)};
+  uint32_t *strip = L.strip, *lds_counts = L.counts;
+  uint32_t *s_left = L.left;
+  const int lane = tid & 63;
+  for (uint32_t job = gwave; job < n_regions * split && !(cfg.flags & DCRX_F_PROFILE_NO_EVENTS); job += n_gwaves) {
+    const uint32_t region = job / split, part = job % split;
+    const V2ListRef l = v2_list<NW>(Q, which, region);
+    const uint32_t en = min(Q.counts[V2_L_COUNTS * region + which], l.cap);
+    auto draw = [&]() -> uint32_t {
+      uint32_t t = 0;
+      if (lane == 0) t = __hip_atomic_fetch_add(tickets + V2_L_COUNTS * region + V2_L_TICKETS, which == V2_L_E ? 1u : 0x10000u, __ATOMIC_RELAXED, __HIP_MEMORY_SCOPE_AGENT);
+      t = (uint32_t)__builtin_amdgcn_readfirstlane((int)t);
+      return split + (which == V2_L_E ? (t & 0xFFFFu) : (t >> 16));
+    };
+    constexpr bool AHEAD = NW <= 10;
+    uint32_t x1[2 + 2 * NW];
+    uint32_t first = 64 * part, next_first = 64 * part + 64 * en + 64;
+    if (first < en) next_first = 64 * draw();
+    if constexpr (AHEAD) v2_get_rows<2 + 2 * NW>(l.rows, l.cap, first + lane, first + lane < en, x1);
+    for (; first < en; ) {
+      uint32_t x[2 + 2 * NW];
+      const bool more = next_first < en;
+      uint32_t after_raw = 0;
+      uint32_t nf = next_first;
+      if constexpr (AHEAD) {
+#pragma unroll
+        for (int k = 0; k < 2 + 2 * NW; k++) x[k] = x1[k];
+        nf = v2_landed(x, next_first);
+      }
+      if (more && lane == 0) after_raw = __hip_atomic_fetch_add(tickets + V2_L_COUNTS * region + V2_L_TICKETS, which == V2_L_E ? 1u : 0x10000u, __ATOMIC_RELAXED, __HIP_MEMORY_SCOPE_AGENT);
+      if constexpr (AHEAD) {
+        v2_get_rows<2 + 2 * NW>(l.rows, l.cap, nf + lane, nf + lane < en, x1);
+      } else {
+        v2_get_rows<2 + 2 * NW>(l.rows, l.cap, first + lane, first + lane < en, x);
+      }
+      uint32_t lg[NW], w[NW];
+#pragma unroll
+      for (int k = 0; k < NW; k++) { lg[k] = x[1 + k]; w[k] = x[1 + NW + k]; }
+      int status = -2;
+      uint32_t errs = 0;
+      uint64_t tup = 0;
+      const uint32_t r = x[0] & V2_R_MASK;
+      if (first + lane < en) {
+        status = RESCUE2_SLOW;
+        if (!(x[0] & V2_R_EXC)) {
+          const int n = UNIFORM_LEN ? (int)B.read_len : (int)B.lens[r];
+#pragma unroll
+          for (int k = 0; k < NW; k++) strip[k] = w[k];
+          auto on_ok = [&](dcrx_record_t rec, const uint32_t e) {
+            rec.frame = (uint8_t)(o ? 0 : 1);
+            DCRX_STORE_FINISH(records + r, rec);
+            if (S.dev) tup = sink_tuple_lean(rec, S.wpack, (e & 8u) != 0u && 2 * rt.split[1] != (int)rt.t.L[1]);
+          };
+          status = rescue2_fast_to<ORI == 1, NW, SHAPE>(rt, lw, lg, n, cfg, on_ok, errs, *Tmem, C, Cdry, x[1 + 2 * NW]);
+          if (status > 0) {
+            dcrx_record_t rec;
+            rec.v = rec.j = rec.v_start = rec.j_end = rec.ins_start = rec.ins_len = 0; rec.vdel = rec.jdel = 0;
+            rec.status = (uint8_t)status; rec.frame = (uint8_t)(o ? 0 : 1);
+            DCRX_STORE_FINISH(records + r, rec);
+          } else if (status < 0) errs = 0;
+        }
+      }
+      v2_tally_rescue(lds_counts, lane, status, errs, o == 0);
+      if (S.dev) sink_put(S, region, which == V2_L_E ? S.e_off : S.c_off, first + (uint32_t)lane, first + lane < en, status == DCRX_S_OK, r, tup, lane, nullptr);
+      if (__builtin_expect(status == RESCUE2_SLOW, 0)) {
+        const V2FinishLocals R = v2_finish_args(ka_lo, ka_hi);
+        v2_note_left(s_left, first + (uint32_t)lane, R.B, R.queue, R.gqueue, R.qcap, R.queue_count, r, (x[0] & V2_R_EXC) != 0u);
+      }
+      first = next_first;
+      if (more) {
+        const uint32_t t = (uint32_t)__builtin_amdgcn_readfirstlane((int)after_raw);
+        next_first = 64u * (split + (which == V2_L_E ? (t & 0xFFFFu) : (t >> 16)));
+      }
+    }
+    const uint32_t n_left = min(s_left[0], (uint32_t)V2_LEFT_SLOTS);
+    if (__builtin_expect(n_left != 0u, 0)) {
+      const bool live = (uint32_t)lane < n_left;
+      const uint32_t slot = live ? s_left[1 + lane] : 0u;
+      uint32_t x[1 + 2 * NW];
+      v2_get_rows<1 + 2 * NW>(l.rows, l.cap, slot, live, x);
+      if (live) {
+        V2EntryWords<NW> e;
+#pragma unroll
+        for (int k = 0; k < NW; k++) { e.lg[k] = x[1 + k]; e.w[k] = x[1 + NW + k]; }
+        const V2FinishLocals R = v2_finish_args(ka_lo, ka_hi);
+        if (!v2_left_push<NW>(R.Q.left, R.queue_count, x[0], e.lg, e.w))
+          v2_hand_over(R.B, R.queue, R.gqueue, R.qcap, R.queue_count, R.B.n_reads < (1ull << 30), x[0] & V2_R_MASK, (x[0] & V2_R_EXC) != 0u);
+      }
+      if (lane == 0) s_left[0] = 0u;
+    }
+  }
+}
+
 template <bool UNIFORM_LEN, int NW, int ORI, bool SINK>
+DCRX_V2_ROLE void v2_general_role(const uint32_t mode_, const uint32_t vblock_, const uint32_t ka_lo, const uint32_t ka_hi);
+
+template <bool UNIFORM_LEN, int NW, int ORI, bool SINK, int WHICH>
 DCRX_V2_ROLE void v2_rescue_role(const uint32_t vblock_, const uint32_t ka_lo, const uint32_t ka_hi) {
   extern __shared__ __align__(64) uint32_t smem[];
   V2FinishLocals A = v2_finish_args(ka_lo, ka_hi);
@@ -1115,10 +1143,12 @@
   uint32_t kw_base[K_NCLASS];
 #pragma unroll
   for (int c = 0; c < K_NCLASS; c++) kw_base[c] = A.T0.kw_base[c];
-  const Rescue2Tabs rt = rescue2_tabs(A.T0, V, reinterpret_cast<const uint8_t *>(L.side), reinterpret_cast<const uint8_t *>(L.bk), ORI == 1, kw_base);
+  Rescue2Tabs rt = rescue2_tabs(A.T0, V, reinterpret_cast<const uint8_t *>(L.side), reinterpret_cast<const uint8_t *>(L.bk), ORI == 1, kw_base);
+  v2_gene_rows(rt, A.Tmem, L.side, L.bk, ORI == 1, L.genes, tid & 63);
   constexpr uint32_t WPB = DCRX_V2_FBLOCK / 64;
-  v2_rescue_jobs<UNIFORM_LEN, NW, ORI>(rt, L, A.B, A.cfg, A.records, A.Q, A.n_regions, A.R.rsplit, A.queue, A.gqueue, A.qcap, A.queue_count, A.Tmem,
-                                       vblock * WPB + (uint32_t)(tid >> 6), A.R.rgrid * WPB, tid, A.S, A.tickets);
+  const V2RescueSplit rs = v2_rescue_split(A.n_regions, A.R.rsplit);
+  v2_rescue_jobs<UNIFORM_LEN, NW, ORI, WHICH>(rt, L, A.B, A.cfg, A.records, A.Q, A.n_regions, WHICH == V2_L_E ? rs.split_e : rs.split_c, ka_lo, ka_hi,
+                                              A.Tmem, vblock * WPB + (uint32_t)(tid >> 6), (WHICH == V2_L_E ? rs.e_blocks : rs.c_blocks) * WPB, tid, A.S, A.tickets);
 }
 template <bool UNIFORM_LEN, int NW, int ORI, bool SINK>
 DCRX_V2_ROLE void v2_tail_role(const uint32_t vblock_, const uint32_t ka_lo, const uint32_t ka_hi) {
@@ -1222,6 +1252,10 @@
     const uint32_t paired = 2u * min(R.rgrid, R.tgrid);
     if (b < paired) { role = (b & 1u) ? 2 : 1; b >>= 1; }
     else { b -= paired; role = R.rgrid > R.tgrid ? 1 : 2; b += min(R.rgrid, R.tgrid); }
+    if (role == 1) {
+      const uint32_t e_blocks = v2_rescue_split(A.n_regions, R.rsplit).e_blocks;
+      if (b >= e_blocks) { role = 3; b -= e_blocks; }
+    }
   }
   const V2Ori V = A.T0.v2[ORI];
   V2FinishLds L = v2_finish_layout<NW, DCRX_V2_FBLOCK>(A.T0, V, smem, tid);
@@ -1229,7 +1263,8 @@
   if (staged) {
     L = v2_finish_stage<NW, DCRX_V2_FBLOCK>(A.T0, V, smem, tid);
     __syncthreads();
-    if (role == 1) v2_rescue_role<UNIFORM_LEN, NW, ORI, SINK>(b, (uint32_t)ka, (uint32_t)(ka >> 32));
+    if (role == 1) v2_rescue_role<UNIFORM_LEN, NW, ORI, SINK, V2_L_E>(b, (uint32_t)ka, (uint32_t)(ka >> 32));
+    else if (role == 3) v2_rescue_role<UNIFORM_LEN, NW, ORI, SINK, V2_L_C>(b, (uint32_t)ka, (uint32_t)(ka >> 32));
     else if (TAIL_ROLE && role == 2) v2_tail_role<UNIFORM_LEN, NW, ORI, SINK>(b, (uint32_t)ka, (uint32_t)(ka >> 32));
     else v2_general_role<UNIFORM_LEN, NW, ORI, SINK>(blockIdx.x == 0 ? 3u : 1u, b, (uint32_t)ka, (uint32_t)(ka >> 32));
   }
@@ -1273,23 +1308,18 @@
 }
 
 template <bool UNIFORM_LEN, int NW, int ORI>
-__global__ __launch_bounds__(DCRX_V2_FBLOCK, DCRX_V2_RWAVES) void rescue2_kernel(
-    DevTables T0, BatchDev B, CfgDev cfg, dcrx_record_t *__restrict__ records, unsigned long long *__restrict__ counters,
-    V2Lists Q, uint32_t n_regions, uint32_t split, uint32_t *__restrict__ queue, uint32_t *__restrict__ gqueue, uint32_t qcap,
-    uint32_t *__restrict__ queue_count, const DevTables *__restrict__ Tmem) {
+__global__ __launch_bounds__(DCRX_V2_FBLOCK, DCRX_V2_RWAVES) void rescue2_kernel(const V2FinishArgs A) {
   extern __shared__ __align__(64) uint32_t smem[];
   const int tid = threadIdx.x;
-  const V2Ori V = T0.v2[ORI];
-  const V2FinishLds L = v2_finish_stage<NW, DCRX_V2_FBLOCK>(T0, V, smem, tid);
-  uint32_t kw_base[K_NCLASS];
-#pragma unroll
-  for (int c = 0; c < K_NCLASS; c++) kw_base[c] = T0.kw_base[c];
-  const Rescue2Tabs rt = rescue2_tabs(T0, V, reinterpret_cast<const uint8_t *>(L.side), reinterpret_cast<const uint8_t *>(L.bk), ORI == 1, kw_base);
+  const uint64_t ka = (uint64_t)__builtin_amdgcn_kernarg_segment_ptr();
+  const V2Ori V = A.T0.v2[ORI];
+  const V2FinishLds L = v2_finish_stage<NW, DCRX_V2_FBLOCK>(A.T0, V, smem, tid);
   __syncthreads();
-  v2_rescue_jobs<UNIFORM_LEN, NW, ORI>(rt, L, B, cfg, records, Q, n_regions, split, queue, gqueue, qcap, queue_count, Tmem,
-                                       blockIdx.x * (DCRX_V2_FBLOCK / 64) + (uint32_t)(tid >> 6), gridDim.x * (DCRX_V2_FBLOCK / 64), tid, V2SinkCall{}, Q.counts);
+  const uint32_t e_blocks = v2_rescue_split(A.n_regions, A.R.rsplit).e_blocks;
+  if (blockIdx.x < e_blocks) v2_rescue_role<UNIFORM_LEN, NW, ORI, false, V2_L_E>(blockIdx.x, (uint32_t)ka, (uint32_t)(ka >> 32));
+  else v2_rescue_role<UNIFORM_LEN, NW, ORI, false, V2_L_C>(blockIdx.x - e_blocks, (uint32_t)ka, (uint32_t)(ka >> 32));
   __syncthreads();
-  if (tid < DCRX_N_COUNTERS && L.counts[tid]) atomicAdd(&counters[tid], (unsigned long long)L.counts[tid]);
+  if (tid < DCRX_N_COUNTERS && L.counts[tid]) atomicAdd(&A.counters[tid], (unsigned long long)L.counts[tid]);
 }
 
 template <bool UNIFORM_LEN, int NW, int ORI>
@@ -1557,7 +1587,7 @@
     }
     if (ring_batches && want && !retry && !(cfg.flags & ~(DCRX_F_V2_SHAPE(3)))) {
       const uint32_t fixed = v2_scan_lds_bytes(T, o) + (T.lds_image_bytes - T.dfa_bytes) + T.v2[o].bk_bytes + 64u * V2_ERING_BATCHES * (uint32_t)v2_ering_stride<NW>() * 4u +
-                             DCRX_N_COUNTERS * 4u;
+                             DCRX_N_COUNTERS * 4u + 2u * R2G_ROW * 4u;
       for (uint32_t nb = ring_batches; nb >= 8u; nb >>= 1)
         if (fixed + nb * 64u * V2_RING_STRIDE * 4u <= 160u * 1024u) { ring_batches_e = nb; scan_lds_e = fixed + nb * 64u * V2_RING_STRIDE * 4u; break; }
       if (!ring_batches_e && eslot && fuse_e_env < 0) eslot->fuse_e = 0;
@@ -1754,7 +1784,8 @@
     const uint32_t rsplit = fuse_e ? 1u : rsplit_full;
     static const uint32_t rescue_waves_c = [] { const char *e = dcrx_debug_env("DCRX_DEBUG_RESCUE_WAVES_C"); const int v = e ? atoi(e) : 0; return v >= 256 ? (uint32_t)v : 0u; }();
     const uint32_t csplit = rescue_waves_c ? std::max<uint32_t>(1u, std::min<uint32_t>(64u, rescue_waves_c / n_regions)) : rsplit_full;
-    const uint32_t fgrid = (n_regions * (rsplit + csplit) + DCRX_V2_FBLOCK / 64 - 1) / (DCRX_V2_FBLOCK / 64);
+    const V2RescueSplit rs = v2_rescue_split(n_regions, rsplit | (csplit << 8));
+    const uint32_t fgrid = rs.e_blocks + rs.c_blocks;
     const uint32_t egrid = (n_regions + DCRX_V2_FBLOCK / 64 - 1) / (DCRX_V2_FBLOCK / 64);
     static const uint32_t bsplit_env = [] { const char *e = dcrx_debug_env("DCRX_DEBUG_X_BSPLIT"); const int v = e ? atoi(e) : 0; return (v >= 1 && v <= 16) ? (uint32_t)v : 0u; }();
     const uint32_t bsplit = bsplit_env ? bsplit_env : (separate ? std::max<uint32_t>(1u, std::min<uint32_t>(16u, 1024u / n_regions)) : (fuse_e ? 2u : 1u));
@@ -1799,8 +1830,7 @@
       if (cfg.flags & DCRX_F_V2_NO_LEAN_RESCUE) {
         for (int which = V2_L_E; which <= V2_L_C; which++) { e = general(s, which, true, nullptr); if (e != hipSuccess) return e; }
       } else {
-        hipLaunchKernelGGL(kr, dim3(fgrid), dim3(DCRX_V2_FBLOCK), llds, s, T, B, cfg, rec, d_counters, Q, n_regions, rsplit | (csplit << 8), queue, gqueue, qcap,
-                           queue_count, P.dev_tables);
+        hipLaunchKernelGGL(kr, dim3(fgrid), dim3(DCRX_V2_FBLOCK), llds, s, A);
         e = hipGetLastError();
         if (e != hipSuccess) return e;
       }
diff --git a/decombinator_amd/csrc/dcrx_v2_device.h b/decombinator_amd/csrc/dcrx_v2_device.h
--- a/decombinator_amd/csrc/dcrx_v2_device.h
+++ b/decombinator_amd/csrc/dcrx_v2_device.h
@@ -856,7 +856,25 @@
   uint32_t kw_base[2][2];
   uint32_t Lh[2][2];
   int32_t split[2];
+#ifndef DCRX_HOST_EMUL
+  dcrx_ldsaddr gene_rows;
+#else
+  dcrx_ldsaddr gene_rows[2 * 16];
+#endif
 };
+enum { R2G_MASK = 0, R2G_KW = 2, R2G_PK = 4, R2G_BASE = 6, R2G_LH = 8, R2G_TAGPK = 10, R2G_L = 11, R2G_SPLIT = 12, R2G_ROW = 16 };
+template <class W>
+DCRX_DEV void rescue2_gene_rows(const Rescue2Tabs &rt, W *rows) {
+  for (int g = 0; g < 2; g++) {
+    W *r = rows + g * R2G_ROW;
+    for (int h = 0; h < 2; h++) {
+      r[R2G_MASK + h] = (W)rt.h_mask[g][h]; r[R2G_KW + h] = (W)rt.h_kw[g][h]; r[R2G_PK + h] = (W)rt.h_pk[g][h];
+      r[R2G_BASE + h] = (W)rt.kw_base[g][h]; r[R2G_LH + h] = (W)rt.Lh[g][h];
+    }
+    r[R2G_TAGPK] = (W)rt.tag_pk[g]; r[R2G_L] = (W)rt.t.L[g]; r[R2G_SPLIT] = (W)(uint32_t)rt.split[g];
+    r[13] = r[14] = r[15] = (W)0;
+  }
+}
 
 DCRX_DEV Rescue2Tabs rescue2_tabs(const DevTables &T0, const V2Ori &V0, const uint8_t *side, const uint8_t *bk, const bool rev,
                                   const uint32_t (&kw_base)[K_NCLASS]) {
@@ -877,6 +895,11 @@
   }
   r.kw_begin = at_side(T0.kw_begin);
   r.kw_tags = at_side(T0.kw_tags);
+#ifndef DCRX_HOST_EMUL
+  r.gene_rows = 0;
+#else
+  rescue2_gene_rows(r, r.gene_rows);
+#endif
   return r;
 }
 
@@ -898,14 +921,30 @@
 struct GeneOf {
   const Rescue2Tabs &rt;
   bool j;
-  DCRX_DEV uint32_t h_mask(int h) const { return G >= 0 ? rt.h_mask[G < 0 ? 0 : G][h] : (j ? rt.h_mask[1][h] : rt.h_mask[0][h]); }
-  DCRX_DEV dcrx_ldsaddr h_kw(int h) const { return G >= 0 ? rt.h_kw[G < 0 ? 0 : G][h] : (j ? rt.h_kw[1][h] : rt.h_kw[0][h]); }
-  DCRX_DEV dcrx_ldsaddr h_pk(int h) const { return G >= 0 ? rt.h_pk[G < 0 ? 0 : G][h] : (j ? rt.h_pk[1][h] : rt.h_pk[0][h]); }
-  DCRX_DEV uint32_t kw_base(int h) const { return G >= 0 ? rt.kw_base[G < 0 ? 0 : G][h] : (j ? rt.kw_base[1][h] : rt.kw_base[0][h]); }
-  DCRX_DEV int Lh(int h) const { return (int)(G >= 0 ? rt.Lh[G < 0 ? 0 : G][h] : (j ? rt.Lh[1][h] : rt.Lh[0][h])); }
-  DCRX_DEV dcrx_ldsaddr tag_pk() const { return G >= 0 ? rt.tag_pk[G < 0 ? 0 : G] : (j ? rt.tag_pk[1] : rt.tag_pk[0]); }
-  DCRX_DEV int Lt() const { return (int)(G >= 0 ? rt.t.L[G < 0 ? 0 : G] : (j ? rt.t.L[1] : rt.t.L[0])); }
-  DCRX_DEV int split() const { return G >= 0 ? rt.split[G < 0 ? 0 : G] : (j ? rt.split[1] : rt.split[0]); }
+  DCRX_DEV uint32_t row(const int field) const {
+#ifndef DCRX_HOST_EMUL
+    uint32_t a = rt.gene_rows + (j ? 4u * R2G_ROW : 0u);
+    asm volatile("" : "+v"(a));
+    return dcrx_lds_at<uint32_t>(a, (uint32_t)field);
+#else
+    return (uint32_t)rt.gene_rows[(j ? R2G_ROW : 0) + field];
+#endif
+  }
+  DCRX_DEV dcrx_ldsaddr row_addr(const int field) const {
+#ifndef DCRX_HOST_EMUL
+    return row(field);
+#else
+    return rt.gene_rows[(j ? R2G_ROW : 0) + field];
+#endif
+  }
+  DCRX_DEV uint32_t h_mask(int h) const { return G >= 0 ? rt.h_mask[G < 0 ? 0 : G][h] : row(R2G_MASK + h); }
+  DCRX_DEV dcrx_ldsaddr h_kw(int h) const { return G >= 0 ? rt.h_kw[G < 0 ? 0 : G][h] : row_addr(R2G_KW + h); }
+  DCRX_DEV dcrx_ldsaddr h_pk(int h) const { return G >= 0 ? rt.h_pk[G < 0 ? 0 : G][h] : row_addr(R2G_PK + h); }
+  DCRX_DEV uint32_t kw_base(int h) const { return G >= 0 ? rt.kw_base[G < 0 ? 0 : G][h] : row(R2G_BASE + h); }
+  DCRX_DEV int Lh(int h) const { return (int)(G >= 0 ? rt.Lh[G < 0 ? 0 : G][h] : row(R2G_LH + h)); }
+  DCRX_DEV dcrx_ldsaddr tag_pk() const { return G >= 0 ? rt.tag_pk[G < 0 ? 0 : G] : row_addr(R2G_TAGPK); }
+  DCRX_DEV int Lt() const { return (int)(G >= 0 ? rt.t.L[G < 0 ? 0 : G] : row(R2G_L)); }
+  DCRX_DEV int split() const { return G >= 0 ? rt.split[G < 0 ? 0 : G] : (int)row(R2G_SPLIT); }
   DCRX_DEV uint32_t fbit() const { return G >= 0 ? (G == 0 ? V2_F_VH : V2_F_JH) : (j ? V2_F_JH : V2_F_VH); }
 };
 
```

After: 31150. 6.1% lower.
